# PoTaTo-Mika/fish-speech

Measured on AMD Instinct MI355X. Metric: audio-sec/wall-sec (RTF) + p50 first-sample latency, S2-Pro 4B @1/2/4/8 GPU, higher is better.
Workload: dtype bf16; 1 GPU; BASELINE config 2 per GPU: one utterance = 64-token prompt + 216 Dual-AR frames (top_k 30, top_p 0.8, temp 0.8) + codec decode [1,10,216] -> 442368 samples; global_batch=1, frames=216, prompt_len=64, first_chunk_frames=1, vocoder_chunks=first_chunk_frames, then growing 4x, vocoder=serial, parallelism=dp1

## Files before the change

### fish-speech_amd/csrc/fm_attn_dev.h

```cpp
#pragma once
#include "fm_common.h"
#include "fm_kernels.h"

constexpr int FAST_ATTN_MAXJ = 16;

template <typename T> __device__ __forceinline__ void ld_pair(const T* p, float& x0, float& x1) {
    if constexpr (sizeof(T) == 2) {
        const uint32_t w = *reinterpret_cast<const uint32_t*>(p);
        x0 = __uint_as_float(w << 16);
        x1 = __uint_as_float(w & 0xffff0000u);
    } else {
        x0 = ld(p, 0);
        x1 = ld(p, 1);
    }
}
template <typename T>
__device__ __forceinline__ void raw_pair(const T* qkv, int ldq, const float* qslab, int kp, int R, const T* bias,
                                         int r, size_t e, float& x0, float& x1) {
    if (qslab) {
        const size_t i = (size_t)r * ldq + e, st = (size_t)R * ldq;
        float a = qslab[i], b = qslab[i + 1];
        for (int q = 1; q < kp; ++q) {
            a += qslab[q * st + i];
            b += qslab[q * st + i + 1];
        }
        if (bias) {
            a += ld(bias, e);
            b += ld(bias, e + 1);
        }
        x0 = rnd<T>(a);
        x1 = rnd<T>(b);
    } else {
        ld_pair<T>(qkv + (size_t)r * ldq + e, x0, x1);
    }
}

template <typename T>
__device__ __forceinline__ void fast_attn_head(const FastFusedArgs<T>& a, int r, int h, int lane,
                                               unsigned long long (&tz)[7]) {
    const int hd = a.hd, g = a.nh / a.nkv, kvh = h / g, cpos = a.cpos, half = hd >> 1;
    const float* tab = a.rope + (size_t)cpos * hd;
    const int slot = a.row_slot[r];
    float q0[2], q1[2], k0[2], k1[2], v0[2], v1[2], qw0[2], qw1[2], kw0[2], kw1[2], c_[2], s_[2];
#pragma unroll
    for (int u = 0; u < 2; ++u) {
        const int p = lane + 64 * u;
        const bool ok = p < half;
        const int pp = ok ? p : 0;
        raw_pair<T>(a.qkv, a.ldqkv, a.qslab, a.qslab_kp, gridDim.x, a.qbias, r, (size_t)h * hd + 2 * pp, q0[u], q1[u]);
        raw_pair<T>(a.qkv, a.ldqkv, a.qslab, a.qslab_kp, gridDim.x, a.qbias, r, (size_t)(a.nh + kvh) * hd + 2 * pp,
                    k0[u], k1[u]);
        raw_pair<T>(a.qkv, a.ldqkv, a.qslab, a.qslab_kp, gridDim.x, a.qbias, r,
                    (size_t)(a.nh + a.nkv + kvh) * hd + 2 * pp, v0[u], v1[u]);
        qw0[u] = a.qk_norm ? ld(a.qn, 2 * pp) : 1.f;
        qw1[u] = a.qk_norm ? ld(a.qn, 2 * pp + 1) : 1.f;
        kw0[u] = a.qk_norm ? ld(a.kn, 2 * pp) : 1.f;
        kw1[u] = a.qk_norm ? ld(a.kn, 2 * pp + 1) : 1.f;
        c_[u] = tab[2 * pp];
        s_[u] = tab[2 * pp + 1];
        if (!ok) q0[u] = q1[u] = k0[u] = k1[u] = v0[u] = v1[u] = 0.f;
    }
    const size_t base = (size_t)slot * a.slot_stride + a.layer_off + (size_t)kvh * a.S * hd;
    T* kc = a.kc + base;
    T* vc = a.vc + base;
    float K0[FAST_ATTN_MAXJ][2], K1[FAST_ATTN_MAXJ][2], V0[FAST_ATTN_MAXJ][2], V1[FAST_ATTN_MAXJ][2];
#pragma unroll
    for (int j = 0; j < FAST_ATTN_MAXJ; ++j) {
        if (j < cpos) {
#pragma unroll
            for (int u = 0; u < 2; ++u) {
                const int p = lane + 64 * u;
                const int pp = p < half ? p : 0;
                ld_pair<T>(kc + (size_t)j * hd + 2 * pp, K0[j][u], K1[j][u]);
                ld_pair<T>(vc + (size_t)j * hd + 2 * pp, V0[j][u], V1[j][u]);
                if (p >= half) K0[j][u] = K1[j][u] = V0[j][u] = V1[j][u] = 0.f;
            }
        }
    }
    if (a.dbg) tz[1] = __builtin_amdgcn_s_memrealtime();
    auto prep = [&](float (&x0)[2], float (&x1)[2], const float (&w0)[2], const float (&w1)[2], bool norm) {
        if (norm) {
            float ss = 0.f;
#pragma unroll
            for (int u = 0; u < 2; ++u) ss += x0[u] * x0[u] + x1[u] * x1[u];
            ss = wave_sum(ss);
            const float rs = 1.0f / sqrtf(ss / (float)hd + a.eps);
#pragma unroll
            for (int u = 0; u < 2; ++u) {
                x0[u] = rnd<T>((x0[u] * rs) * w0[u]);
                x1[u] = rnd<T>((x1[u] * rs) * w1[u]);
            }
        }
#pragma unroll
        for (int u = 0; u < 2; ++u) {
            const float y0 = rnd<T>(x0[u] * c_[u] - x1[u] * s_[u]);
            const float y1 = rnd<T>(x1[u] * c_[u] + x0[u] * s_[u]);
            x0[u] = y0;
            x1[u] = y1;
        }
    };
    prep(q0, q1, qw0, qw1, a.qk_norm);
    prep(k0, k1, kw0, kw1, a.qk_norm);
    if (a.qdbg) {
#pragma unroll
        for (int u = 0; u < 2; ++u) {
            const int p = lane + 64 * u;
            if (p < half) {
                a.qdbg[((size_t)r * a.nh + h) * hd + 2 * p] = q0[u];
                a.qdbg[((size_t)r * a.nh + h) * hd + 2 * p + 1] = q1[u];
            }
        }
    }
    if (a.dbg) tz[2] = __builtin_amdgcn_s_memrealtime();
    if (h == kvh * g) {
#pragma unroll
        for (int u = 0; u < 2; ++u) {
            const int p = lane + 64 * u;
            if (p < half) {
                st(kc + (size_t)cpos * hd, 2 * p, k0[u]);
                st(kc + (size_t)cpos * hd, 2 * p + 1, k1[u]);
                st(vc + (size_t)cpos * hd, 2 * p, v0[u]);
                st(vc + (size_t)cpos * hd, 2 * p + 1, v1[u]);
            }
        }
    }
    float sc[FAST_ATTN_MAXJ + 1];
    float mx = -INFINITY;
#pragma unroll
    for (int j = 0; j <= FAST_ATTN_MAXJ; ++j) {
        if (j > cpos) break;
        float d = 0.f;
#pragma unroll
        for (int u = 0; u < 2; ++u) {
            const float a0 = j < cpos ? K0[j < FAST_ATTN_MAXJ ? j : 0][u] : k0[u];
            const float a1 = j < cpos ? K1[j < FAST_ATTN_MAXJ ? j : 0][u] : k1[u];
            d += q0[u] * a0 + q1[u] * a1;
        }
        d = wave_sum(d);
        sc[j] = rnd<T>(rnd<T>(d) * a.scale);
        mx = fmaxf(mx, sc[j]);
    }
    if (a.dbg) tz[3] = __builtin_amdgcn_s_memrealtime();
    float den = 0.f;
#pragma unroll
    for (int j = 0; j <= FAST_ATTN_MAXJ; ++j) {
        if (j > cpos) break;
        sc[j] = expf(sc[j] - mx);
        den += sc[j];
    }
    float o0[2] = {0.f, 0.f}, o1[2] = {0.f, 0.f};
#pragma unroll
    for (int j = 0; j <= FAST_ATTN_MAXJ; ++j) {
        if (j > cpos) break;
        const float p = rnd<T>(sc[j] / den);
#pragma unroll
        for (int u = 0; u < 2; ++u) {
            o0[u] += p * (j < cpos ? V0[j < FAST_ATTN_MAXJ ? j : 0][u] : v0[u]);
            o1[u] += p * (j < cpos ? V1[j < FAST_ATTN_MAXJ ? j : 0][u] : v1[u]);
        }
    }
    T* out = a.out + (size_t)r * a.nh * hd + (size_t)h * hd;
#pragma unroll
    for (int u = 0; u < 2; ++u) {
        const int p = lane + 64 * u;
        if (p < half) {
            st(out, 2 * p, o0[u]);
            st(out, 2 * p + 1, o1[u]);
        }
    }
}

constexpr int FATT_MAXPP = 8;
template <typename T>
__device__ __forceinline__ void fast_attn_heads8_lds(const FastFusedArgs<T>& a, int hbase, int hend, int lane,
                                                     const T* raw, const T* kvs, const T* qn, const T* kn,
                                                     const float* tab, T* out, bool store_kv, int slot) {
    const int hd = a.hd, g = a.nh / a.nkv, cpos = a.cpos, PP = hd >> 4;
    const int sub = lane & 7, h = hbase + (lane >> 3);
    const bool live = h < hend;
    const int hh = live ? h : hbase, kvh = hh / g;
    float q0[FATT_MAXPP], q1[FATT_MAXPP], k0[FATT_MAXPP], k1[FATT_MAXPP], v0[FATT_MAXPP], v1[FATT_MAXPP];
#pragma unroll
    for (int i = 0; i < FATT_MAXPP; ++i) {
        const int d = 2 * (sub + 8 * (i < PP ? i : 0));
        q0[i] = ld(raw, (size_t)hh * hd + d);
        q1[i] = ld(raw, (size_t)hh * hd + d + 1);
        k0[i] = ld(raw, (size_t)(a.nh + kvh) * hd + d);
        k1[i] = ld(raw, (size_t)(a.nh + kvh) * hd + d + 1);
        v0[i] = ld(raw, (size_t)(a.nh + a.nkv + kvh) * hd + d);
        v1[i] = ld(raw, (size_t)(a.nh + a.nkv + kvh) * hd + d + 1);
        if (i >= PP) q0[i] = q1[i] = k0[i] = k1[i] = v0[i] = v1[i] = 0.f;
    }
    auto sum8 = [](float v) {
        v += __shfl_xor(v, 1);
        v += __shfl_xor(v, 2);
        v += __shfl_xor(v, 4);
        return v;
    };
    auto prep = [&](float (&x0)[FATT_MAXPP], float (&x1)[FATT_MAXPP], const T* w, bool norm) {
        if (norm) {
            float ss = 0.f;
#pragma unroll
            for (int i = 0; i < FATT_MAXPP; ++i) ss += x0[i] * x0[i] + x1[i] * x1[i];
            ss = sum8(ss);
            const float rs = 1.0f / sqrtf(ss / (float)hd + a.eps);
#pragma unroll
            for (int i = 0; i < FATT_MAXPP; ++i) {
                const int d = 2 * (sub + 8 * (i < PP ? i : 0));
                x0[i] = rnd<T>((x0[i] * rs) * ld(w, d));
                x1[i] = rnd<T>((x1[i] * rs) * ld(w, d + 1));
            }
        }
#pragma unroll
        for (int i = 0; i < FATT_MAXPP; ++i) {
            const int d = 2 * (sub + 8 * (i < PP ? i : 0));
            const float c = tab[d], s = tab[d + 1];
            const float y0 = rnd<T>(x0[i] * c - x1[i] * s);
            const float y1 = rnd<T>(x1[i] * c + x0[i] * s);
            x0[i] = y0;
            x1[i] = y1;
        }
    };
    prep(q0, q1, qn, a.qk_norm);
    prep(k0, k1, kn, a.qk_norm);
    if (store_kv && live && h == kvh * g) {
        const size_t base = (size_t)slot * a.slot_stride + a.layer_off + (size_t)kvh * a.S * hd + (size_t)cpos * hd;
#pragma unroll
        for (int i = 0; i < FATT_MAXPP; ++i) {
            if (i < PP) {
                const int d = 2 * (sub + 8 * i);
                st(a.kc + base, d, k0[i]);
                st(a.kc + base, d + 1, k1[i]);
                st(a.vc + base, d, v0[i]);
                st(a.vc + base, d + 1, v1[i]);
            }
        }
    }
    const T* K = kvs + (size_t)(2 * kvh) * cpos * hd;
    const T* V = K + (size_t)cpos * hd;
    float sc[FAST_ATTN_MAXJ + 1];
    float mx = -INFINITY;
#pragma unroll
    for (int j = 0; j <= FAST_ATTN_MAXJ; ++j) {
        if (j > cpos) break;
        float dd = 0.f;
#pragma unroll
        for (int i = 0; i < FATT_MAXPP; ++i) {
            if (i < PP) {
                const int d = 2 * (sub + 8 * i);
                const float a0 = j < cpos ? ld(K, (size_t)j * hd + d) : k0[i];
                const float a1 = j < cpos ? ld(K, (size_t)j * hd + d + 1) : k1[i];
                dd += q0[i] * a0 + q1[i] * a1;
            }
        }
        dd = sum8(dd);
        sc[j] = rnd<T>(rnd<T>(dd) * a.scale);
        mx = fmaxf(mx, sc[j]);
    }
    float den = 0.f;
#pragma unroll
    for (int j = 0; j <= FAST_ATTN_MAXJ; ++j) {
        if (j > cpos) break;
        sc[j] = expf(sc[j] - mx);
        den += sc[j];
    }
    float o0[FATT_MAXPP], o1[FATT_MAXPP];
#pragma unroll
    for (int i = 0; i < FATT_MAXPP; ++i) o0[i] = o1[i] = 0.f;
#pragma unroll
    for (int j = 0; j <= FAST_ATTN_MAXJ; ++j) {
        if (j > cpos) break;
        const float pj = rnd<T>(sc[j] / den);
#pragma unroll
        for (int i = 0; i < FATT_MAXPP; ++i) {
            if (i < PP) {
                const int d = 2 * (sub + 8 * i);
                o0[i] += pj * (j < cpos ? ld(V, (size_t)j * hd + d) : v0[i]);
                o1[i] += pj * (j < cpos ? ld(V, (size_t)j * hd + d + 1) : v1[i]);
            }
        }
    }
    if (live) {
        T* o = out + (size_t)(h - hbase) * hd;
#pragma unroll
        for (int i = 0; i < FATT_MAXPP; ++i) {
            if (i < PP) {
                const int d = 2 * (sub + 8 * i);
                st(o, d, o0[i]);
                st(o, d + 1, o1[i]);
            }
        }
    }
}
```

### fish-speech_amd/csrc/fm_kernels.h

```cpp
#pragma once
#include <algorithm>
#include "fm_common.h"

enum { EPI_STORE = 0, EPI_RESID = 1, EPI_SWIGLU = 2, EPI_F32 = 3 };

template <typename T> void launch_swiglu_i8(hipStream_t s, const T* t, int ldt, T* act, int lda, int inter, int R);
template <typename T> void launch_pack(hipStream_t s, const T* src, int N, int K, T* dst);
template <typename T> void launch_quant_rows(hipStream_t s, T* w, int N, int K, int8_t* q, T* scale);
template <typename T> void launch_i8_to(hipStream_t s, const int8_t* q, int64_t n, T* dst);
void launch_pack_q8(hipStream_t s, const int8_t* src, int N, int K, int8_t* dst);
void launch_quant4(hipStream_t s, bf16_t* w, int N, int K, int gs, uint8_t* q, uint32_t* sz);
void launch_pack_q4(hipStream_t s, const uint8_t* q, int N, int K, uint8_t* dst);
void launch_pack_q4_rows(hipStream_t s, const uint8_t* q, int N, int K, uint32_t* dst);
void launch_pack_sz4(hipStream_t s, const uint32_t* sz, int N, int K, int gs, uint32_t* dst);

template <typename T> struct LinearArgs {
    const T* W;
    const T* W2;
    const T* bias;
    const T* X;
    int ldx, R, N, K;
    T* Y;
    int ldy;
    const T* res;
    int ldr;
    float* Yf;
    float* part = nullptr;
    int* tickets = nullptr;
    const T* wscale = nullptr;
};

template <typename T> struct QkArgs {
    const T* qkv;
    int ldqkv;
    const int* row_slot;
    const int* row_pos;
    int fixed_pos;
    int nh, nkv, hd, qk_norm;
    float eps;
    const T* qn;
    const T* kn;
    const float* rope;
    T* qout;
    T* kc;
    T* vc;
    size_t slot_stride, layer_off;
    int S;
    const float* qslab = nullptr;
    int qslab_kp = 1;
    const T* qbias = nullptr;
};

template <typename T> struct AttnArgs {
    const T* q;
    const int* row_slot;
    const int* row_pos;
    const T* kc;
    const T* vc;
    size_t slot_stride, layer_off;
    int S, nh, nkv, hd, split, maxsplit;
    float scale;
    float* part;
};

template <typename T> struct FastAttnArgs {
    const T* q;
    const int* row_slot;
    const T* kc;
    const T* vc;
    size_t slot_stride, layer_off;
    int S, nh, nkv, hd, cpos;
    float scale;
    T* out;
};

struct SlotParams {
    float temperature, top_p;
    int top_k, mask_im_end;
    uint64_t seed;
    int step;
    int force;
};

struct SampleArgs {
    const float* logits;
    int ldl, Nl;
    const int* row_slot;
    const SlotParams* sp;
    const int32_t* ras;
    int ras_stride, ras_enable;
    int slow, sb, se, im_end, cb, draw, col_idx;
    unsigned long long* dbg;
    int32_t* cols;
    int ldc;
    const int32_t* force_cols;
    float* tap;
    int tap_ld;
    int kth_fast;
};

template <typename T>
void launch_embed(hipStream_t s, const int32_t* tok, int R, const T* emb, const T* cbemb, int d,
                  int C, int cb, int sb, int se, int scale, T* x, const int* row_slot);
template <typename T>
void launch_gather_rows(hipStream_t s, const int32_t* codes, int ldc, int col, const T* table,
                        int d, int rows, int R, T* x);
template <typename T>
void launch_rmsnorm(hipStream_t s, const T* x, int ldx, const T* w, int d, float eps, T* y,
                    int ldy, int R);
template <typename T> void launch_linear(hipStream_t s, const LinearArgs<T>& a, int epi);
constexpr size_t LINEAR_PART_CAP = (size_t)8 << 20;
int linear_ksb(int N, int K, int R, int nacc, bool can_split);
template <typename T> void launch_qk_rope_cache(hipStream_t s, const QkArgs<T>& a, int R);
template <typename T>
void launch_attn(hipStream_t s, const AttnArgs<T>& a, int R, int nsplit, T* out, bool one_slot);
template <typename T> void launch_fast_attn(hipStream_t s, const FastAttnArgs<T>& a, int R);
void launch_finish(hipStream_t s, int R, const int* row_slot, int* row_pos, const int32_t* cols,
                   int ldc, int32_t* tok_in, int32_t* ras, int ras_stride, int C1, int update_ras,
                   SlotParams* sp);
template <typename T>
void launch_synth(hipStream_t s, T* dst, int64_t n, uint64_t seed, uint32_t tid, float center,
                  int log2_half);
template <typename T>
void launch_convert(hipStream_t s, const void* src, int src_bf16, int64_t n, T* dst);

enum { PRO_PLAIN = 0, PRO_NORM = 1, PRO_PRENORM = 3, PRO_FATT = 4 };
enum { EPI_SLAB = 4, EPI_SLABFIN = 5, EPI_SWIGLU8 = 7 };

template <typename T> struct FastFusedArgs {
    const T* qkv;
    int ldqkv;
    const int* row_slot;
    int nh, nkv, hd, qk_norm;
    float eps;
    const T* qn;
    const T* kn;
    const float* rope;
    T* kc;
    T* vc;
    size_t slot_stride, layer_off;
    int S, cpos;
    float scale;
    T* out;
    unsigned long long* dbg;
    float* qdbg = nullptr;
    int nwb = 4;
    const float* qslab = nullptr;
    int qslab_kp = 1;
    const T* qbias = nullptr;
    const int* row_pos = nullptr;
};
template <typename T> struct GemvArgs {
    const T* W;
    const T* W2;
    const T* bias;
    const T* X;
    int ldx;
    const int32_t* xidx;
    int xidx_ld, xidx_col;
    int xidx_rows;
    const int32_t* residx;
    const T* res;
    int ldr;
    const float* ss_in;
    int ss_gran;
    const T* nw;
    float eps;
    int R, N, K;
    T* Y;
    int ldy;
    float* Yf;
    T* res_out;
    int ldro;
    float* ss_out;
    int* tickets;
    T* xn_out;
    int ldxo;
    unsigned long long* dbg;
    FastFusedArgs<T> att;
    int fatt_off;
    const unsigned char* Wq;
    const T* wscale;
    const uint32_t* wsz;
    int q4_xsum_off;
    const T* pf_kc;
    const T* pf_vc;
    const int32_t* pf_slot;
    const int32_t* pf_pos;
    size_t pf_slot_stride, pf_layer_off;
    int pf_S, pf_nkv, pf_hd;
    int dummy_tail;
};
struct FmTuning {
    int gemv_nt = 1;
    int gemv_u = 8;
    int gemv_wpb = 4;
    int sampler_kth = 1;
    int sampler_fast = 1;
    int attn_cap = 32;
    int attn_wo = 0;
    int ksb_blocks = 512;
    int batched_fused_attn = 1;
    int attn_cap_batched = 128;
    int linear_u32 = 4;
    int linear_fill = 0;
    int attn3 = 1;
    int attn_fd = 1;
    int fd_min = 32;
    int fd_min_batched = 512;
    int fd_nw = 8;
    int fin_ksb = 0;
    int fd_nw_batched = 4;
    int fd_min16 = 256;
    int prefill_attn = 1;
    int prompt_gemm = 1;
    int prompt_skinny = 1;
    int prompt_skinny_blocks = 256;
    int prompt_unroll = 1;
    int prompt_qkv_slab = 1;
    int prompt_fin = 1;
    int prompt_swiglu = 1;
    int prompt_ks_tiles = 384;
    int prompt_ks_max = 8;
    int conv2 = 1;
    int conv_splitk = 1;
    int resunit_cfg = 1;
    int resunit_enc = 1;
    int resunit_384 = 1;
    int codec_norm = 1;
    int codec_rope = 1;
    int codec_swiglu = 1;
    int codec_fuse = 1;
    int bstream = 1;
    int bstream_kparts = 0;
    int bstream_nw = 0;
    int bs_dummy = 2;
    int gemv_dummy = 2;
    int bs_qkv_slab = 1;
    int fast_tail = 1;
    int fkv_prefetch = 0;
    int kv_prefetch = 1;
    int bstream_chain = 0;
    int bstream_acc = 1;
    int rmsnorm_block = 0;
    int ksb_balance = 0;
    int chain_max = 4;
    int chain_sleep = 4;
    int gemv_chain = 0;
    int bs_xfirst = 1;
    int bs_vec_epi = 1;
    int bsacc_kparts = 0;
    int q_u = 4;
    int fin8 = 1;
    int fin_split = 0;
    int int4_stream = 1;
    int fw_delay = 0;
    int fw_cheap = 0;
    int fw_prio = 0;
    int fattn_wo = 1;
    int row_qkv_rp = 8;
    int rowgemv_q4 = 31;
    int rowgemv = 27;
    int row_copies = 1;
    int prefix_vec = 1;
    unsigned long long* dbg = nullptr;
};
FmTuning& fm_tuning();
struct KvPrefixArgs {
    char *kc, *vc;
    char* store;
    const int* slots;
    size_t slot_stride_b, layer_stride_b, head_stride_b;
    size_t run_bytes;
    int64_t run_units;
    int nkv;
    int to_store;
};
void launch_kv_prefix_copy(hipStream_t s, const KvPrefixArgs& a, int n_layer, int nslots);
inline size_t fatt_lds_bytes(int ldqkv, int nkv, int S, int hd, size_t esz) {
    return ((size_t)ldqkv + (size_t)nkv * 2 * (S - 1) * hd + 2 * (size_t)hd) * esz + (size_t)hd * 4 + 64;
}
inline size_t gemv_lds_bytes(int R, int Kb, size_t esz) {
    return (size_t)R * (Kb + 8) * esz + 16 * sizeof(float) + (2 * 8 * 16 + 16) * (size_t)R * sizeof(float) +
           8 * 8 * sizeof(float);
}
template <typename T> void launch_gemv(hipStream_t s, const GemvArgs<T>& a, int pro, int epi, int ksb);
enum { ROWGEMV_FIN = 0, ROWGEMV_NORM_STORE = 1, ROWGEMV_NORM_SWIGLU = 2, ROWGEMV_NORM_F32 = 3 };
struct RowGemvArgs {
    const bf16_t* W;
    const int8_t* Wq;
    const bf16_t* wscale;
    const uint32_t* Wq4;
    const uint32_t* wsz;
    int gs;
    const bf16_t* X;
    int ldx;
    const int32_t* xidx;
    int xcol, xrows;
    const bf16_t* bias;
    const bf16_t* nw;
    float eps;
    const bf16_t* res;
    int ldr;
    const int32_t* residx;
    int res_col, res_rows;
    bf16_t* res_out;
    bf16_t* Y;
    float* Yf;
    int N, K;
    const bf16_t* pf_kc;
    const bf16_t* pf_vc;
    const int32_t* pf_slot;
    const int32_t* pf_pos;
    size_t pf_slot_stride, pf_layer_off;
    int pf_S, pf_nkv, pf_hd;
    unsigned long long* dbg;
};
int rowgemv_u(int K, int qm);
void launch_rowgemv(hipStream_t s, const RowGemvArgs& a, int kind);
struct FattnWoArgs {
    FastFusedArgs<bf16_t> at;
    RowGemvArgs wo;
    uint32_t* xt;
    int gen;
    int* err;
    int delay;
    int cheap;
    int prio;
    unsigned long long* dbg;
};
bool fattn_wo_ok(int nh, int nkv, int hd, int cpos, int N, int K, int qm);
void launch_fattn_wo(hipStream_t s, const FattnWoArgs& a);
constexpr int GEMV_CHAIN_MAX = 4;
constexpr int GEMV_CHAIN_LINE = 32;
constexpr int GEMV_CHAIN_SLOTS = 17;
constexpr int GEMV_CHAIN_WORDS = GEMV_CHAIN_MAX * GEMV_CHAIN_SLOTS * GEMV_CHAIN_LINE;
enum { GEMV_CHAIN_WO_W2 = 0, GEMV_CHAIN_W13 = 1, GEMV_CHAIN_QKV = 2, GEMV_CHAIN_HEAD = 3 };
template <typename T> struct GemvChainArgs {
    GemvArgs<T> st[GEMV_CHAIN_MAX];
    int kind[GEMV_CHAIN_MAX];
    int off[GEMV_CHAIN_MAX + 1];
    int n;
    unsigned* cnt;
    int* err;
    int sleep;
};
template <typename T> void launch_gemv_chain(hipStream_t s, const GemvChainArgs<T>& c);

template <typename T> struct BstreamArgs {
    const T* W;
    const T* bias;
    const T* X;
    int ldx, R, N, K;
    T* Y;
    int ldy;
    float* Yf;
    int kparts = 1;
    const T* wscale = nullptr;
    unsigned long long* dbg = nullptr;
    int pro = 0;
    const float* ss_in = nullptr;
    const T* nw = nullptr;
    float eps = 0.f;
    const T* res = nullptr;
    int ldr = 0;
    T* res_out = nullptr;
    int ldro = 0;
    float* ss_out = nullptr;
    int* tickets = nullptr;
    int dummy_tail = 0;
    int xfirst = 1;
    int vec_epi = 1;
};
struct BstreamPlan {
    bool ok = false;
    int kparts = 1, nw = 0, spw = 0, tpi = 1, grid = 0;
    int acc = 0, ntm = 0;
};
BstreamPlan bstream_plan(int N, int K, int R, int epi, size_t esz);
void bsacc_init();
template <typename T> bool launch_bstream(hipStream_t s, const BstreamArgs<T>& a, int epi, const BstreamPlan& p);
template <typename T> struct FinalizeArgs {
    const float* slab;
    int kparts, lds;
    const T* bias;
    const T* res;
    int ldr;
    T* x_out;
    int ldx;
    const T* nw;
    float eps;
    T* xn_out;
    int ldxn, d, R;
    const T* wscale = nullptr;
    int ch = 0;
    int* cnt = nullptr;
    float* ss_part = nullptr;
    int fin8 = 0;
    int* err = nullptr;
};
template <typename T> void launch_finalize_norm(hipStream_t s, const FinalizeArgs<T>& a);

struct PromptSkinnyArgs {
    const bf16_t* w;
    const bf16_t* x;
    int ldx, R, N, K;
    float* slab;
    bf16_t* act = nullptr;
    int lda = 0;
};
void launch_prompt_skinny(hipStream_t s, const PromptSkinnyArgs& a, int ks);
int prompt_skinny_ks(int N, int K, int target);

template <typename T> struct AttnDecArgs {
    const T* qkv;
    int ldqkv;
    const int* row_slot;
    const int* row_pos;
    int nh, nkv, hd, qk_norm;
    float eps;
    const T* qn;
    const T* kn;
    const float* rope;
    T* kc;
    T* vc;
    size_t slot_stride, layer_off;
    int S, maxsplit;
    float scale;
    float* part;
    int cap;
    int* cnt;
    T* out;
    unsigned long long* dbg;
    float* qdbg = nullptr;
    int nwb = 4;
    const float* qslab = nullptr;
    int qslab_kp = 1;
    const T* qbias = nullptr;
};
template <typename T> void launch_attn_decode2(hipStream_t s, const AttnDecArgs<T>& a, int R);
inline size_t attn2_lds_bytes(int hd, int g, int cap, size_t esz) {
    return (size_t)cap * (hd + 8) * esz + (size_t)cap * hd * esz + (size_t)g * hd * 4 + (size_t)g * cap * 4 +
           16 + 8 * (size_t)g * 4;
}
inline int attn2_cap(int hd, int g, size_t esz) {
    long budget = 150L * 1024 - 16 - 8L * g * 4 - (long)g * hd * 4;
    long per = (long)(2 * hd + 8) * (long)esz + 4L * g;
    long c = budget / per;
    c = c > 256 ? 256 : c;
    return (int)(c & ~15L);
}
constexpr int FD_NSP = 16;
inline bool attn_fd_ok(int hd, int g) { return (hd == 32 || hd == 64 || hd == 128) && g >= 1 && g <= 4; }
template <typename T> void launch_attn_fd(hipStream_t s, const AttnDecArgs<T>& a, int R);
template <typename T> void launch_attn_decode3(hipStream_t s, const AttnDecArgs<T>& a, int R);
template <typename T> void launch_fast_attn_fused(hipStream_t s, const FastFusedArgs<T>& a, int R);
template <typename T> void launch_fast_attn2(hipStream_t s, const FastFusedArgs<T>& a, int R);
template <typename T> void launch_sample_radix(hipStream_t s, const SampleArgs& a, int R);
void sample_init();
template <typename T>
void launch_attn_combine(hipStream_t s, const float* part, const int* row_pos, int R, int nh, int hd,
                         int split, int maxsplit, T* out);
```

### fish-speech_amd/csrc/fm_llm.cpp

```cpp
#include <dlfcn.h>
#include <execinfo.h>
#include <hip/hip_runtime.h>
#include <math.h>
#include <signal.h>

#include <algorithm>
#include <array>
#include <memory>

#include "fm_codec.h"
#include "fm_kernels.h"
#include "fm_runtime.h"

namespace {
void segv_trace(int sig, siginfo_t* si, void*) {
    void* fr[64];
    const int n = backtrace(fr, 64);
    fprintf(stderr, "fishmi: signal %d at address %p, %d frames\n", sig, si ? si->si_addr : nullptr, n);
    for (int i = 0; i < n; ++i) {
        Dl_info d{};
        if (dladdr(fr[i], &d) && d.dli_fname)
            fprintf(stderr, "  #%d %s +0x%lx (%s)\n", i, d.dli_fname,
                    (unsigned long)((const char*)fr[i] - (const char*)d.dli_fbase), d.dli_sname ? d.dli_sname : "?");
        else
            fprintf(stderr, "  #%d %p\n", i, fr[i]);
    }
    fflush(stderr);
    signal(sig, SIG_DFL);
    raise(sig);
}
struct SegvTraceInstaller {
    SegvTraceInstaller() {
        const char* e = getenv("FISHMI_SEGV_TRACE");
        if (!e || e[0] != '1') return;
        struct sigaction sa {};
        sa.sa_sigaction = segv_trace;
        sa.sa_flags = SA_SIGINFO;
        sigaction(SIGSEGV, &sa, nullptr);
        sigaction(SIGBUS, &sa, nullptr);
    }
} g_segv_trace;
}

static thread_local std::string g_err;
void fm_set_error(const std::string& s) { g_err = s; }
extern "C" const char* fm_last_error(void) { return g_err.c_str(); }
extern "C" int fm_device_count(void) {
    int n = 0;
    if (hipGetDeviceCount(&n) != hipSuccess) return 0;
    return n;
}

static constexpr int PREFILL_CHUNK = 1024;
static constexpr int ATTN_PIECE = 256;
static constexpr int ATTN_SPLIT = 64;
static constexpr int GEMV_MAX_ROWS = 8;
static constexpr int KSB_MAX = 8;
static constexpr int BS_KPARTS = 8;

FmTuning& fm_tuning() {
    static FmTuning t;
    return t;
}

static int pick_ksb(int N, int K, int R, size_t esz) {
    const int nb = (N + 15) / 16;
    const FmTuning& tu = fm_tuning();
    int ksb = 1;
    while (ksb < KSB_MAX && nb * ksb < tu.ksb_blocks && K % (32 * ksb * 2) == 0) ksb *= 2;
    if (tu.ksb_balance) {
        double best = 1e9;
        int bk = ksb;
        for (int k = 1; k <= KSB_MAX && K % (32 * k) == 0; k *= 2) {
            const int b = nb * k;
            if (b < 256) continue;
            const double rounds = (double)((b + 255) / 256), waste = rounds * 256.0 / b;
            if (waste < best - 1e-3) {
                best = waste;
                bk = k;
            }
        }
        ksb = bk;
    }
    while (gemv_lds_bytes(R, K / ksb, esz) > 96 * 1024 && ksb < KSB_MAX && K % (32 * ksb * 2) == 0) ksb *= 2;
    while (K / ksb > 4096 && K % (32 * ksb * 2) == 0) ksb *= 2;
    return ksb;
}

struct LayerW {
    void *wqkv = nullptr, *bqkv = nullptr, *wo = nullptr, *bo = nullptr, *qn = nullptr, *kn = nullptr;
    void *w13 = nullptr, *w2 = nullptr, *an = nullptr, *fn = nullptr;
    void *wo_rm = nullptr, *w2_rm = nullptr, *wqkv_rm = nullptr, *w13_rm = nullptr;
};

struct StackDims {
    int n_layer, dim, nh, nkv, hd, inter, qkv_bias, o_bias, qk_norm;
    int nq() const { return nh * hd; }
    int nqkv() const { return (nh + 2 * nkv) * hd; }
};

struct fm_llm {
    fm_model_config c{};
    int device = 0, prec = FM_PREC_BF16, max_slots = 1;
    size_t esz = 2;
    hipStream_t stream = nullptr;
    std::map<std::string, DTensor> w;
    bool finalized = false;
    StackDims sd{}, fdm{};
    int S = 0, C = 0, C1 = 0, cb = 0, nsem = 0, Nhead = 0, maxsplit = 0, Rmax = 0;
    std::vector<LayerW> slow, fast;
    void *emb = nullptr, *cbemb = nullptr, *norm = nullptr, *head_c = nullptr, *fproj_w = nullptr,
         *fproj_b = nullptr, *femb = nullptr, *fnorm = nullptr, *fout = nullptr;
    void *kc = nullptr, *vc = nullptr, *fkc = nullptr, *fvc = nullptr;
    size_t slot_stride = 0, layer_stride = 0, fslot_stride = 0, flayer_stride = 0;
    float *rope = nullptr, *frope = nullptr;
    void *x = nullptr, *h = nullptr, *xn = nullptr, *qkv = nullptr, *q = nullptr, *att = nullptr,
         *act = nullptr;
    void *xl = nullptr, *xnl = nullptr, *fx = nullptr, *fh = nullptr, *fxn = nullptr;
    void *x2 = nullptr, *fx2 = nullptr;
    unsigned* chain_cnt = nullptr;
    int* chain_err = nullptr;
    int* h_chain_err = nullptr;
    void* plast = nullptr;
    float *part = nullptr, *logits = nullptr, *flogits = nullptr;
    void* act2 = nullptr;
    int* attn_cnt = nullptr;
    float *ssX = nullptr, *ssH = nullptr;
    int* tickets = nullptr;
    float* skpart = nullptr;
    long long skpart_cap = 0;
    float *slabA = nullptr, *slabB = nullptr;
    float *bsA = nullptr, *bsB = nullptr;
    float* bsQ = nullptr;
    int *frame_slot = nullptr, *frame_pos = nullptr, *prow_slot = nullptr, *prow_pos = nullptr;
    int32_t *tok_in = nullptr, *cols = nullptr, *ptok = nullptr, *ras = nullptr;
    SlotParams* sp = nullptr;
    int32_t* force_cols = nullptr;
    float *tap_slow = nullptr, *tap_fast = nullptr;
    std::vector<int> host_force;
    int32_t* h_cols = nullptr;
    int32_t* h_hist = nullptr;
    size_t h_hist_n = 0;
    std::vector<int> host_pos, host_step;
    std::vector<int> uploaded_slots;
    bool use_graph = true;
    std::map<int, hipGraphExec_t> graphs;
    Profiler prof;
    std::vector<void*> allocs;
    int quant = FM_QUANT_NONE;
    int q4_gs = 0;
    int* fin_cnt = nullptr;
    float* fin_ss = nullptr;
    struct QInfo {
        const unsigned char* q8 = nullptr;
        const void* scale = nullptr;
        const uint32_t* sz = nullptr;
    };
    std::map<const void*, QInfo> qmap;
    std::map<const void*, void*> rowmajor;
    std::map<const void*, const void*> rowsz;
    std::map<const void*, const void*> rowscale;
    bool row_ok = false;
    bool row_qkv_ok = false;
    bool row_w13_ok = false;
    uint32_t* fxt = nullptr;
    void* fout_rm = nullptr;
    int32_t* fiota = nullptr;
    struct Prefix {
        void* buf = nullptr;
        int npos = 0;
        size_t bytes = 0;
    };
    std::map<int, Prefix> prefixes;
    int next_prefix_id = 1;
    int* pfx_slots = nullptr;
    const QInfo* qinfo(const void* W) const {
        auto it = qmap.find(W);
        return it == qmap.end() ? nullptr : &it->second;
    }

    ~fm_llm() {
        if (device >= 0) (void)hipSetDevice(device);
        for (auto& g : graphs) (void)hipGraphExecDestroy(g.second);
        for (auto& kv : w) {
            if (kv.second.p) (void)hipFree(kv.second.p);
            if (kv.second.q) (void)hipFree(kv.second.q);
        }
        for (void* p : allocs) (void)hipFree(p);
        for (auto& kv : prefixes) (void)hipFree(kv.second.buf);
        if (h_cols) (void)hipHostFree(h_cols);
        if (h_hist) (void)hipHostFree(h_hist);
        if (h_chain_err) (void)hipHostFree(h_chain_err);
        if (stream) (void)hipStreamDestroy(stream);
    }
    void* dalloc(size_t bytes, bool zero = true) {
        void* p = nullptr;
        if (bytes == 0) bytes = 16;
        hipError_t e = hipMalloc(&p, bytes);
        if (e != hipSuccess)
            throw FmError{FM_ERR_OOM, "hipMalloc(" + std::to_string(bytes) + ") failed: " + hipGetErrorString(e)};
        if (zero) HIPCHK(hipMemsetAsync(p, 0, bytes, stream));
        allocs.push_back(p);
        return p;
    }
};

static void add_t(fm_llm* m, const std::string& n, int64_t rows, int64_t cols) {
    DTensor t;
    t.rows = rows;
    t.cols = cols;
    t.numel = rows * cols;
    m->w[n] = t;
}
static void add_stack(fm_llm* m, const std::string& pre, const StackDims& s) {
    for (int i = 0; i < s.n_layer; ++i) {
        std::string p = pre + std::to_string(i) + ".";
        add_t(m, p + "attention.wqkv.weight", s.nqkv(), s.dim);
        if (s.qkv_bias) add_t(m, p + "attention.wqkv.bias", 1, s.nqkv());
        add_t(m, p + "attention.wo.weight", s.dim, s.nq());
        if (s.o_bias) add_t(m, p + "attention.wo.bias", 1, s.dim);
        if (s.qk_norm) {
            add_t(m, p + "attention.q_norm.weight", 1, s.hd);
            add_t(m, p + "attention.k_norm.weight", 1, s.hd);
        }
        add_t(m, p + "feed_forward.w1.weight", s.inter, s.dim);
        add_t(m, p + "feed_forward.w3.weight", s.inter, s.dim);
        add_t(m, p + "feed_forward.w2.weight", s.dim, s.inter);
        add_t(m, p + "ffn_norm.weight", 1, s.dim);
        add_t(m, p + "attention_norm.weight", 1, s.dim);
    }
}

static void build_inventory(fm_llm* m) {
    const fm_model_config& c = m->c;
    m->sd = StackDims{c.n_layer, c.dim, c.n_head, c.n_local_heads, c.head_dim, c.intermediate_size,
                      c.qkv_bias, c.o_bias, c.qk_norm};
    m->fdm = StackDims{c.n_fast_layer, c.fast_dim, c.fast_n_head, c.fast_n_local_heads, c.fast_head_dim,
                       c.fast_intermediate_size, c.fast_qkv_bias, c.fast_o_bias, c.fast_qk_norm};
    add_t(m, "embeddings.weight", c.vocab_size, c.dim);
    add_t(m, "codebook_embeddings.weight", (int64_t)c.codebook_size * c.num_codebooks, c.dim);
    add_stack(m, "layers.", m->sd);
    add_t(m, "norm.weight", 1, c.dim);
    if (!c.tie_word_embeddings) add_t(m, "output.weight", c.vocab_size, c.dim);
    if (c.fast_dim != c.dim) {
        add_t(m, "fast_project_in.weight", c.fast_dim, c.dim);
        add_t(m, "fast_project_in.bias", 1, c.fast_dim);
    }
    add_t(m, "fast_embeddings.weight", c.codebook_size, c.fast_dim);
    add_stack(m, "fast_layers.", m->fdm);
    add_t(m, "fast_norm.weight", 1, c.fast_dim);
    add_t(m, "fast_output.weight", c.codebook_size, c.fast_dim);
}

static DTensor& tensor_for(fm_llm* m, const char* name, int64_t numel) {
    auto it = m->w.find(name);
    FMCHECK(it != m->w.end(), std::string("unknown tensor: ") + name);
    FMCHECK(it->second.numel == numel, std::string("wrong numel for ") + name + ": got " +
                                           std::to_string(numel) + ", want " + std::to_string(it->second.numel));
    DTensor& t = it->second;
    if (!t.p) {
        const int64_t rows = t.rows > 1 ? (t.rows + 15) / 16 * 16 : 1;
        const size_t bytes = (size_t)rows * t.cols * m->esz;
        HIPCHK(hipMalloc(&t.p, bytes));
        HIPCHK(hipMemsetAsync(t.p, 0, bytes, m->stream));
    }
    return t;
}

template <typename T> struct Run {
    typedef T type_t;
    fm_llm* m;
    hipStream_t s;
    int64_t E;
    bool rows_distinct_slots = false;
    explicit Run(fm_llm* mm) : m(mm), s(mm->stream), E(sizeof(T)) {}

    bool prompt_gemm(const void* W, const void* W2, const void* bias, const void* X, int ldx, int R, int N, int K,
                     void* Y, int ldy, const void* res, int ldr, int epi, const char* cls) {
        if (R <= 32 || W2 || m->qinfo(W) || !fm_tuning().prompt_gemm ||
            (epi != EPI_STORE && epi != EPI_RESID && epi != EPI_SWIGLU8) || N % 16 || K % 32 || N < 96 ||
            (epi == EPI_SWIGLU8 && (bias || N % 16)))
            return false;
        ConvArgs<T> c{};
        c.x = (const T*)X;
        c.ldx = ldx;
        c.Ci = K;
        c.Lq = R;
        c.Lx = R;
        c.w = (const T*)W;
        c.Co = N;
        c.ntaps = 1;
        c.stride = 1;
        c.nphase = 1;
        c.bias = (const T*)bias;
        c.res = epi == EPI_RESID ? (const T*)res : nullptr;
        c.ldr = ldr;
        c.out = Y;
        c.ldo = ldy;
        c.flags = CE_STORE | (bias ? CE_BIAS : 0) | (epi == EPI_RESID ? CE_RES : 0) |
                  (epi == EPI_SWIGLU8 ? CE_SWIGLU8 : 0);
        hipStream_t st = s;
        const int64_t bytes = (int64_t)N * K * E + (int64_t)R * K * E + (int64_t)R * N * E;
        const double flops = 2.0 * R * N * K;
        if constexpr (sizeof(T) == 2) {
            auto al16 = [](const void* p) { return ((uintptr_t)p & 15) == 0; };
            const int ks = prompt_skinny_ks(N, K, fm_tuning().prompt_skinny_blocks);
            if (fm_tuning().prompt_skinny && ks > 0 && R <= 64 && ldx % 8 == 0 && al16(X) && al16(Y) && ldy % 8 == 0 &&
                (!c.res || (al16(c.res) && ldr % 8 == 0)) && (long long)ks * R * N <= m->skpart_cap) {
                c.ksplit = ks;
                c.slab = m->skpart;
                c.slab_cap = (size_t)m->skpart_cap;
                PromptSkinnyArgs p{(const bf16_t*)W, (const bf16_t*)X, ldx, R, N, K, m->skpart};
                const bool direct = ks == 1 && epi == EPI_SWIGLU8;
                if (direct) {
                    p.act = (bf16_t*)Y;
                    p.lda = ldy;
                }
                auto go = [st, c, p, ks, direct] {
                    launch_prompt_skinny(st, p, ks);
                    if (!direct) launch_conv_epi<T>(st, c);
                };
                m->prof.record(cls, bytes, go);
                run_(cls, bytes, flops, go);
                return true;
            }
        }
        if (epi == EPI_SWIGLU8) return false;
        const long long t128 = (long long)FM_CEIL(R, 128) * FM_CEIL(N, 128);
        int ks = 1;
        while (t128 * ks < fm_tuning().prompt_ks_tiles && ks < fm_tuning().prompt_ks_max && K / 32 >= 8 * ks * 2)
            ks *= 2;
        c.ksplit = ks;
        c.slab = m->skpart;
        c.slab_cap = (size_t)m->skpart_cap;
        auto go = [st, c] { launch_conv_gemm<T>(st, c); };
        m->prof.record(cls, bytes, go);
        run_(cls, bytes, flops, go);
        return true;
    }
    bool prompt_slab(const void* W, const void* X, int ldx, int R, int N, int K, int* ks_out) {
        if constexpr (sizeof(T) != 2) {
            return false;
        } else {
            if (!fm_tuning().prompt_fin || !fm_tuning().prompt_skinny || !fm_tuning().prompt_gemm || R <= 32 ||
                R > 64 || m->qinfo(W) || N % 16 || K % 32 || ldx % 8 || ((uintptr_t)X & 15))
                return false;
            const int ks = prompt_skinny_ks(N, K, fm_tuning().prompt_skinny_blocks);
            if (ks <= 0 || (long long)ks * R * N > m->skpart_cap) return false;
            const PromptSkinnyArgs p{(const bf16_t*)W, (const bf16_t*)X, ldx, R, N, K, m->skpart};
            hipStream_t st = s;
            auto go = [st, p, ks] { launch_prompt_skinny(st, p, ks); };
            const int64_t bytes = (int64_t)N * K * E + (int64_t)R * K * E + (int64_t)ks * R * N * 4;
            m->prof.record("linear", bytes, go);
            run_("linear", bytes, 2.0 * R * N * K, go);
            *ks_out = ks;
            return true;
        }
    }
    void linear(const void* W, const void* W2, const void* bias, const void* X, int ldx, int R, int N,
                int K, void* Y, int ldy, const void* res, int ldr, float* Yf, int epi, const char* cls) {
        if (bs_use(R, false) && !W2 && !res && (epi == EPI_F32 || epi == EPI_STORE) &&
            bs_linear(W, bias, X, ldx, R, N, K, Y, ldy, Yf, epi))
            return;
        if (prompt_gemm(W, W2, bias, X, ldx, R, N, K, Y, ldy, res, ldr, epi, cls)) return;
        LinearArgs<T> a{(const T*)W, (const T*)W2, (const T*)bias, (const T*)X, ldx, R, N, K, (T*)Y,
                        ldy, (const T*)res, ldr, Yf};
        if (const auto* q = m->qinfo(W)) a.wscale = (const T*)q->scale;
        if (R > GEMV_MAX_ROWS && R <= 64) {
            FMCHECK(m->skpart_cap >= (long long)LINEAR_PART_CAP, "split-K partial buffer too small");
            a.part = m->skpart;
            a.tickets = m->tickets;
        }
        const int64_t wbytes = (int64_t)N * K * E * (epi == EPI_SWIGLU ? 2 : 1);
        const int64_t bytes = wbytes + (int64_t)R * K * E + (int64_t)R * N * (epi == EPI_F32 ? 4 : E);
        const double flops = 2.0 * R * N * K * (epi == EPI_SWIGLU ? 2 : 1);
        hipStream_t st = s;
        auto go = [st, a, epi] { launch_linear<T>(st, a, epi); };
        m->prof.record(cls, bytes, go);
        run_(cls, bytes, flops, go);
    }

    struct BsPending {
        bool on = false;
        const float* slab = nullptr;
        int kparts = 0, d = 0, R = 0;
        void* res = nullptr;
        void* out = nullptr;
        const void* sc = nullptr;
    } pend;
    void attn_slow(const AttnDecArgs<T>& aa, int R) { attn_slow_on(s, aa, R); }
    static void attn_slow_on(hipStream_t s, const AttnDecArgs<T>& aa, int R) {
        if (fm_tuning().attn_fd && attn_fd_ok(aa.hd, aa.nh / aa.nkv)) {
            AttnDecArgs<T> b = aa;
            b.cap = std::max(16, R > GEMV_MAX_ROWS ? fm_tuning().fd_min_batched : fm_tuning().fd_min);
            if (R <= GEMV_MAX_ROWS && fm_tuning().fd_nw > 4) {
                b.nwb = fm_tuning().fd_nw;
                b.cap = std::max(16, fm_tuning().fd_min16);
            } else if (R > GEMV_MAX_ROWS && fm_tuning().fd_nw_batched > 4) {
                b.nwb = fm_tuning().fd_nw_batched;
            }
            launch_attn_fd<T>(s, b, R);
        } else if (fm_tuning().attn3 && R > GEMV_MAX_ROWS && aa.hd % 32 == 0 && aa.hd <= 128 && aa.nh / aa.nkv <= 6)
            launch_attn_decode3<T>(s, aa, R);
        else
            launch_attn_decode2<T>(s, aa, R);
    }
    bool bs_frame = false;
    bool bs_use(int R, bool) const {
        return fm_tuning().bstream && bs_frame && R > GEMV_MAX_ROWS && R <= 32 && m->bsA;
    }
    struct BsExtra {
        int pro = PRO_PLAIN;
        const float* ss_in = nullptr;
        const void* nw = nullptr;
        const void* res = nullptr;
        void* res_out = nullptr;
        float* ss_out = nullptr;
    };
    bool bs_linear(const void* W, const void* bias, const void* X, int ldx, int R, int N, int K, void* Y, int ldy,
                   float* Yf, int epi, int* kparts_out = nullptr, const BsExtra* ex = nullptr) {
        const BstreamPlan p = bstream_plan(N, K, R, epi, E);
        if (!p.ok || ((epi == EPI_SLABFIN || (ex && ex->pro == PRO_PRENORM)) && !p.acc)) return false;
        BstreamArgs<T> a{(const T*)W, (const T*)bias, (const T*)X, ldx, R, N, K, (T*)Y, ldy, Yf};
        if (const auto* q = m->qinfo(W)) a.wscale = (const T*)q->scale;
        a.dbg = fm_tuning().dbg;
        if (ex) {
            a.pro = ex->pro;
            a.ss_in = ex->ss_in;
            a.nw = (const T*)ex->nw;
            a.eps = m->c.norm_eps;
            a.res = (const T*)ex->res;
            a.ldr = N;
            a.res_out = (T*)ex->res_out;
            a.ldro = N;
            a.ss_out = ex->ss_out;
            a.tickets = m->tickets;
        }
        const int64_t bytes = (int64_t)N * K * E + (int64_t)R * K * E +
                              (int64_t)R * N * (epi == EPI_SLAB ? 4 * p.kparts : (epi == EPI_F32 ? 4 : E));
        const double flops = 2.0 * R * N * K;
        hipStream_t st = s;
        auto go = [st, a, epi, p] { FMCHECK(launch_bstream<T>(st, a, epi, p), "bstream: no kernel for the plan"); };
        m->prof.record("linear", bytes, go);
        run_("linear", bytes, flops, go);
        if (kparts_out) *kparts_out = p.kparts;
        return true;
    }
    const void* wscale(const void* W) const {
        const auto* q = m->qinfo(W);
        return q ? q->scale : nullptr;
    }
    bool x_ss = false;
    bool bs_chain(const StackDims& d, int R) const {
        if (!fm_tuning().bstream_chain || E != 2 || R > 32) return false;
        auto ok = [&](int N, int K, int epi) { return bstream_plan(N, K, R, epi, E).acc; };
        return ok(d.nqkv(), d.dim, EPI_STORE) && ok(d.dim, d.nq(), EPI_SLABFIN) && ok(2 * d.inter, d.dim, EPI_SWIGLU8) &&
               ok(d.dim, d.inter, EPI_SLABFIN);
    }
    void finalize_norm(const float* slab, int kparts, const void* bias, const void* res, void* out, const void* nw,
                       void* xn, int d, int R, const void* sc) {
        FinalizeArgs<T> f{slab, kparts, d, (const T*)bias, (const T*)res, d, (T*)out, d, (const T*)nw,
                          m->c.norm_eps, (T*)xn, d, d, R, (const T*)sc};
        if (fm_tuning().fin_split > 1 && m->fin_cnt) {
            f.ch = fm_tuning().fin_split;
            f.cnt = m->fin_cnt;
            f.ss_part = m->fin_ss;
            f.err = m->chain_err;
        }
        run_("norm", 0, 0, [&] { launch_finalize_norm<T>(s, f); });
    }
// ... 28 lines not shown
            e.ss_in = m->ssX;
            e.nw = L.an;
            FMCHECK(bs_linear(L.wqkv, L.bqkv, xb, d.dim, R, d.nqkv(), d.dim, m->qkv, d.nqkv(), nullptr, EPI_STORE,
                              nullptr, &e),
                    "bsacc: no PRENORM QKV plan");
        } else if (bs) {
            bs_norm_in(d, L, R, xb, xnb);
            int kp = 0;
            const bool fused_fast = is_fast && fixed_pos >= 0 && fixed_pos < 16 && d.hd <= 256;
            const bool fused_slow = !is_fast && rows_distinct_slots && fm_tuning().attn_fd &&
                                    attn_fd_ok(d.hd, d.nh / d.nkv);
            const bool slab_ok = fm_tuning().bs_qkv_slab && fm_tuning().batched_fused_attn && m->bsQ && R <= 32 &&
                                 (fused_fast || fused_slow) && !m->qinfo(L.wqkv);
            if (slab_ok && bs_linear(L.wqkv, nullptr, xnb, d.dim, R, d.nqkv(), d.dim, nullptr, d.nqkv(), m->bsQ,
                                     EPI_SLAB, &kp)) {
                qslab = m->bsQ;
                qslab_kp = kp;
            } else if (!bs_linear(L.wqkv, L.bqkv, xnb, d.dim, R, d.nqkv(), d.dim, m->qkv, d.nqkv(), nullptr, EPI_STORE))
                linear(L.wqkv, nullptr, L.bqkv, xnb, d.dim, R, d.nqkv(), d.dim, m->qkv, d.nqkv(), nullptr, 0,
                       nullptr, EPI_STORE, "linear");
        } else {
            bs_norm_in(d, L, R, xb, xnb);
            int kq = 0;
            if (!is_fast && !rows_distinct_slots && fm_tuning().prompt_qkv_slab &&
                prompt_slab(L.wqkv, xnb, d.dim, R, d.nqkv(), d.dim, &kq)) {
                qslab = m->skpart;
                qslab_kp = kq;
            } else {
                linear(L.wqkv, nullptr, L.bqkv, xnb, d.dim, R, d.nqkv(), d.dim, m->qkv, d.nqkv(), nullptr, 0,
                       nullptr, EPI_STORE, "linear");
            }
        }
        const float scale = 1.0f / sqrtf((float)d.hd);
        const bool rows_are_slots = is_fast || rows_distinct_slots;
        if (rows_are_slots && !is_fast && fm_tuning().batched_fused_attn) {
            AttnDecArgs<T> aa{(const T*)m->qkv, d.nqkv(), rslot, rpos, d.nh, d.nkv, d.hd, d.qk_norm, eps,
                              (const T*)L.qn, (const T*)L.kn, rope, (T*)kc, (T*)vc, sstride, loff, Sc,
                              m->maxsplit, scale, m->part};
            aa.cap = attn2_cap(d.hd, d.nh / d.nkv, E);
            if (fm_tuning().attn_cap_batched) aa.cap = std::min(aa.cap, fm_tuning().attn_cap_batched);
            aa.maxsplit = FM_CEIL(Sc, aa.cap);
            aa.cnt = m->attn_cnt;
            aa.dbg = fm_tuning().dbg;
            aa.out = (T*)m->att;
            aa.qslab = qslab;
            aa.qslab_kp = qslab_kp;
            aa.qbias = (const T*)L.bqkv;
            FMCHECK(!qslab || (fm_tuning().attn_fd && attn_fd_ok(d.hd, d.nh / d.nkv)), "bs_qkv_slab needs attn_fd");
            hipStream_t st = s;
            auto go = [st, aa, R] { attn_slow_on(st, aa, R); };
            m->prof.record("attn_slow", 0, go);
            run_rec("attn", go);
        } else if (is_fast && fm_tuning().batched_fused_attn && fixed_pos >= 0 && fixed_pos < 16 && d.hd <= 256) {
            FastFusedArgs<T> fa{(const T*)m->qkv, d.nqkv(), rslot, d.nh, d.nkv, d.hd, d.qk_norm, eps,
                                (const T*)L.qn, (const T*)L.kn, rope, (T*)kc, (T*)vc, sstride, loff, Sc,
                                fixed_pos, scale, (T*)m->att};
            fa.dbg = fm_tuning().dbg;
            fa.qslab = qslab;
            fa.qslab_kp = qslab_kp;
            fa.qbias = (const T*)L.bqkv;
            hipStream_t st = s;
            run_rec("attn", [st, fa, R] { launch_fast_attn2<T>(st, fa, R); });
        } else {
            QkArgs<T> qa{(const T*)m->qkv, d.nqkv(), rslot, rpos, fixed_pos, d.nh, d.nkv, d.hd, d.qk_norm,
                         eps, (const T*)L.qn, (const T*)L.kn, rope, (T*)m->q, (T*)kc, (T*)vc, sstride, loff, Sc};
            qa.qslab = qslab;
            qa.qslab_kp = qslab_kp;
            qa.qbias = (const T*)L.bqkv;
            run_("rope", 0, 0, [&] { launch_qk_rope_cache<T>(s, qa, R); });
            if (!is_fast) {
                auto attn_rows = [&](int r0, int len, bool one_slot) {
                    for (int p0 = r0; p0 < r0 + len; p0 += ATTN_PIECE) {
                        const int pn = std::min(ATTN_PIECE, r0 + len - p0);
                        const size_t o = (size_t)p0 * d.nh * d.hd;
                        AttnArgs<T> aa{(const T*)m->q + o, rslot + p0, rpos + p0, (const T*)kc, (const T*)vc, sstride,
                                       loff, Sc, d.nh, d.nkv, d.hd, ATTN_SPLIT, m->maxsplit, scale, m->part};
                        run_("attn", 0, 0, [&] { launch_attn<T>(s, aa, pn, m->maxsplit, (T*)m->att + o, one_slot); });
                    }
                };
                if (!segs.empty())
                    for (const auto& sg : segs) attn_rows(sg[0], sg[1], true);
                else
                    attn_rows(0, R, !rows_are_slots);
            } else {
                FastAttnArgs<T> fa{(const T*)m->q, rslot, (const T*)kc, (const T*)vc, sstride, loff, Sc,
                                   d.nh, d.nkv, d.hd, fixed_pos, scale, (T*)m->att};
                run_("attn", 0, 0, [&] { launch_fast_attn<T>(s, fa, R); });
            }
        }
        int kp = 0;
        if (chain) {
            BsExtra eo;
            eo.res = xb;
            eo.res_out = hb;
            eo.ss_out = m->ssH;
            FMCHECK(bs_linear(L.wo, L.bo, m->att, d.nq(), R, d.dim, d.nq(), nullptr, d.dim, m->bsA, EPI_SLABFIN, &kp, &eo),
                    "bsacc: no SLABFIN wo plan");
            BsExtra e13;
            e13.pro = PRO_PRENORM;
            e13.ss_in = m->ssH;
            e13.nw = L.fn;
            FMCHECK(bs_linear(L.w13, nullptr, hb, d.dim, R, 2 * d.inter, d.dim, m->act, d.inter, nullptr, EPI_SWIGLU8,
                              nullptr, &e13),
                    "bsacc: no PRENORM w13 plan");
            BsExtra e2;
            e2.res = hb;
            e2.res_out = xb;
            e2.ss_out = m->ssX;
            FMCHECK(bs_linear(L.w2, nullptr, m->act, d.inter, R, d.dim, d.inter, nullptr, d.dim, m->bsB, EPI_SLABFIN, &kp,
                              &e2),
                    "bsacc: no SLABFIN w2 plan");
            x_ss = true;
            return;
        }
        if (bs && bs_linear(L.wo, nullptr, m->att, d.nq(), R, d.dim, d.nq(), nullptr, d.dim, m->bsA, EPI_SLAB, &kp)) {
            finalize_norm(m->bsA, kp, L.bo, xb, hb, L.fn, xnb, d.dim, R, wscale(L.wo));
        } else if (!bs && prompt_slab(L.wo, m->att, d.nq(), R, d.dim, d.nq(), &kp)) {
            finalize_norm(m->skpart, kp, L.bo, xb, hb, L.fn, xnb, d.dim, R, nullptr);
        } else {
            linear(L.wo, nullptr, L.bo, m->att, d.nq(), R, d.dim, d.nq(), hb, d.dim, xb, d.dim, nullptr,
                   EPI_RESID, "linear");
            run_("norm", 0, 0, [&] {
                launch_rmsnorm<T>(s, (const T*)hb, d.dim, (const T*)L.fn, d.dim, eps, (T*)xnb, d.dim, R);
            });
        }
        if (!(bs && bs_linear(L.w13, nullptr, xnb, d.dim, R, 2 * d.inter, d.dim, m->act, d.inter, nullptr,
                              EPI_SWIGLU8))) {
            if (!(fm_tuning().prompt_swiglu &&
                  prompt_gemm(L.w13, nullptr, nullptr, xnb, d.dim, R, 2 * d.inter, d.dim, m->act, d.inter, nullptr, 0,
                              EPI_SWIGLU8, "linear"))) {
                linear(L.w13, nullptr, nullptr, xnb, d.dim, R, 2 * d.inter, d.dim, m->act2, 2 * d.inter, nullptr, 0,
                       nullptr, EPI_STORE, "linear");
                run_("other", 0, 0, [&] {
                    launch_swiglu_i8<T>(s, (const T*)m->act2, 2 * d.inter, (T*)m->act, d.inter, d.inter, R);
                });
            }
        }
        if (bs && bs_linear(L.w2, nullptr, m->act, d.inter, R, d.dim, d.inter, nullptr, d.dim, m->bsB, EPI_SLAB, &kp)) {
            pend.on = true;
            pend.slab = m->bsB;
            pend.kparts = kp;
            pend.d = d.dim;
            pend.R = R;
            pend.res = hb;
            pend.out = xb;
            pend.sc = wscale(L.w2);
        } else if (!bs && prompt_slab(L.w2, m->act, d.inter, R, d.dim, d.inter, &kp)) {
            pend.on = true;
            pend.slab = m->skpart;
            pend.kparts = kp;
            pend.d = d.dim;
            pend.R = R;
            pend.res = hb;
            pend.out = xb;
            pend.sc = nullptr;
        } else {
            linear(L.w2, nullptr, nullptr, m->act, d.inter, R, d.dim, d.inter, xb, d.dim, hb, d.dim, nullptr,
                   EPI_RESID, "linear");
        }
    }

    GemvArgs<T> ga() {
        GemvArgs<T> a{};
        a.eps = m->c.norm_eps;
        a.dummy_tail = fm_tuning().gemv_dummy;
        return a;
    }
    struct ChainSt {
        GemvArgs<T> a;
        int kind;
        int64_t bytes;
        double flops;
    };
    std::vector<ChainSt> chain;
    int chain_kind(const GemvArgs<T>& a, int pro, int epi, int ksb) const {
        const FmTuning& t = fm_tuning();
        if (!t.gemv_chain || m->prof.on || ksb != 1 || a.R != 1 || a.Wq || m->qinfo(a.W) || !t.gemv_nt ||
            t.gemv_u != 8 || t.gemv_wpb != 4 || a.N % 16 || a.xidx)
            return -1;
        if (pro == PRO_PLAIN && epi == EPI_SLABFIN) return GEMV_CHAIN_WO_W2;
        if (a.xn_out || a.K > 4096 || pro != PRO_PRENORM) return a.xn_out && pro == PRO_PRENORM && epi == EPI_F32 &&
                                                                    a.K <= 4096 ? GEMV_CHAIN_HEAD : -1;
        if (epi == EPI_SWIGLU8) return GEMV_CHAIN_W13;
        if (epi == EPI_STORE) return GEMV_CHAIN_QKV;
        if (epi == EPI_F32) return GEMV_CHAIN_HEAD;
        return -1;
    }
    void chain_flush() {
        if (chain.empty()) return;
        std::vector<ChainSt> c;
        c.swap(chain);
        if (c.size() == 1) {
            static const int pro_of[4] = {PRO_PLAIN, PRO_PRENORM, PRO_PRENORM, PRO_PRENORM};
            static const int epi_of[4] = {EPI_SLABFIN, EPI_SWIGLU8, EPI_STORE, EPI_F32};
            gemv_now(c[0].a, pro_of[c[0].kind], epi_of[c[0].kind], 1, "linear");
            return;
        }
        GemvChainArgs<T> g{};
        int64_t bytes = 0;
        double flops = 0;
        g.n = (int)c.size();
        for (int i = 0; i < g.n; ++i) {
            g.st[i] = c[i].a;
            if (!g.st[i].tickets) g.st[i].tickets = m->tickets;
            g.kind[i] = c[i].kind;
            bytes += c[i].bytes;
            flops += c[i].flops;
        }
        g.cnt = m->chain_cnt;
        g.err = m->chain_err;
        g.sleep = fm_tuning().chain_sleep;
        hipStream_t st = s;
        auto go = [st, g] { launch_gemv_chain<T>(st, g); };
        m->prof.record("linear", bytes, go);
        m->prof.run(s, "linear", bytes, flops, go);
    }
    void gemv(GemvArgs<T> a, int pro, int epi, int ksb, const char* cls) {
        const int kind = chain_kind(a, pro, epi, ksb);
        if (kind < 0) {
            chain_flush();
            gemv_now(a, pro, epi, ksb, cls);
            return;
        }
        const size_t E = sizeof(T);
        const int64_t bytes = (int64_t)a.N * a.K * E + (int64_t)a.K * E;
        chain.push_back(ChainSt{a, kind, bytes, 2.0 * a.N * a.K});
        if ((int)chain.size() >= std::min(GEMV_CHAIN_MAX, fm_tuning().chain_max) || kind == GEMV_CHAIN_HEAD)
            chain_flush();
    }
    void gemv_now(GemvArgs<T> a, int pro, int epi, int ksb, const char* cls) {
        int64_t wbytes = (int64_t)a.N * a.K * E * (epi == EPI_SWIGLU ? 2 : 1);
        const auto* q = m->qinfo(a.W);
        if (q && q->sz && !fm_tuning().int4_stream) q = nullptr;
        if (q) {
            a.Wq = q->q8;
            if (q->sz) {
                a.wsz = q->sz;
                a.wscale = nullptr;
                while (ksb > 1 && (a.K / ksb) % 128) ksb /= 2;
                wbytes = (int64_t)a.N * a.K / 2 + (int64_t)(a.N + 15) / 16 * 16 * (a.K / 128) * 4;
            } else {
                a.wscale = (const T*)q->scale;
                while (ksb > 1 && (a.K / ksb) % 64) ksb /= 2;
                wbytes = (int64_t)a.N * a.K;
            }
        }
        const int64_t bytes = wbytes + (int64_t)a.R * a.K * E;
        const double flops = 2.0 * a.R * a.N * a.K * (epi == EPI_SWIGLU ? 2 : 1);
        hipStream_t st = s;
        if (!a.tickets) a.tickets = m->tickets;
        auto go = [st, a, pro, epi, ksb] { launch_gemv<T>(st, a, pro, epi, ksb); };
        m->prof.record(cls, bytes, go);
        m->prof.run(s, cls, bytes, flops, go);
    }
    int row_bits() const {
        const FmTuning& t = fm_tuning();
        return m->quant == FM_QUANT_INT4 ? t.rowgemv_q4 : t.rowgemv;
    }
    bool row_fin(int n) const {
        const FmTuning& t = fm_tuning();
        return sizeof(T) == 2 && n == 1 && m->row_ok && (row_bits() & 1) && !t.gemv_chain && !t.attn_wo &&
               (m->quant != FM_QUANT_INT4 || t.int4_stream);
    }
    bool row_qkv(int n) const {
        const FmTuning& t = fm_tuning();
        return sizeof(T) == 2 && n == 1 && m->row_qkv_ok && m->quant != FM_QUANT_INT8 && (row_bits() & 2) &&
               !t.gemv_chain && (m->quant != FM_QUANT_INT4 || t.int4_stream);
    }
    bool row_w13(int n) const {
        const FmTuning& t = fm_tuning();
        return sizeof(T) == 2 && n == 1 && m->row_w13_ok && (row_bits() & 4) && !t.gemv_chain &&
               (m->quant != FM_QUANT_INT4 || t.int4_stream);
    }
    void rowgemv(const RowGemvArgs& a, int kind) {
        chain_flush();
        const int64_t wbytes = a.Wq4 ? (int64_t)a.N * a.K / 2 + (int64_t)a.N * (a.K / a.gs) * 4
                               : (a.Wq ? (int64_t)a.N * a.K + (int64_t)a.N * 2 : (int64_t)a.N * a.K * 2);
        const int64_t bytes = wbytes + (int64_t)a.K * 2;
        hipStream_t st = s;
        auto go = [st, a, kind] { launch_rowgemv(st, a, kind); };
        m->prof.record("linear", bytes, go);
        m->prof.run(s, "linear", bytes, 2.0 * a.N * a.K, go);
    }
    template <typename F> void run_(const char* cls, int64_t bytes, double flops, F&& f) {
        chain_flush();
        m->prof.run(s, cls, bytes, flops, std::forward<F>(f));
    }
    template <typename F> void run_rec(const char* cls, F go) {
        chain_flush();
        m->prof.record(cls, 0, go);
        m->prof.run(s, cls, 0, 0, go);
    }
    struct KsbPlan {
        int wo, w2;
    };
    KsbPlan plan(const StackDims& d, int n) {
        auto fin_ksb = [&](int N, int K) {
            const int fk = fm_tuning().fin_ksb;
            if (fk > 0 && K % (32 * fk) == 0) return fk;
            return gemv_lds_bytes(n, K, E) <= 120 * 1024 ? 1 : pick_ksb(N, K, n, E);
        };
        return KsbPlan{fin_ksb(d.dim, d.nq()), fin_ksb(d.dim, d.inter)};
    }
    void block_small(const StackDims& d, const LayerW& L, int n, bool first, const void* x_in, int ldx_in,
                     const int32_t* xidx, int xcol, void* xb, void* hb, bool is_fast, int cpos, int layer,
                     const KsbPlan& kp, void* xo, bool kv_only = false) {
        const int C1 = m->C1;
        const float scale = 1.0f / sqrtf((float)d.hd);
        FastFusedArgs<T> fa{(const T*)m->qkv, d.nqkv(), m->frame_slot, d.nh, d.nkv, d.hd, d.qk_norm,
                            m->c.norm_eps, (const T*)L.qn, (const T*)L.kn, m->frope, (T*)m->fkc,
                            (T*)m->fvc, m->fslot_stride, (size_t)layer * m->flayer_stride, m->C, cpos,
                            scale, (T*)m->att};
        fa.dbg = fm_tuning().dbg;
        const bool rf = row_fin(n);
        auto row_w = [&](RowGemvArgs& r, void* rm, const void* packed) {
            if (m->quant == FM_QUANT_INT4) {
                r.Wq4 = (const uint32_t*)rm;
                r.wsz = (const uint32_t*)m->rowsz.at(packed);
                r.gs = m->q4_gs;
            } else if (m->quant) {
                r.Wq = (const int8_t*)rm;
                auto it = m->rowscale.find(packed);
                r.wscale = (const bf16_t*)(it != m->rowscale.end() ? it->second : m->qinfo(packed)->scale);
            } else {
                r.W = (const bf16_t*)rm;
            }
        };
        const int fq = m->quant == FM_QUANT_INT8 ? 1 : (m->quant == FM_QUANT_INT4 ? 2 : 0);
        const bool fw = is_fast && !kv_only && rf && fm_tuning().fattn_wo && m->fxt && m->fdm.n_layer * m->C >= 2 &&
                        m->fdm.n_layer * m->C <= 40 &&
                        fattn_wo_ok(d.nh, d.nkv, d.hd, cpos, d.dim, d.nq(), fq);
        const bool att_wo = is_fast && !kv_only && fm_tuning().attn_wo && !m->quant && n == 1 && cpos < 16 && d.hd % 16 == 0 &&
                            d.hd <= 128 && d.nh % d.nkv == 0 && (d.nq() / kp.wo) % d.hd == 0 && d.nqkv() % 8 == 0;
        {
            GemvArgs<T> a = ga();
            a.W = (const T*)L.wqkv;
            a.bias = (const T*)L.bqkv;
            a.nw = (const T*)L.an;
            a.R = n;
            a.N = d.nqkv();
            a.K = d.dim;
            a.Y = (T*)m->qkv;
            a.ldy = d.nqkv();
            if (!is_fast && n == 1 && fm_tuning().kv_prefetch) {
                a.pf_kc = (const T*)m->kc;
                a.pf_vc = (const T*)m->vc;
                a.pf_slot = m->frame_slot;
                a.pf_pos = m->frame_pos;
                a.pf_slot_stride = m->slot_stride;
                a.pf_layer_off = (size_t)layer * m->layer_stride;
                a.pf_S = m->S;
                a.pf_nkv = d.nkv;
                a.pf_hd = d.hd;
            } else if (is_fast && n == 1 && fm_tuning().fkv_prefetch && m->fiota && cpos < 16) {
                a.pf_kc = (const T*)m->fkc;
                a.pf_vc = (const T*)m->fvc;
                a.pf_slot = m->frame_slot;
                a.pf_pos = m->fiota + cpos;
                a.pf_slot_stride = m->fslot_stride;
                a.pf_layer_off = (size_t)layer * m->flayer_stride;
                a.pf_S = m->C;
                a.pf_nkv = d.nkv;
                a.pf_hd = d.hd;
            }
            const int epi = EPI_STORE;
            if (row_qkv(n) && (!first || (row_bits() & 16))) {
                RowGemvArgs r{};
                row_w(r, L.wqkv_rm, L.wqkv);
                if (first) {
                    r.X = (const bf16_t*)x_in;
                    r.ldx = ldx_in;
                    r.xidx = xidx;
                    r.xcol = xcol;
                    r.xrows = xidx ? m->cb : 0;
                } else {
                    r.X = (const bf16_t*)xb;
                }
                r.bias = (const bf16_t*)L.bqkv;
                r.nw = (const bf16_t*)L.an;
                r.eps = m->c.norm_eps;
                r.Y = (bf16_t*)m->qkv;
                r.N = d.nqkv();
                r.K = d.dim;
                r.pf_kc = (const bf16_t*)a.pf_kc;
                r.pf_vc = (const bf16_t*)a.pf_vc;
                r.pf_slot = a.pf_slot;
                r.pf_pos = a.pf_pos;
                r.pf_slot_stride = a.pf_slot_stride;
                r.pf_layer_off = a.pf_layer_off;
                r.pf_S = a.pf_S;
                r.pf_nkv = a.pf_nkv;
                r.pf_hd = a.pf_hd;
                rowgemv(r, ROWGEMV_NORM_STORE);
            } else if (first) {
                a.X = (const T*)x_in;
                a.ldx = ldx_in;
                a.xidx = xidx;
                a.xidx_ld = C1;
                a.xidx_col = xcol;
                a.xidx_rows = xidx ? m->cb : 0;
                gemv(a, PRO_NORM, epi, 1, "linear");
            } else {
                a.X = (const T*)xb;
                a.ldx = d.dim;
                a.ss_in = m->ssX;
                a.ss_gran = rf ? 1 : 0;
                gemv(a, PRO_PRENORM, epi, 1, "linear");
            }
        }
        if (!is_fast) {
            AttnDecArgs<T> aa{(const T*)m->qkv, d.nqkv(), m->frame_slot, m->frame_pos, d.nh, d.nkv, d.hd,
                              d.qk_norm, m->c.norm_eps, (const T*)L.qn, (const T*)L.kn, m->rope, (T*)m->kc,
                              (T*)m->vc, m->slot_stride, (size_t)layer * m->layer_stride, m->S,
                              m->maxsplit, scale, m->part};
            aa.cap = attn2_cap(d.hd, d.nh / d.nkv, E);
            if (fm_tuning().attn_cap) aa.cap = std::min(aa.cap, fm_tuning().attn_cap);
            aa.maxsplit = FM_CEIL(m->S, aa.cap);
            aa.cnt = m->attn_cnt;
            aa.dbg = fm_tuning().dbg;
            aa.out = (T*)m->att;
            hipStream_t st = s;
            auto go = [st, aa, n] { attn_slow_on(st, aa, n); };
            m->prof.record("attn_slow", 0, go);
            run_rec("attn", go);
        } else if (!att_wo && !fw) {
            hipStream_t st = s;
            const bool f2 = cpos < 16 && d.hd <= 256;
            run_rec("attn", [st, fa, n, f2] {
                if (f2)
                    launch_fast_attn2<T>(st, fa, n);
                else
                    launch_fast_attn_fused<T>(st, fa, n);
            });
        }
        if (kv_only) return;
        if (fw) {
            FattnWoArgs A{};
            A.at = *reinterpret_cast<const FastFusedArgs<bf16_t>*>(&fa);
            A.at.dbg = nullptr;
            A.at.row_pos = m->frame_pos;
            RowGemvArgs& r = A.wo;
            row_w(r, L.wo_rm, L.wo);
            r.X = (const bf16_t*)m->att;
            r.bias = (const bf16_t*)L.bo;
            if (first) {
                r.res = (const bf16_t*)x_in;
                r.ldr = ldx_in;
                r.residx = xidx;
                r.res_col = xcol;
                r.res_rows = xidx ? m->cb : 0;
            } else {
                r.res = (const bf16_t*)xb;
                r.ldr = d.dim;
            }
            r.res_out = (bf16_t*)hb;
            r.N = d.dim;
            r.K = d.nq();
            A.xt = m->fxt;
            A.gen = 1 + layer + m->fdm.n_layer * cpos;
            A.err = m->chain_err;
            A.delay = fm_tuning().fw_delay;
            A.cheap = fm_tuning().fw_cheap;
            A.prio = fm_tuning().fw_prio;
            chain_flush();
            const int64_t bytes = r.Wq4 ? (int64_t)r.N * r.K / 2 + (int64_t)r.N * (r.K / r.gs) * 4
                                  : (r.Wq ? (int64_t)r.N * r.K + (int64_t)r.N * 2 : (int64_t)r.N * r.K * 2);
            hipStream_t st = s;
            auto go = [st, A] { launch_fattn_wo(st, A); };
            m->prof.record("attn_wo", bytes, go);
            m->prof.run(s, "attn", bytes, 2.0 * r.N * r.K, go);
        } else if (rf) {
            RowGemvArgs r{};
            row_w(r, L.wo_rm, L.wo);
            r.X = (const bf16_t*)m->att;
            r.bias = (const bf16_t*)L.bo;
            if (first) {
                r.res = (const bf16_t*)x_in;
                r.ldr = ldx_in;
                r.residx = xidx;
                r.res_col = xcol;
                r.res_rows = xidx ? m->cb : 0;
            } else {
                r.res = (const bf16_t*)xb;
                r.ldr = d.dim;
            }
            r.res_out = (bf16_t*)hb;
            r.N = d.dim;
            r.K = d.nq();
            rowgemv(r, ROWGEMV_FIN);
        } else {
            GemvArgs<T> a = ga();
            a.W = (const T*)L.wo;
            a.bias = (const T*)L.bo;
            a.X = (const T*)m->att;
            a.ldx = d.nq();
            a.R = n;
            a.N = d.dim;
            a.K = d.nq();
            a.Yf = m->slabA;
            a.ldy = d.dim;
            if (first) {
                a.res = (const T*)x_in;
                a.ldr = ldx_in;
                a.residx = xidx;
                a.xidx_ld = C1;
                a.xidx_col = xcol;
                a.xidx_rows = xidx ? m->cb : 0;
            } else {
                a.res = (const T*)xb;
                a.ldr = d.dim;
            }
            a.res_out = (T*)hb;
            a.ldro = d.dim;
            a.ss_out = m->ssH;
            a.tickets = m->tickets;
            if (att_wo) {
                a.att = fa;
                gemv(a, PRO_FATT, EPI_SLABFIN, kp.wo, "linear");
            } else {
                gemv(a, PRO_PLAIN, EPI_SLABFIN, kp.wo, "linear");
            }
        }
        if (row_w13(n)) {
            RowGemvArgs r{};
            row_w(r, L.w13_rm, L.w13);
            r.X = (const bf16_t*)hb;
            r.nw = (const bf16_t*)L.fn;
            r.eps = m->c.norm_eps;
            r.Y = (bf16_t*)m->act;
            r.N = 2 * d.inter;
            r.K = d.dim;
            rowgemv(r, ROWGEMV_NORM_SWIGLU);
        } else {
            GemvArgs<T> a = ga();
            a.W = (const T*)L.w13;
            a.nw = (const T*)L.fn;
            a.R = n;
            a.N = 2 * d.inter;
            a.K = d.dim;
            a.X = (const T*)hb;
            a.ldx = d.dim;
            a.ss_in = m->ssH;
            a.ss_gran = rf ? 1 : 0;
            a.Y = (T*)m->act;
            a.ldy = d.inter;
            gemv(a, PRO_PRENORM, EPI_SWIGLU8, 1, "linear");
        }
        if (rf) {
            RowGemvArgs r{};
            row_w(r, L.w2_rm, L.w2);
            r.X = (const bf16_t*)m->act;
            r.res = (const bf16_t*)hb;
            r.ldr = d.dim;
            r.res_out = (bf16_t*)xo;
            r.N = d.dim;
            r.K = d.inter;
            rowgemv(r, ROWGEMV_FIN);
        } else {
            GemvArgs<T> a = ga();
            a.W = (const T*)L.w2;
            a.X = (const T*)m->act;
            a.ldx = d.inter;
            a.R = n;
            a.N = d.dim;
            a.K = d.inter;
            a.Yf = m->slabB;
            a.ldy = d.dim;
            a.res = (const T*)hb;
            a.ldr = d.dim;
            a.res_out = (T*)xo;
            a.ldro = d.dim;
            a.ss_out = m->ssX;
            a.tickets = m->tickets;
            gemv(a, PRO_PLAIN, EPI_SLABFIN, kp.w2, "linear");
        }
    }

    void* xbuf(void* x0, void* x1, int l) const { return (fm_tuning().gemv_chain && (l & 1)) ? x1 : x0; }
    void* xfin = nullptr;
    void slow_small(int n) {
        const KsbPlan kp = plan(m->sd, n);
        for (int l = 0; l < m->sd.n_layer; ++l)
            block_small(m->sd, m->slow[l], n, l == 0, m->x, m->c.dim, nullptr, 0, xbuf(m->x, m->x2, l), m->h, false, 0,
                        l, kp, xbuf(m->x, m->x2, l + 1));
        xfin = xbuf(m->x, m->x2, m->sd.n_layer);
    }

    const void* head_small(const void* xlast, bool pending, int n, int ksb_prev) {
        const fm_model_config& c = m->c;
        GemvArgs<T> a = ga();
        a.W = (const T*)m->head_c;
        a.nw = (const T*)m->norm;
        a.R = n;
        a.N = m->Nhead;
        a.K = c.dim;
        a.Yf = m->logits;
        a.ldy = m->Nhead;
        a.xn_out = (T*)m->xnl;
        a.ldxo = c.dim;
        const void* xs = xfin ? xfin : m->x;
        if (pending) {
            a.X = (const T*)xs;
            a.ldx = c.dim;
            a.ss_in = m->ssX;
            a.ss_gran = row_fin(n) ? 1 : 0;
            gemv(a, PRO_PRENORM, EPI_F32, 1, "linear");
        } else {
            a.X = (const T*)xlast;
            a.ldx = c.dim;
            gemv(a, PRO_NORM, EPI_F32, 1, "linear");
        }
        const void* hid = c.norm_fastlayer_input ? m->xnl : (pending ? xs : xlast);
        if (m->fproj_w) {
            GemvArgs<T> p = ga();
            p.W = (const T*)m->fproj_w;
            p.bias = (const T*)m->fproj_b;
            p.X = (const T*)hid;
            p.ldx = c.dim;
            p.R = n;
            p.N = c.fast_dim;
            p.K = c.dim;
            p.Y = (T*)m->xl;
            p.ldy = c.fast_dim;
            gemv(p, PRO_PLAIN, EPI_STORE, 1, "linear");
            return m->xl;
        }
        return hid;
    }

    void fast_small(int n, int cc, bool with_head, const void* hidden) {
        const fm_model_config& c = m->c;
        const KsbPlan kp = plan(m->fdm, n);
        for (int l = 0; l < m->fdm.n_layer; ++l) {
            const bool first = l == 0;
            const void* xin = cc == 0 ? hidden : m->femb;
            const int32_t* xidx = cc == 0 ? nullptr : m->cols;
            const bool kv_only = !with_head && l == m->fdm.n_layer - 1 && fm_tuning().fast_tail;
            block_small(m->fdm, m->fast[l], n, first, xin, c.fast_dim, xidx, cc, xbuf(m->fx, m->fx2, l), m->fh, true,
                        cc, l, kp, xbuf(m->fx, m->fx2, l + 1), kv_only);
        }
        if (with_head && sizeof(T) == 2 && n == 1 && m->fout_rm && (row_bits() & 8) && !fm_tuning().gemv_chain &&
            (m->quant != FM_QUANT_INT4 || fm_tuning().int4_stream)) {
            RowGemvArgs r{};
            auto row_w = [&](RowGemvArgs& rr, void* rm, const void* packed) {
                if (m->quant == FM_QUANT_INT4) {
                    rr.Wq4 = (const uint32_t*)rm;
                    rr.wsz = (const uint32_t*)m->rowsz.at(packed);
                    rr.gs = m->q4_gs;
                } else if (m->quant) {
                    rr.Wq = (const int8_t*)rm;
                    rr.wscale = (const bf16_t*)m->qinfo(packed)->scale;
                } else {
                    rr.W = (const bf16_t*)rm;
                }
            };
            row_w(r, m->fout_rm, m->fout);
            r.X = (const bf16_t*)xbuf(m->fx, m->fx2, m->fdm.n_layer);
            r.nw = (const bf16_t*)m->fnorm;
            r.eps = c.norm_eps;
            r.Yf = m->flogits;
            r.N = m->cb;
            r.K = c.fast_dim;
            rowgemv(r, ROWGEMV_NORM_F32);
        } else if (with_head) {
            GemvArgs<T> a = ga();
            a.W = (const T*)m->fout;
            a.nw = (const T*)m->fnorm;
            a.R = n;
            a.N = m->cb;
            a.K = c.fast_dim;
            a.Yf = m->flogits;
            a.ldy = m->cb;
            a.X = (const T*)xbuf(m->fx, m->fx2, m->fdm.n_layer);
            a.ldx = c.fast_dim;
            a.ss_in = m->ssX;
            a.ss_gran = row_fin(n) ? 1 : 0;
            gemv(a, PRO_PRENORM, EPI_F32, 1, "linear");
        }
    }

    void frame_tail_small(int n, bool ras_enable, bool sample, const void* hidden) {
        if (sample) {
            SampleArgs a = sargs(true, ras_enable, 0);
            run_("sample", 0, 0, [&] { launch_sample_radix<T>(s, a, n); });
        }
        fast_small(n, 0, false, hidden);
        for (int cc = 1; cc < m->C; ++cc) {
            fast_small(n, cc, true, hidden);
            if (sample) {
                SampleArgs a = sargs(false, 0, cc);
                run_("sample", 0, 0, [&] { launch_sample_radix<T>(s, a, n); });
            }
        }
    }

    void decode_frame_small(int n) {
        run_("other", 0, 0, [&] {
            launch_embed<T>(s, m->tok_in, n, (const T*)m->emb, (const T*)m->cbemb, m->c.dim, m->C, m->cb,
                            m->c.semantic_begin_id, m->c.semantic_end_id, m->c.scale_codebook_embeddings,
                            (T*)m->x, m->frame_slot);
        });
        slow_small(n);
        const KsbPlan kp = plan(m->sd, n);
        const void* hid = head_small(nullptr, true, n, kp.w2);
        frame_tail_small(n, true, true, hid);
        chain_flush();
        launch_finish(s, n, m->frame_slot, m->frame_pos, m->cols, m->C1, m->tok_in, m->ras, m->C1 * 10, m->C1,
                      1, m->sp);
    }

    void slow_layers(int R, const int* rslot, const int* rpos) {
        x_ss = false;
        for (int l = 0; l < m->sd.n_layer; ++l)
            block(m->sd, m->slow[l], R, rslot, rpos, -1, false, m->kc, m->vc, m->slot_stride,
                  (size_t)l * m->layer_stride, m->S, m->rope, m->x, m->h, m->xn);
        flush();
    }

    void head_and_hidden(const void* xlast, int n) {
        const fm_model_config& c = m->c;
        chain_flush();
        run_("norm", 0, 0, [&] {
            launch_rmsnorm<T>(s, (const T*)xlast, c.dim, (const T*)m->norm, c.dim, c.norm_eps, (T*)m->xnl,
                              c.dim, n);
        });
        linear(m->head_c, nullptr, nullptr, m->xnl, c.dim, n, m->Nhead, c.dim, nullptr, m->Nhead,
               nullptr, 0, m->logits, EPI_F32, "linear");
        const void* src = c.norm_fastlayer_input ? m->xnl : xlast;
        if (m->fproj_w)
            linear(m->fproj_w, nullptr, m->fproj_b, src, c.dim, n, c.fast_dim, c.dim, m->fx, c.fast_dim,
                   nullptr, 0, nullptr, EPI_STORE, "linear");
        else
            HIPCHK(hipMemcpyAsync(m->fx, src, (size_t)n * c.dim * E, hipMemcpyDeviceToDevice, s));
    }

    void fast_pass(int n, int cpos, bool with_head) {
        const fm_model_config& c = m->c;
        x_ss = false;
        for (int l = 0; l < m->fdm.n_layer; ++l)
            block(m->fdm, m->fast[l], n, m->frame_slot, nullptr, cpos, true, m->fkc, m->fvc,
                  m->fslot_stride, (size_t)l * m->flayer_stride, m->C, m->frope, m->fx, m->fh, m->fxn);
        flush();
        if (with_head) {
            run_("norm", 0, 0, [&] {
                launch_rmsnorm<T>(s, (const T*)m->fx, c.fast_dim, (const T*)m->fnorm, c.fast_dim,
                                  c.norm_eps, (T*)m->fxn, c.fast_dim, n);
            });
            linear(m->fout, nullptr, nullptr, m->fxn, c.fast_dim, n, m->cb, c.fast_dim, nullptr, m->cb,
                   nullptr, 0, m->flogits, EPI_F32, "linear");
        }
    }

    SampleArgs sargs(bool slow, int ras_enable, int c) {
        const fm_model_config& cc = m->c;
        SampleArgs a{};
        a.logits = slow ? m->logits : m->flogits;
        a.ldl = slow ? m->Nhead : m->cb;
        a.Nl = a.ldl;
        a.row_slot = m->frame_slot;
        a.sp = m->sp;
        a.ras = m->ras;
        a.ras_stride = m->C1 * 10;
        a.ras_enable = ras_enable;
        a.slow = slow;
        a.sb = cc.semantic_begin_id;
        a.se = cc.semantic_end_id;
// ... 354 lines not shown
            if (qi.q8) m->qmap[pk] = qi;
            const bool keep = row_keep(m, kv.first, (int)t.rows, (int)t.cols);
            if (keep) {
                void* rw = m->dalloc((size_t)t.rows * t.cols / 2, false);
                launch_pack_q4_rows(m->stream, (const uint8_t*)t.q, (int)t.rows, (int)t.cols, (uint32_t*)rw);
                HIPCHK(hipGetLastError());
                m->rowmajor[pk] = rw;
                m->rowsz[pk] = t.s;
                m->allocs.push_back(const_cast<void*>(t.s));
            }
            HIPCHK(hipStreamSynchronize(m->stream));
            HIPCHK(hipFree(t.q));
            if (!keep) HIPCHK(hipFree(const_cast<void*>(t.s)));
            t.q = nullptr;
            t.s = nullptr;
        } else if (m->quant) {
            m->qmap[pk] = fm_llm::QInfo{(const unsigned char*)pack_q8_dev(m, t.q, (int)t.rows, (int)t.cols), t.s};
            HIPCHK(hipStreamSynchronize(m->stream));
            if (row_keep(m, kv.first, (int)t.rows, (int)t.cols)) {
                m->rowmajor[pk] = t.q;
                m->allocs.push_back(t.q);
            } else {
                HIPCHK(hipFree(t.q));
            }
            t.q = nullptr;
        }
        HIPCHK(hipStreamSynchronize(m->stream));
        if (!m->quant && row_keep(m, kv.first, (int)t.rows, (int)t.cols)) {
            m->rowmajor[pk] = t.p;
            m->allocs.push_back(t.p);
        } else {
            HIPCHK(hipFree(t.p));
        }
        t.p = pk;
    }
    auto stack = [&](const std::string& pre, const StackDims& d, std::vector<LayerW>& out) {
        out.resize(d.n_layer);
        for (int i = 0; i < d.n_layer; ++i) {
            std::string p = pre + std::to_string(i) + ".";
            LayerW& L = out[i];
            L.wqkv = W(m, p + "attention.wqkv.weight");
            L.bqkv = Wopt(m, p + "attention.wqkv.bias");
            L.wo = W(m, p + "attention.wo.weight");
            L.bo = Wopt(m, p + "attention.wo.bias");
            L.qn = Wopt(m, p + "attention.q_norm.weight");
            L.kn = Wopt(m, p + "attention.k_norm.weight");
            L.w13 = pack_w13(m, p, d.inter, d.dim);
            L.w2 = W(m, p + "feed_forward.w2.weight");
            L.an = W(m, p + "attention_norm.weight");
            L.fn = W(m, p + "ffn_norm.weight");
            auto rm = [&](const void* pk) -> void* {
                auto it = m->rowmajor.find(pk);
                return it == m->rowmajor.end() ? nullptr : it->second;
            };
            L.wo_rm = rm(L.wo);
            L.w2_rm = rm(L.w2);
            L.wqkv_rm = rm(L.wqkv);
            L.w13_rm = rm(L.w13);
        }
    };
    stack("layers.", m->sd, m->slow);
    stack("fast_layers.", m->fdm, m->fast);
    {
        int32_t io[16];
        for (int c = 0; c < 16; ++c) io[c] = c - 1;
        m->fiota = (int32_t*)m->dalloc(sizeof(io), false);
        HIPCHK(hipMemcpy(m->fiota, io, sizeof(io), hipMemcpyHostToDevice));
    }
    if (m->prec == FM_PREC_BF16)
        m->fxt = (uint32_t*)m->dalloc((size_t)m->fdm.nh * m->fdm.hd * sizeof(uint32_t));
    m->row_ok = m->row_qkv_ok = m->row_w13_ok = true;
    for (auto* st : {&m->slow, &m->fast})
        for (const LayerW& L : *st) {
            m->row_ok = m->row_ok && L.wo_rm && L.w2_rm;
            m->row_qkv_ok = m->row_qkv_ok && L.wqkv_rm;
            m->row_w13_ok = m->row_w13_ok && L.w13_rm;
        }
    if (m->quant) {
        for (auto* st : {&m->slow, &m->fast})
            for (LayerW& L : *st) L.bqkv = L.bo = nullptr;
    }
    m->emb = W(m, "embeddings.weight");
    m->cbemb = W(m, "codebook_embeddings.weight");
    m->norm = W(m, "norm.weight");
    m->fproj_w = Wopt(m, "fast_project_in.weight");
    m->fproj_b = m->quant ? nullptr : Wopt(m, "fast_project_in.bias");
    m->femb = W(m, "fast_embeddings.weight");
    m->fnorm = W(m, "fast_norm.weight");
    m->fout = W(m, "fast_output.weight");
    {
        auto it = m->rowmajor.find(m->fout);
        m->fout_rm = it == m->rowmajor.end() ? nullptr : it->second;
    }
    const void* outw = c.tie_word_embeddings ? m->emb : W(m, "output.weight");
    m->nsem = c.semantic_end_id - c.semantic_begin_id + 1;
    m->Nhead = m->nsem + 1;
    FMCHECK(m->Nhead <= 8192, "constrained head wider than 8192 rows is not supported");
    const size_t rowb = (size_t)c.dim * m->esz;
    void* head_rm = m->dalloc((size_t)(m->Nhead + 15) / 16 * 16 * rowb);
    HIPCHK(hipMemcpyAsync(head_rm, (const char*)outw + (size_t)c.semantic_begin_id * rowb,
                          (size_t)m->nsem * rowb, hipMemcpyDeviceToDevice, m->stream));
    HIPCHK(hipMemcpyAsync((char*)head_rm + (size_t)m->nsem * rowb,
                          (const char*)outw + (size_t)c.im_end_id * rowb, rowb, hipMemcpyDeviceToDevice,
                          m->stream));
    m->head_c = pack_dev(m, head_rm, m->Nhead, c.dim);
    m->allocs.push_back(m->head_c);
    if (m->quant == FM_QUANT_INT4 && !c.tie_word_embeddings) {
        DTensor& o = m->w.at("output.weight");
        const size_t gb = (size_t)(c.dim / m->q4_gs) * 4;
        void* hq = nullptr;
        void* hs = nullptr;
        HIPCHK(hipMalloc(&hq, (size_t)(m->Nhead + 15) / 16 * 16 * c.dim));
        HIPCHK(hipMalloc(&hs, (size_t)(m->Nhead + 15) / 16 * 16 * gb));
        HIPCHK(hipMemcpyAsync(hq, (const char*)o.q + (size_t)c.semantic_begin_id * c.dim, (size_t)m->nsem * c.dim,
                              hipMemcpyDeviceToDevice, m->stream));
        HIPCHK(hipMemcpyAsync((char*)hq + (size_t)m->nsem * c.dim, (const char*)o.q + (size_t)c.im_end_id * c.dim,
                              c.dim, hipMemcpyDeviceToDevice, m->stream));
        HIPCHK(hipMemcpyAsync(hs, (const char*)o.s + (size_t)c.semantic_begin_id * gb, (size_t)m->nsem * gb,
                              hipMemcpyDeviceToDevice, m->stream));
        HIPCHK(hipMemcpyAsync((char*)hs + (size_t)m->nsem * gb, (const char*)o.s + (size_t)c.im_end_id * gb, gb,
                              hipMemcpyDeviceToDevice, m->stream));
        const fm_llm::QInfo qi = pack_q4_dev(m, hq, hs, m->Nhead, c.dim);
        if (qi.q8) m->qmap[m->head_c] = qi;
        HIPCHK(hipStreamSynchronize(m->stream));
        for (void* p : {hq, hs, o.q, o.s}) HIPCHK(hipFree(p));
        o.q = o.s = nullptr;
    } else if (m->quant && !c.tie_word_embeddings) {
        DTensor& o = m->w.at("output.weight");
        void* hq = m->dalloc((size_t)(m->Nhead + 15) / 16 * 16 * c.dim);
        HIPCHK(hipMemcpyAsync(hq, (const char*)o.q + (size_t)c.semantic_begin_id * c.dim, (size_t)m->nsem * c.dim,
                              hipMemcpyDeviceToDevice, m->stream));
        HIPCHK(hipMemcpyAsync((char*)hq + (size_t)m->nsem * c.dim, (const char*)o.q + (size_t)c.im_end_id * c.dim,
                              c.dim, hipMemcpyDeviceToDevice, m->stream));
        void* hs = m->dalloc((size_t)(m->Nhead + 15) / 16 * 16 * m->esz);
        HIPCHK(hipMemcpyAsync(hs, (const char*)o.s + (size_t)c.semantic_begin_id * m->esz, (size_t)m->nsem * m->esz,
                              hipMemcpyDeviceToDevice, m->stream));
        HIPCHK(hipMemcpyAsync((char*)hs + (size_t)m->nsem * m->esz, (const char*)o.s + (size_t)c.im_end_id * m->esz,
                              m->esz, hipMemcpyDeviceToDevice, m->stream));
        m->qmap[m->head_c] = fm_llm::QInfo{(const unsigned char*)pack_q8_dev(m, hq, m->Nhead, c.dim), hs};
        HIPCHK(hipStreamSynchronize(m->stream));
        HIPCHK(hipFree(o.q));
        o.q = nullptr;
    }
    const StackDims& d = m->sd;
    m->layer_stride = (size_t)d.nkv * m->S * d.hd;
    m->slot_stride = m->layer_stride * d.n_layer;
    m->kc = m->dalloc(m->slot_stride * m->max_slots * m->esz);
    m->vc = m->dalloc(m->slot_stride * m->max_slots * m->esz);
    const StackDims& f = m->fdm;
    m->flayer_stride = (size_t)f.nkv * m->C * f.hd;
    m->fslot_stride = m->flayer_stride * f.n_layer;
    m->fkc = m->dalloc(m->fslot_stride * m->max_slots * m->esz);
    m->fvc = m->dalloc(m->fslot_stride * m->max_slots * m->esz);
    auto rt = rope_table_host(m->S, d.hd, c.rope_base);
    m->rope = (float*)m->dalloc(rt.size() * 4, false);
    HIPCHK(hipMemcpy(m->rope, rt.data(), rt.size() * 4, hipMemcpyHostToDevice));
    auto frt = rope_table_host(m->C, f.hd, c.rope_base);
    m->frope = (float*)m->dalloc(frt.size() * 4, false);
    HIPCHK(hipMemcpy(m->frope, frt.data(), frt.size() * 4, hipMemcpyHostToDevice));
    const int R = m->Rmax = std::max(m->max_slots, PREFILL_CHUNK);
    const int dmax = std::max(c.dim, c.fast_dim);
    const int qkvmax = std::max(d.nqkv(), f.nqkv()), qmax = std::max(d.nq(), f.nq());
    const int imax = std::max(d.inter, f.inter);
    const size_t E = m->esz;
    m->x = m->dalloc((size_t)R * dmax * E);
    m->h = m->dalloc((size_t)R * dmax * E);
    m->xn = m->dalloc((size_t)R * dmax * E);
    m->qkv = m->dalloc((size_t)R * qkvmax * E);
    m->q = m->dalloc((size_t)R * qmax * E);
    m->att = m->dalloc((size_t)R * qmax * E);
    m->act = m->dalloc((size_t)R * imax * E);
    m->act2 = m->dalloc((size_t)R * 2 * imax * E);
    const int n = m->max_slots;
    m->xl = m->dalloc((size_t)n * dmax * E);
    m->plast = m->dalloc((size_t)n * dmax * E);
    m->xnl = m->dalloc((size_t)n * dmax * E);
    m->fx = m->dalloc((size_t)n * dmax * E);
    m->fh = m->dalloc((size_t)n * dmax * E);
    m->fxn = m->dalloc((size_t)n * dmax * E);
    m->x2 = m->dalloc((size_t)std::min(n, GEMV_MAX_ROWS) * dmax * E);
    m->fx2 = m->dalloc((size_t)std::min(n, GEMV_MAX_ROWS) * dmax * E);
    m->chain_cnt = (unsigned*)m->dalloc(GEMV_CHAIN_WORDS * sizeof(unsigned));
    m->chain_err = (int*)m->dalloc(16 * sizeof(int));
    HIPCHK(hipHostMalloc((void**)&m->h_chain_err, 16 * sizeof(int), hipHostMallocDefault));
    m->h_chain_err[0] = 0;
    m->maxsplit = FM_CEIL(m->S, ATTN_SPLIT);
    const int Rpart = std::max(m->max_slots, ATTN_PIECE);
    m->part = (float*)m->dalloc((size_t)Rpart * d.nh * std::max(m->maxsplit, FM_CEIL(m->S, 16)) * (d.hd + 2) * 4, false);
    m->attn_cnt = (int*)m->dalloc((size_t)R * d.nkv * sizeof(int));
    m->ssX = (float*)m->dalloc((size_t)(dmax / 16) * std::min(n, 32) * 4);
    m->ssH = (float*)m->dalloc((size_t)(dmax / 16) * std::min(n, 32) * 4);
    {
        const int maxn = std::max({m->Nhead, 2 * c.intermediate_size, 2 * c.fast_intermediate_size, qkvmax, dmax, m->cb});
        m->tickets = (int*)m->dalloc((size_t)(maxn / 16 + 16) * sizeof(int));
        m->fin_cnt = (int*)m->dalloc((size_t)std::max(m->max_slots, 64) * 2 * sizeof(int));
        m->fin_ss = (float*)m->dalloc((size_t)std::max(m->max_slots, 64) * 16 * sizeof(float));
        m->skpart_cap = 16ll << 20;
        m->skpart = (float*)m->dalloc((size_t)m->skpart_cap * sizeof(float), false);
    }
    HIPCHK(hipMemsetAsync(m->attn_cnt, 0, (size_t)R * d.nkv * sizeof(int), m->stream));
    m->slabA = (float*)m->dalloc((size_t)KSB_MAX * std::min(n, GEMV_MAX_ROWS) * dmax * 4);
    m->slabB = (float*)m->dalloc((size_t)KSB_MAX * std::min(n, GEMV_MAX_ROWS) * dmax * 4);
    if (n > GEMV_MAX_ROWS) {
        m->bsA = (float*)m->dalloc((size_t)BS_KPARTS * 32 * dmax * 4, false);
        m->bsB = (float*)m->dalloc((size_t)BS_KPARTS * 32 * dmax * 4, false);
        m->bsQ = (float*)m->dalloc((size_t)BS_KPARTS * 32 * std::max(m->sd.nqkv(), m->fdm.nqkv()) * 4, false);
    }
    m->logits = (float*)m->dalloc((size_t)n * m->Nhead * 4);
    m->flogits = (float*)m->dalloc((size_t)n * m->cb * 4);
    m->frame_slot = (int*)m->dalloc(n * 4);
    m->frame_pos = (int*)m->dalloc(n * 4);
    m->prow_slot = (int*)m->dalloc(PREFILL_CHUNK * 4);
    m->prow_pos = (int*)m->dalloc(PREFILL_CHUNK * 4);
    m->pfx_slots = (int*)m->dalloc((size_t)n * 4);
    m->tok_in = (int32_t*)m->dalloc((size_t)n * m->C1 * 4);
    m->cols = (int32_t*)m->dalloc((size_t)n * m->C1 * 4);
    m->ptok = (int32_t*)m->dalloc((size_t)PREFILL_CHUNK * m->C1 * 4);
    m->ras = (int32_t*)m->dalloc((size_t)n * m->C1 * 10 * 4);
    m->sp = (SlotParams*)m->dalloc(sizeof(SlotParams) * n);
    m->force_cols = (int32_t*)m->dalloc((size_t)n * m->C1 * 4);
    m->tap_slow = (float*)m->dalloc((size_t)n * m->Nhead * 4);
    m->tap_fast = (float*)m->dalloc((size_t)n * std::max(m->C - 1, 1) * m->cb * 4);
    m->host_force.assign(n, 0);
    HIPCHK(hipHostMalloc((void**)&m->h_cols, (size_t)2 * n * m->C1 * 4, hipHostMallocDefault));
    m->host_pos.assign(n, 0);
    m->host_step.assign(n, 0);
    HIPCHK(hipStreamSynchronize(m->stream));
    m->finalized = true;
}

template <typename F> static int with_prec(fm_llm* m, F&& f) {
    if (m->prec == FM_PREC_BF16) {
        Run<bf16_t> r(m);
        f(r);
        r.chain_flush();
    } else {
        Run<float> r(m);
        f(r);
        r.chain_flush();
    }
    return 0;
}

static void check_tokens(fm_llm* m, const int32_t* tok, int T) {
    const fm_model_config& c = m->c;
    for (int t = 0; t < T; ++t) {
        const int t0 = tok[t];
        FMCHECK(t0 >= 0 && t0 < c.vocab_size, "token id out of range: " + std::to_string(t0));
        for (int q = 0; q < m->C; ++q) {
            const int v = tok[(size_t)(q + 1) * T + t];
            FMCHECK(v >= 0 && v < m->cb, "codebook token out of range: " + std::to_string(v));
        }
    }
}

static void reset_slot(fm_llm* m, int slot, const fm_sampling* sp) {
    HIPCHK(hipMemsetAsync((char*)m->ras + (size_t)slot * m->C1 * 10 * 4, 0, (size_t)m->C1 * 10 * 4, m->stream));
    SlotParams p{};
    if (sp) {
        FMCHECK(sp->top_k >= 1, "top_k must be >= 1: got " + std::to_string(sp->top_k));
        p.temperature = sp->temperature;
        p.top_p = sp->top_p;
        p.top_k = sp->top_k;
        p.mask_im_end = sp->mask_im_end;
        p.seed = sp->seed;
    } else {
        p.temperature = 0.7f;
        p.top_p = 0.9f;
        p.top_k = 1;
    }
    p.step = 0;
    p.force = m->host_force[slot];
    HIPCHK(hipMemcpyAsync(m->sp + slot, &p, sizeof p, hipMemcpyHostToDevice, m->stream));
    HIPCHK(hipStreamSynchronize(m->stream));
    m->host_step[slot] = 0;
}

static void upload_frame_rows(fm_llm* m, const int32_t* slots, int n) {
    std::vector<int> s(slots, slots + n), p(n);
    if (s == m->uploaded_slots) return;
    for (int i = 0; i < n; ++i) p[i] = m->host_pos[s[i]];
    HIPCHK(hipMemcpyAsync(m->frame_slot, s.data(), (size_t)n * 4, hipMemcpyHostToDevice, m->stream));
    HIPCHK(hipMemcpyAsync(m->frame_pos, p.data(), (size_t)n * 4, hipMemcpyHostToDevice, m->stream));
    HIPCHK(hipStreamSynchronize(m->stream));
    m->uploaded_slots = s;
}

static void chain_err_async(fm_llm* m) {
    if (fm_tuning().gemv_chain || fm_tuning().fin_split > 1 ||
        (m->fxt && fm_tuning().fattn_wo))
        HIPCHK(hipMemcpyAsync(m->h_chain_err, m->chain_err, sizeof(int), hipMemcpyDeviceToHost, m->stream));
}
static void chain_err_check(fm_llm* m) {
    if (!m->h_chain_err || !m->h_chain_err[0]) return;
    m->h_chain_err[0] = 0;
    HIPCHK(hipMemset(m->chain_cnt, 0, GEMV_CHAIN_WORDS * sizeof(unsigned)));
    HIPCHK(hipMemset(m->chain_err, 0, 16 * sizeof(int)));
    if (m->fin_cnt) HIPCHK(hipMemset(m->fin_cnt, 0, (size_t)std::max(m->max_slots, 64) * 2 * sizeof(int)));
    throw FmError{FM_ERR_STATE,
                  "in-launch hand-off wait timed out (gemv chain / split finalize / fused fast "
                  "attention + wo; counters reset)"};
}

static void launch_frame(fm_llm* m, int n) {
    if (m->use_graph && !m->prof.on) {
        auto it = m->graphs.find(n);
        if (it == m->graphs.end()) {
            hipGraph_t g;
            HIPCHK(hipStreamBeginCapture(m->stream, hipStreamCaptureModeThreadLocal));
            with_prec(m, [&](auto& r) { r.decode_frame(n); });
            HIPCHK(hipStreamEndCapture(m->stream, &g));
            hipGraphExec_t ge;
            HIPCHK(hipGraphInstantiate(&ge, g, nullptr, nullptr, 0));
            HIPCHK(hipGraphDestroy(g));
            it = m->graphs.emplace(n, ge).first;
        }
        HIPCHK(hipGraphLaunch(it->second, m->stream));
    } else {
        with_prec(m, [&](auto& r) { r.decode_frame(n); });
    }
}

extern "C" {

int fm_llm_open(const fm_model_config* cfg, int device, int precision, int max_slots, fm_llm** out) {
    return fm_guard([&] {
        FMCHECK(cfg && out, "null argument");
        FMCHECK(precision == FM_PREC_BF16 || precision == FM_PREC_FP32, "bad precision");
        FMCHECK(max_slots >= 1 && max_slots <= 4096, "bad max_slots");
        const fm_model_config& c = *cfg;
        FMCHECK(c.dim % 32 == 0 && c.fast_dim % 32 == 0, "dims must be multiples of 32");
        FMCHECK(c.intermediate_size % 32 == 0 && c.fast_intermediate_size % 32 == 0,
                "intermediate sizes must be multiples of 32");
        FMCHECK((c.n_head * c.head_dim) % 32 == 0 && (c.fast_n_head * c.fast_head_dim) % 32 == 0,
                "n_head*head_dim must be a multiple of 32");
        FMCHECK(c.head_dim % 8 == 0 && c.head_dim <= 256 && c.fast_head_dim <= 256, "bad head_dim");
        FMCHECK(c.n_head % c.n_local_heads == 0 && c.fast_n_head % c.fast_n_local_heads == 0, "bad GQA");
        FMCHECK(c.num_codebooks >= 1 && c.num_codebooks <= 63, "bad num_codebooks");
        FMCHECK(c.codebook_size <= 8192, "codebook_size > 8192 unsupported");
        FMCHECK(c.im_end_id >= 0 && c.im_end_id < c.vocab_size, "im_end_id must be set");
        FMCHECK(c.semantic_begin_id >= 0 && c.semantic_end_id < c.vocab_size &&
                    c.semantic_begin_id <= c.semantic_end_id,
                "bad semantic id range");
        int ndev = fm_device_count();
        FMCHECK(ndev > 0, "no HIP device visible");
        FMCHECK(device >= 0 && device < ndev, "bad device index");
        HIPCHK(hipSetDevice(device));
        std::unique_ptr<fm_llm> m(new fm_llm());
        m->c = c;
        m->device = device;
        m->prec = precision;
        m->esz = precision == FM_PREC_BF16 ? 2 : 4;
        m->max_slots = max_slots;
        m->S = (c.max_seq_len + 7) / 8 * 8;
        m->C = c.num_codebooks;
        m->C1 = c.num_codebooks + 1;
        m->cb = c.codebook_size;
        HIPCHK(hipStreamCreateWithFlags(&m->stream, hipStreamNonBlocking));
        const char* g = getenv("FISHMI_GRAPH");
        m->use_graph = !(g && g[0] == '0');
        build_inventory(m.get());
        *out = m.release();
    });
}

int fm_llm_set_quant_int4(fm_llm* m, int groupsize) {
    return fm_guard([&] {
        FMCHECK(m && (groupsize == 32 || groupsize == 64 || groupsize == 128 || groupsize == 256),
                "int4: groupsize must be 32, 64, 128 or 256 (WeightOnlyInt4QuantHandler, quantize.py:366)");
        FMCHECK(!m->finalized, "weights are frozen after finalize");
        for (auto& kv : m->w) FMCHECK(!kv.second.set, "set the quantization mode before any tensor");
        FMCHECK(m->quant == FM_QUANT_NONE, "quantization mode already set");
        FMCHECK(m->prec == FM_PREC_BF16, "int4: bf16 precision only (the reference quantizes the bf16 weights)");
        const fm_model_config& c = m->c;
        FMCHECK(!c.qkv_bias && !c.o_bias && !c.fast_qkv_bias && !c.fast_o_bias,
                "int4: the linears must be bias-free (quantize.py:371)");
        for (auto& kv : m->w) {
            if (!is_quant_linear(kv.first)) continue;
            FMCHECK(kv.second.cols % groupsize == 0, "int4: in_features must be a multiple of the group size: " + kv.first);
            FMCHECK(m->w.find(base_of(kv.first) + ".bias") == m->w.end(),
                    "int4: the linears must be bias-free (quantize.py:371): " + kv.first);
        }
        m->quant = FM_QUANT_INT4;
        m->q4_gs = groupsize;
    });
}

int fm_llm_set_quant(fm_llm* m, int mode) {
    if (mode == FM_QUANT_INT4) return fm_llm_set_quant_int4(m, 128);
    return fm_guard([&] {
        FMCHECK(m && (mode == FM_QUANT_NONE || mode == FM_QUANT_INT8), "bad arguments");
        FMCHECK(!m->finalized, "weights are frozen after finalize");
        for (auto& kv : m->w) FMCHECK(!kv.second.set, "set the quantization mode before any tensor");
        if (mode == m->quant) return;
        FMCHECK(m->quant == FM_QUANT_NONE, "quantization mode already set");
        m->quant = mode;
        std::vector<std::pair<std::string, int64_t>> add;
        for (auto& kv : m->w) {
            if (!is_quant_linear(kv.first)) continue;
            FMCHECK(kv.second.cols % 64 == 0, "int8 weights need in_features % 64 == 0: " + kv.first);
            add.emplace_back(base_of(kv.first) + ".scales", kv.second.rows);
            auto b = m->w.find(base_of(kv.first) + ".bias");
            if (b != m->w.end()) b->second.optional = true;
        }
        for (auto& a : add) {
            add_t(m, a.first, 1, a.second);
            m->w[a.first].optional = true;
        }
    });
}

int fm_llm_set_tensor(fm_llm* m, const char* name, const void* data, int dtype, int64_t numel) {
    return fm_guard([&] {
        FMCHECK(m && name && data, "null argument");
        FMCHECK(!m->finalized, "weights are frozen after finalize");
        HIPCHK(hipSetDevice(m->device));
        if (dtype == FM_DT_I8) {
            FMCHECK(m->quant == FM_QUANT_INT8 && is_quant_linear(name), std::string("int8 data for ") + name +
                                                                             " needs fm_llm_set_quant(INT8) and a linear weight");
            auto it = m->w.find(name);
            FMCHECK(it != m->w.end() && it->second.numel == numel, std::string("unknown tensor or wrong numel: ") + name);
            DTensor& t = it->second;
            FMCHECK(!t.set, std::string("tensor set twice: ") + name);
            const size_t bytes = (size_t)(t.rows + 15) / 16 * 16 * t.cols;
            HIPCHK(hipMalloc(&t.q, bytes));
            HIPCHK(hipMemsetAsync(t.q, 0, bytes, m->stream));
            HIPCHK(hipMemcpyAsync(t.q, data, (size_t)numel, hipMemcpyHostToDevice, m->stream));
            HIPCHK(hipStreamSynchronize(m->stream));
            t.set = true;
            return;
        }
        DTensor& t = tensor_for(m, name, numel);
        const size_t sb = dtype == FM_DT_BF16 ? 2 : 4;
        void* tmp = nullptr;
        HIPCHK(hipMalloc(&tmp, (size_t)numel * sb));
        HIPCHK(hipMemcpy(tmp, data, (size_t)numel * sb, hipMemcpyHostToDevice));
        if (m->prec == FM_PREC_BF16)
            launch_convert<bf16_t>(m->stream, tmp, dtype == FM_DT_BF16, numel, (bf16_t*)t.p);
        else
            launch_convert<float>(m->stream, tmp, dtype == FM_DT_BF16, numel, (float*)t.p);
        HIPCHK(hipStreamSynchronize(m->stream));
        HIPCHK(hipFree(tmp));
        t.set = true;
    });
}

int fm_llm_synth_tensor(fm_llm* m, const char* name, int64_t numel, uint64_t seed, float center,
                        int log2_half) {
    return fm_guard([&] {
        FMCHECK(m && name, "null argument");
        FMCHECK(!m->finalized, "weights are frozen after finalize");
        HIPCHK(hipSetDevice(m->device));
        DTensor& t = tensor_for(m, name, numel);
        if (m->prec == FM_PREC_BF16)
            launch_synth<bf16_t>(m->stream, (bf16_t*)t.p, numel, seed, fnv1a32(name), center, log2_half);
        else
            launch_synth<float>(m->stream, (float*)t.p, numel, seed, fnv1a32(name), center, log2_half);
        HIPCHK(hipGetLastError());
        t.set = true;
    });
}

int fm_llm_finalize(fm_llm* m) {
    return fm_guard([&] {
        FMCHECK(m, "null handle");
        HIPCHK(hipSetDevice(m->device));
        finalize(m);
    });
}

static void do_prefill(fm_llm* m, int slot, const int32_t* tokens, int T, const fm_sampling* sp,
                       int32_t* first_col, int pos0 = 0) {
    FMCHECK(slot >= 0 && slot < m->max_slots, "bad slot");
    FMCHECK(T >= 1 && pos0 >= 0 && pos0 + T < m->c.max_seq_len, "prompt must end before max_seq_len");
    FMCHECK(pos0 <= m->host_pos[slot], "prefix reuse past the slot's cached positions");
    check_tokens(m, tokens, T);
    reset_slot(m, slot, sp);
    const int32_t one = slot;
    m->uploaded_slots.clear();
    HIPCHK(hipMemcpyAsync(m->frame_slot, &one, 4, hipMemcpyHostToDevice, m->stream));
    with_prec(m, [&](auto& r) {
        const void* last = r.prefill_slow(slot, tokens, T, pos0);
        const void* hid = r.head_small(last, false, 1, 1);
        r.frame_tail_small(1, false, true, hid);
    });
    int pos = pos0 + T - 1;
    HIPCHK(hipMemcpyAsync(m->frame_pos, &pos, 4, hipMemcpyHostToDevice, m->stream));
    launch_finish(m->stream, 1, m->frame_slot, m->frame_pos, m->cols, m->C1, m->tok_in, m->ras,
                  m->C1 * 10, m->C1, 0, m->sp);
    HIPCHK(hipMemcpyAsync(m->h_cols, m->cols, (size_t)m->C1 * 4, hipMemcpyDeviceToHost, m->stream));
    HIPCHK(hipStreamSynchronize(m->stream));
    m->prof.collect();
    m->host_pos[slot] = pos0 + T;
    m->host_step[slot] = 1;
    m->uploaded_slots.clear();
    if (first_col) memcpy(first_col, m->h_cols, (size_t)m->C1 * 4);
}

static void do_prefill_batch(fm_llm* m, int n, const int32_t* slots, const int32_t* tokens, const int32_t* T,
                             const fm_sampling* sps, int32_t* first_cols, const int32_t* pos0 = nullptr) {
    FMCHECK(n >= 1 && n <= m->max_slots, "bad request count");
    std::vector<const int32_t*> tk(n);
    size_t off = 0;
    for (int i = 0; i < n; ++i) {
        FMCHECK(slots[i] >= 0 && slots[i] < m->max_slots, "bad slot");
        for (int j = 0; j < i; ++j) FMCHECK(slots[j] != slots[i], "duplicate slot");
        const int p0 = pos0 ? pos0[i] : 0;
        FMCHECK(T[i] >= 1 && p0 >= 0 && (int64_t)p0 + T[i] < m->c.max_seq_len, "prompt must end before max_seq_len");
        FMCHECK(p0 <= m->host_pos[slots[i]], "prefix reuse past the slot's cached positions");
        tk[i] = tokens + off;
        check_tokens(m, tk[i], T[i]);
        off += (size_t)m->C1 * T[i];
    }
    for (int i = 0; i < n; ++i) reset_slot(m, slots[i], sps ? sps + i : nullptr);
    m->uploaded_slots.clear();
    HIPCHK(hipMemcpyAsync(m->frame_slot, slots, (size_t)n * 4, hipMemcpyHostToDevice, m->stream));
    with_prec(m, [&](auto& r) {
        r.prefill_multi(n, slots, tk.data(), T, pos0);
        if (n <= GEMV_MAX_ROWS) {
            const void* hid = r.head_small(m->plast, false, n, 1);
            r.frame_tail_small(n, false, true, hid);
        } else {
            r.bs_frame = true;
            r.head_and_hidden(m->plast, n);
            r.frame_tail(n, false, true);
            r.bs_frame = false;
        }
    });
    std::vector<int> pos(n);
    for (int i = 0; i < n; ++i) pos[i] = (pos0 ? pos0[i] : 0) + T[i] - 1;
    HIPCHK(hipMemcpyAsync(m->frame_pos, pos.data(), (size_t)n * 4, hipMemcpyHostToDevice, m->stream));
    launch_finish(m->stream, n, m->frame_slot, m->frame_pos, m->cols, m->C1, m->tok_in, m->ras, m->C1 * 10,
                  m->C1, 0, m->sp);
    HIPCHK(hipMemcpyAsync(m->h_cols, m->cols, (size_t)n * m->C1 * 4, hipMemcpyDeviceToHost, m->stream));
    HIPCHK(hipStreamSynchronize(m->stream));
    m->prof.collect();
    for (int i = 0; i < n; ++i) {
        m->host_pos[slots[i]] = (pos0 ? pos0[i] : 0) + T[i];
        m->host_step[slots[i]] = 1;
    }
    m->uploaded_slots.clear();
    if (first_cols) memcpy(first_cols, m->h_cols, (size_t)n * m->C1 * 4);
}

int fm_llm_prefill_batch(fm_llm* m, int n, const int32_t* slots, const int32_t* tokens, const int32_t* T,
                         const fm_sampling* sp, int32_t* first_cols) {
    return fm_guard([&] {
        FMCHECK(m && slots && tokens && T, "null argument");
        HIPCHK(hipSetDevice(m->device));
        finalize(m);
        do_prefill_batch(m, n, slots, tokens, T, sp, first_cols);
    });
}

int fm_llm_prefill_batch_at(fm_llm* m, int n, const int32_t* slots, const int32_t* tokens, const int32_t* T,
                            const int32_t* pos0, const fm_sampling* sp, int32_t* first_cols) {
    return fm_guard([&] {
        FMCHECK(m && slots && tokens && T && pos0, "null argument");
        HIPCHK(hipSetDevice(m->device));
        finalize(m);
        do_prefill_batch(m, n, slots, tokens, T, sp, first_cols, pos0);
    });
}

static void prefix_copy(fm_llm* m, const fm_llm::Prefix& e, const int32_t* slots, int n, bool to_store) {
    const StackDims& d = m->sd;
    HIPCHK(hipMemcpyAsync(m->pfx_slots, slots, (size_t)n * 4, hipMemcpyHostToDevice, m->stream));
    KvPrefixArgs a{};
    a.kc = (char*)m->kc;
    a.vc = (char*)m->vc;
    a.store = (char*)e.buf;
    a.slots = m->pfx_slots;
    a.slot_stride_b = m->slot_stride * m->esz;
    a.layer_stride_b = m->layer_stride * m->esz;
    a.head_stride_b = (size_t)m->S * d.hd * m->esz;
    a.run_bytes = (size_t)e.npos * d.hd * m->esz;
    a.nkv = d.nkv;
    a.to_store = to_store ? 1 : 0;
    launch_kv_prefix_copy(m->stream, a, d.n_layer, n);
    HIPCHK(hipGetLastError());
    HIPCHK(hipStreamSynchronize(m->stream));
}

static fm_llm::Prefix& prefix_of(fm_llm* m, int id) {
    auto it = m->prefixes.find(id);
    FMCHECK(it != m->prefixes.end(), "unknown or dropped prefix id " + std::to_string(id));
    return it->second;
}

int fm_llm_prefix_save(fm_llm* m, int slot, int npos, int* prefix_id) {
    return fm_guard([&] {
        FMCHECK(m && prefix_id, "null argument");
        FMCHECK(m->finalized, "prefix_save before any prefill");
        HIPCHK(hipSetDevice(m->device));
        FMCHECK(slot >= 0 && slot < m->max_slots, "bad slot");
        FMCHECK(npos >= 1 && npos <= m->host_pos[slot],
                "prefix_save: npos " + std::to_string(npos) + " outside [1, " + std::to_string(m->host_pos[slot]) +
                    "], the slot's cached positions");
        fm_llm::Prefix e;
        e.npos = npos;
        e.bytes = (size_t)m->sd.n_layer * 2 * m->sd.nkv * npos * m->sd.hd * m->esz;
        const hipError_t err = hipMalloc(&e.buf, e.bytes);
        if (err != hipSuccess) {
            (void)hipGetLastError();
            throw FmError{FM_ERR_OOM, "prefix_save: hipMalloc(" + std::to_string(e.bytes) + ") failed: " +
                                          hipGetErrorString(err)};
        }
        try {
            const int32_t one = slot;
            prefix_copy(m, e, &one, 1, true);
        } catch (...) {
            (void)hipFree(e.buf);
            throw;
        }
        const int id = m->next_prefix_id++;
        m->prefixes[id] = e;
        *prefix_id = id;
    });
}

int fm_llm_prefix_load(fm_llm* m, int prefix_id, const int32_t* slots, int n) {
    return fm_guard([&] {
        FMCHECK(m && slots, "null argument");
        FMCHECK(m->finalized, "prefix_load before any prefill");
        HIPCHK(hipSetDevice(m->device));
        const fm_llm::Prefix& e = prefix_of(m, prefix_id);
        FMCHECK(n >= 1 && n <= m->max_slots, "bad slot count");
        for (int i = 0; i < n; ++i) {
            FMCHECK(slots[i] >= 0 && slots[i] < m->max_slots, "bad slot");
            for (int j = 0; j < i; ++j) FMCHECK(slots[j] != slots[i], "duplicate slot");
        }
        FMCHECK(e.npos <= m->S, "prefix longer than the slot cache");
        prefix_copy(m, e, slots, n, false);
        for (int i = 0; i < n; ++i) {
            m->host_pos[slots[i]] = e.npos;
            m->host_step[slots[i]] = 0;
        }
        m->uploaded_slots.clear();
    });
}

int fm_llm_prefix_drop(fm_llm* m, int prefix_id) {
    return fm_guard([&] {
        FMCHECK(m, "null handle");
        HIPCHK(hipSetDevice(m->device));
        const fm_llm::Prefix e = prefix_of(m, prefix_id);
        HIPCHK(hipStreamSynchronize(m->stream));
        m->prefixes.erase(prefix_id);
        HIPCHK(hipFree(e.buf));
    });
}

int fm_llm_prefix_info(fm_llm* m, int prefix_id, int* npos, int64_t* bytes) {
    return fm_guard([&] {
        FMCHECK(m, "null handle");
        const fm_llm::Prefix& e = prefix_of(m, prefix_id);
        if (npos) *npos = e.npos;
        if (bytes) *bytes = (int64_t)e.bytes;
    });
}

int fm_llm_prefill(fm_llm* m, int slot, const int32_t* tokens, int T, const fm_sampling* sp,
                   int32_t* first_col) {
    return fm_guard([&] {
        FMCHECK(m && tokens, "null argument");
        HIPCHK(hipSetDevice(m->device));
        finalize(m);
        do_prefill(m, slot, tokens, T, sp, first_col);
    });
}

int fm_llm_prefill_at(fm_llm* m, int slot, const int32_t* suffix, int T, int pos0, const fm_sampling* sp,
                      int32_t* first_col) {
    return fm_guard([&] {
        FMCHECK(m && suffix, "null argument");
        HIPCHK(hipSetDevice(m->device));
        finalize(m);
        do_prefill(m, slot, suffix, T, sp, first_col, pos0);
    });
}

int fm_llm_decode(fm_llm* m, const int32_t* slots, int n, int32_t* cols) {
    return fm_guard([&] {
        FMCHECK(m && slots && n >= 1 && n <= m->max_slots, "bad arguments");
        FMCHECK(m->finalized, "call fm_llm_prefill first");
        HIPCHK(hipSetDevice(m->device));
        for (int i = 0; i < n; ++i) {
            FMCHECK(slots[i] >= 0 && slots[i] < m->max_slots, "bad slot");
            FMCHECK(m->host_pos[slots[i]] < m->c.max_seq_len, "slot reached max_seq_len");
        }
        upload_frame_rows(m, slots, n);
        launch_frame(m, n);
        HIPCHK(hipMemcpyAsync(m->h_cols, m->cols, (size_t)n * m->C1 * 4, hipMemcpyDeviceToHost, m->stream));
        chain_err_async(m);
        HIPCHK(hipStreamSynchronize(m->stream));
        chain_err_check(m);
        m->prof.collect();
        for (int i = 0; i < n; ++i) {
            m->host_pos[slots[i]]++;
            m->host_step[slots[i]]++;
        }
        if (cols) memcpy(cols, m->h_cols, (size_t)n * m->C1 * 4);
    });
}

int fm_llm_decode_frames(fm_llm* m, const int32_t* slots, int n, int nframes, int32_t* cols) {
    return fm_guard([&] {
        FMCHECK(m && slots && cols && n >= 1 && n <= m->max_slots && nframes >= 0, "bad arguments");
        FMCHECK(m->finalized, "call fm_llm_prefill first");
        HIPCHK(hipSetDevice(m->device));
        for (int i = 0; i < n; ++i) {
            FMCHECK(slots[i] >= 0 && slots[i] < m->max_slots, "bad slot");
            for (int j = 0; j < i; ++j) FMCHECK(slots[j] != slots[i], "duplicate slot");
            FMCHECK(m->host_pos[slots[i]] + nframes <= m->c.max_seq_len, "slot would pass max_seq_len");
        }
        if (nframes == 0) return;
        const size_t per = (size_t)n * m->C1;
        if (m->h_hist_n < per * nframes) {
            if (m->h_hist) HIPCHK(hipHostFree(m->h_hist));
            m->h_hist = nullptr;
            m->h_hist_n = 0;
            HIPCHK(hipHostMalloc((void**)&m->h_hist, per * nframes * 4, hipHostMallocDefault));
            m->h_hist_n = per * nframes;
        }
        upload_frame_rows(m, slots, n);
        for (int k = 0; k < nframes; ++k) {
            launch_frame(m, n);
            HIPCHK(hipMemcpyAsync(m->h_hist + per * k, m->cols, per * 4, hipMemcpyDeviceToHost, m->stream));
        }
        chain_err_async(m);
        HIPCHK(hipStreamSynchronize(m->stream));
        chain_err_check(m);
        m->prof.collect();
        for (int i = 0; i < n; ++i) {
            m->host_pos[slots[i]] += nframes;
            m->host_step[slots[i]] += nframes;
        }
        memcpy(cols, m->h_hist, per * nframes * 4);
    });
}

static void do_generate(fm_llm* m, int slot, const int32_t* prompt, int T, int pos0, int max_new,
                        const fm_sampling* sp, int32_t* out, int* n_out) {
        FMCHECK(m && prompt && out && n_out, "null argument");
        HIPCHK(hipSetDevice(m->device));
        finalize(m);
        const fm_model_config& c = m->c;
        if (max_new <= 0 || pos0 + T + max_new > c.max_seq_len) max_new = c.max_seq_len - pos0 - T;
        FMCHECK(max_new >= 1, "prompt leaves no room to generate");
        const int C1 = m->C1;
        int32_t col[64];
        do_prefill(m, slot, prompt, T, sp, col, pos0);
        for (int q = 0; q < C1; ++q) out[(size_t)q * max_new] = col[q];
        int n = 1;
        upload_frame_rows(m, &slot, 1);
        hipEvent_t ev[2];
        HIPCHK(hipEventCreateWithFlags(&ev[0], hipEventDisableTiming));
        HIPCHK(hipEventCreateWithFlags(&ev[1], hipEventDisableTiming));
        auto issue = [&](int k) {
            launch_frame(m, 1);
            HIPCHK(hipMemcpyAsync(m->h_cols + (size_t)(k & 1) * m->max_slots * C1, m->cols, (size_t)C1 * 4,
                                  hipMemcpyDeviceToHost, m->stream));
            HIPCHK(hipEventRecord(ev[k & 1], m->stream));
        };
        const int steps = max_new - 1;
        int issued = 0;
        if (steps > 0) issue(issued++);
        for (int k = 0; k < steps; ++k) {
            if (issued < steps && issued <= k + 1) issue(issued++);
            HIPCHK(hipEventSynchronize(ev[k & 1]));
            const int32_t* hc = m->h_cols + (size_t)(k & 1) * m->max_slots * C1;
            for (int q = 0; q < C1; ++q) out[(size_t)q * max_new + n] = hc[q];
            n++;
            if (hc[0] == c.im_end_id) break;
        }
        chain_err_async(m);
        HIPCHK(hipStreamSynchronize(m->stream));
        chain_err_check(m);
        m->prof.collect();
        (void)hipEventDestroy(ev[0]);
        (void)hipEventDestroy(ev[1]);
        m->host_pos[slot] = pos0 + T + issued;
        m->host_step[slot] = 1 + issued;
        m->uploaded_slots.clear();
        *n_out = n;
}

int fm_llm_generate(fm_llm* m, int slot, const int32_t* prompt, int T, int max_new, const fm_sampling* sp,
                    int32_t* out, int* n_out) {
    return fm_guard([&] { do_generate(m, slot, prompt, T, 0, max_new, sp, out, n_out); });
}

int fm_llm_generate_at(fm_llm* m, int slot, const int32_t* suffix, int T, int pos0, int max_new,
                       const fm_sampling* sp, int32_t* out, int* n_out) {
    return fm_guard([&] { do_generate(m, slot, suffix, T, pos0, max_new, sp, out, n_out); });
}

int fm_llm_slot_pos(fm_llm* m, int slot, int* pos) {
    return fm_guard([&] {
        FMCHECK(m && pos && slot >= 0 && slot < m->max_slots, "bad arguments");
        *pos = m->host_pos[slot];
    });
}

int fm_llm_teacher_step(fm_llm* m, int slot, const int32_t* x, int S, int pos0, const int32_t* next_col,
                        float* slow_logits, float* hidden, float* fast_logits) {
    return fm_guard([&] {
        FMCHECK(m && x && S >= 1, "bad arguments");
        HIPCHK(hipSetDevice(m->device));
        finalize(m);
        FMCHECK(slot >= 0 && slot < m->max_slots, "bad slot");
        FMCHECK(pos0 + S <= m->c.max_seq_len, "beyond max_seq_len");
        check_tokens(m, x, S);
        if (next_col)
            for (int q = 1; q < m->C1; ++q)
                FMCHECK(next_col[q] >= 0 && next_col[q] < m->cb, "next_col codebook token out of range");
        if (pos0 == 0) reset_slot(m, slot, nullptr);
        const fm_model_config& c = m->c;
        const int32_t one = slot;
        HIPCHK(hipMemcpyAsync(m->frame_slot, &one, 4, hipMemcpyHostToDevice, m->stream));
        m->uploaded_slots.clear();
        std::vector<float> lg(m->Nhead);
        with_prec(m, [&](auto& r) {
            const void* last = r.prefill_slow(slot, x, S, pos0);
            const void* hid = r.head_small(last, false, 1, 1);
                HIPCHK(hipMemcpyAsync(lg.data(), m->logits, (size_t)m->Nhead * 4, hipMemcpyDeviceToHost, m->stream));
            if (hidden) {
                std::vector<uint8_t> hb((size_t)c.fast_dim * m->esz);
                HIPCHK(hipMemcpyAsync(hb.data(), hid, hb.size(), hipMemcpyDeviceToHost, m->stream));
                HIPCHK(hipStreamSynchronize(m->stream));
                for (int i = 0; i < c.fast_dim; ++i) {
                    if (m->esz == 2) {
                        uint32_t u = ((uint32_t)((uint16_t*)hb.data())[i]) << 16;
                        memcpy(&hidden[i], &u, 4);
                    } else {
                        hidden[i] = ((float*)hb.data())[i];
                    }
                }
            }
            if (next_col) {
                HIPCHK(hipMemcpyAsync(m->cols, next_col, (size_t)m->C1 * 4, hipMemcpyHostToDevice, m->stream));
                r.fast_small(1, 0, false, hid);
                for (int cc = 1; cc < m->C; ++cc) {
                    r.fast_small(1, cc, true, hid);
                                if (fast_logits)
                        HIPCHK(hipMemcpyAsync(fast_logits + (size_t)(cc - 1) * m->cb, m->flogits, (size_t)m->cb * 4,
                                              hipMemcpyDeviceToHost, m->stream));
                }
            }
        });
        HIPCHK(hipStreamSynchronize(m->stream));
        m->prof.collect();
        m->host_pos[slot] = pos0 + S;
        if (slow_logits) {
            for (int i = 0; i < c.vocab_size; ++i) slow_logits[i] = -INFINITY;
            for (int i = 0; i < m->nsem; ++i) slow_logits[c.semantic_begin_id + i] = lg[i];
            slow_logits[c.im_end_id] = lg[m->nsem];
        }
    });
}

int64_t fm_llm_frame_bytes(fm_llm* m, int n, int pos) {
    if (!m) return -1;
    const fm_model_config& c = m->c;
    const int64_t E = (int64_t)m->esz;
    const bool q4 = m->quant == FM_QUANT_INT4 && m->q4_gs % 128 == 0;
    auto lin = [&](int64_t N, int64_t K) -> int64_t {
        if (q4 && K % 128 == 0) return N * K / 2 + N * (K / 128) * 4;
        if (m->quant == FM_QUANT_INT8) return N * K + N * E;
        return N * K * E;
    };
    auto stack_bytes = [&](const StackDims& d) {
        int64_t per = lin(d.nqkv(), d.dim) + lin(d.dim, d.nq()) + lin(2LL * d.inter, d.dim) + lin(d.dim, d.inter) +
                      2LL * d.dim * E;
        if (d.qk_norm) per += 2LL * d.hd * E;
        return per * d.n_layer;
    };
    int64_t b = stack_bytes(m->sd) + (c.tie_word_embeddings ? (int64_t)m->Nhead * c.dim * E : lin(m->Nhead, c.dim)) +
                (int64_t)c.dim * E;
    b += (int64_t)m->C * stack_bytes(m->fdm) + (int64_t)(m->C - 1) * (lin(m->cb, c.fast_dim) + (int64_t)c.fast_dim * E);
    if (m->fproj_w) b += lin(c.fast_dim, c.dim);
    int64_t per_stream = 2LL * m->sd.n_layer * m->sd.nkv * m->sd.hd * E * (pos + 1);
    for (int cc = 0; cc < m->C; ++cc) per_stream += 2LL * m->fdm.n_layer * m->fdm.nkv * m->fdm.hd * E * (cc + 1);
    per_stream += (int64_t)(m->C + 1) * c.dim * E + (int64_t)(m->C - 1) * c.fast_dim * E;
    return b + per_stream * n;
}

int fm_llm_profile(fm_llm* m, int enable) {
    return fm_guard([&] {
        FMCHECK(m, "null handle");
        m->prof.on = enable != 0;
        if (enable) m->prof.acc.clear();
    });
}

int fm_llm_profile_read(fm_llm* m, const char* cls, double* ms, int64_t* launches, int64_t* bytes) {
    return fm_guard([&] {
        FMCHECK(m && cls, "null argument");
        auto it = m->prof.acc.find(cls);
        Profiler::Acc a = it == m->prof.acc.end() ? Profiler::Acc{} : it->second;
        if (ms) *ms = a.ms;
        if (launches) *launches = a.n;
        if (bytes) *bytes = a.bytes;
    });
}

int fm_tune(const char* key, int value) {
    return fm_guard([&] {
        FMCHECK(key, "null key");
        FmTuning& t = fm_tuning();
        const std::string k = key;
        if (k == "gemv_nt") {
            t.gemv_nt = value != 0;
        } else if (k == "gemv_u") {
            FMCHECK(value == 2 || value == 4 || value == 8, "gemv_u must be 2, 4 or 8");
            t.gemv_u = value;
        } else if (k == "sampler_fast") {
            t.sampler_fast = value != 0;
        } else if (k == "attn_cap") {
            FMCHECK(value == 0 || (value >= 16 && value % 16 == 0), "attn_cap must be 0 or a multiple of 16");
            t.attn_cap = value;
        } else if (k == "prefill_attn") {
            t.prefill_attn = value != 0;
        } else if (k == "prefix_vec") {
            t.prefix_vec = value != 0;
        } else if (k == "prompt_qkv_slab") {
            t.prompt_qkv_slab = value != 0;
        } else if (k == "prompt_unroll") {
            t.prompt_unroll = value != 0;
        } else if (k == "prompt_fin") {
            t.prompt_fin = value != 0;
        } else if (k == "prompt_swiglu") {
            t.prompt_swiglu = value != 0;
        } else if (k == "prompt_skinny") {
            t.prompt_skinny = value != 0;
        } else if (k == "prompt_skinny_blocks") {
            FMCHECK(value >= 1, "prompt_skinny_blocks must be >= 1");
            t.prompt_skinny_blocks = value;
        } else if (k == "prompt_ks_tiles") {
            FMCHECK(value >= 1, "prompt_ks_tiles must be >= 1");
            t.prompt_ks_tiles = value;
        } else if (k == "prompt_ks_max") {
            FMCHECK(value == 1 || value == 2 || value == 4 || value == 8, "prompt_ks_max must be 1, 2, 4 or 8");
            t.prompt_ks_max = value;
        } else if (k == "prompt_gemm") {
            t.prompt_gemm = value != 0;
        } else if (k == "conv2") {
            t.conv2 = value != 0;
        } else if (k == "conv_splitk") {
            t.conv_splitk = value != 0;
        } else if (k == "codec_norm") {
            t.codec_norm = value != 0;
        } else if (k == "codec_rope") {
            t.codec_rope = value != 0;
        } else if (k == "codec_swiglu") {
            t.codec_swiglu = value != 0;
        } else if (k == "codec_fuse") {
            t.codec_fuse = value != 0;
        } else if (k == "resunit_enc") {
            t.resunit_enc = value != 0;
        } else if (k == "resunit_384") {
            t.resunit_384 = value != 0;
        } else if (k == "resunit_cfg") {
            FMCHECK(value >= 0 && value <= 2, "resunit_cfg must be 0..2");
            t.resunit_cfg = value;
        } else if (k == "attn_wo") {
            t.attn_wo = value != 0;
        } else if (k == "gemv_wpb") {
            FMCHECK(value == 4 || value == 8, "gemv_wpb must be 4 or 8");
            t.gemv_wpb = value;
        } else if (k == "ksb_blocks") {
            FMCHECK(value >= 1, "ksb_blocks must be >= 1");
            t.ksb_blocks = value;
        } else if (k == "attn_cap_batched") {
            FMCHECK(value == 0 || (value >= 16 && value % 16 == 0), "attn_cap_batched must be 0 or a multiple of 16");
            t.attn_cap_batched = value;
        } else if (k == "linear_u32") {
            FMCHECK(value == 4 || value == 8, "linear_u32 must be 4 or 8");
            t.linear_u32 = value;
        } else if (k == "batched_fused_attn") {
            t.batched_fused_attn = value != 0;
        } else if (k == "linear_fill") {
            FMCHECK(value >= 0, "linear_fill must be >= 0");
            t.linear_fill = value;
        } else if (k == "ksb_balance") {
            t.ksb_balance = value != 0;
        } else if (k == "attn3") {
            t.attn3 = value != 0;
        } else if (k == "attn_fd") {
            t.attn_fd = value != 0;
        } else if (k == "fd_min") {
            FMCHECK(value >= 16 && value % 16 == 0, "fd_min must be a multiple of 16");
            t.fd_min = value;
        } else if (k == "chain_max") {
            FMCHECK(value >= 2 && value <= GEMV_CHAIN_MAX, "chain_max must be 2..4");
            t.chain_max = value;
        } else if (k == "chain_sleep") {
            FMCHECK(value == 1 || value == 4 || value == 16, "chain_sleep must be 1, 4 or 16");
            t.chain_sleep = value;
        } else if (k == "gemv_chain") {
            t.gemv_chain = value != 0;
        } else if (k == "fd_nw") {
            FMCHECK(value == 4 || value == 8 || value == 16, "fd_nw must be 4, 8 or 16");
            t.fd_nw = value;
        } else if (k == "fin_ksb") {
            FMCHECK(value >= 0 && value <= KSB_MAX, "fin_ksb must be in [0, KSB_MAX]");
            t.fin_ksb = value;
        } else if (k == "fd_nw_batched") {
            FMCHECK(value == 4 || value == 8 || value == 16, "fd_nw_batched must be 4, 8 or 16");
            t.fd_nw_batched = value;
        } else if (k == "fd_min16") {
            FMCHECK(value >= 16 && value % 16 == 0, "fd_min16 must be a multiple of 16");
            t.fd_min16 = value;
        } else if (k == "fd_min_batched") {
            FMCHECK(value >= 16 && value % 16 == 0, "fd_min_batched must be a multiple of 16");
            t.fd_min_batched = value;
        } else if (k == "gemv_dummy") {
            FMCHECK(value >= 0 && value <= 2, "gemv_dummy must be 0, 1 or 2");
            t.gemv_dummy = value;
        } else if (k == "bs_dummy") {
            FMCHECK(value >= 0 && value <= 2, "bs_dummy must be 0, 1 or 2");
            t.bs_dummy = value;
        } else if (k == "bs_qkv_slab") {
            t.bs_qkv_slab = value != 0;
        } else if (k == "fast_tail") {
            t.fast_tail = value != 0;
        } else if (k == "fkv_prefetch") {
            t.fkv_prefetch = value != 0;
        } else if (k == "kv_prefetch") {
            t.kv_prefetch = value != 0;
        } else if (k == "bstream") {
            t.bstream = value != 0;
        } else if (k == "bstream_kparts") {
            FMCHECK(value == 0 || value == 1 || value == 2 || value == 4 || value == 8, "bstream_kparts must be 0, 1, 2, 4 or 8");
            t.bstream_kparts = value;
        } else if (k == "bstream_acc") {
            t.bstream_acc = value;
        } else if (k == "bstream_chain") {
            t.bstream_chain = value;
        } else if (k == "bstream_nw") {
            FMCHECK(value >= 0 && value <= 16, "bstream_nw must be in [0, 16]");
            t.bstream_nw = value;
        } else if (k == "bs_xfirst") {
            t.bs_xfirst = value != 0;
        } else if (k == "bs_vec_epi") {
            t.bs_vec_epi = value != 0;
        } else if (k == "bsacc_kparts") {
            FMCHECK(value == 0 || value == 1 || value == 2 || value == 4 || value == 8, "bsacc_kparts must be 0, 1, 2, 4 or 8");
            t.bsacc_kparts = value;
        } else if (k == "q_u") {
            FMCHECK(value == 2 || value == 4 || value == 8 || value == 16, "q_u must be 2, 4, 8 or 16");
            t.q_u = value;
        } else if (k == "fin8") {
            t.fin8 = value != 0;
        } else if (k == "fin_split") {
            FMCHECK(value >= 0 && value <= 16, "fin_split must be 0..16");
            t.fin_split = value;
        } else if (k == "int4_stream") {
            t.int4_stream = value != 0;
        } else if (k == "fw_delay") {
            FMCHECK(value >= 0 && value <= 1000, "fw_delay must be 0..1000 (10-ns ticks)");
            t.fw_delay = value;
        } else if (k == "fw_prio") {
            t.fw_prio = value != 0;
        } else if (k == "fw_cheap") {
            t.fw_cheap = value != 0;
        } else if (k == "fattn_wo") {
            t.fattn_wo = value != 0;
        } else if (k == "sampler_kth") {
            t.sampler_kth = value != 0;
        } else if (k == "row_qkv_rp") {
            FMCHECK(value == 4 || value == 8 || value == 16, "row_qkv_rp must be 4, 8 or 16");
            t.row_qkv_rp = value;
        } else if (k == "rowgemv_q4") {
            FMCHECK(value >= 0 && value <= 31, "rowgemv_q4 must be 0..31");
            t.rowgemv_q4 = value;
        } else if (k == "row_copies") {
            t.row_copies = value != 0;
        } else if (k == "rowgemv") {
            FMCHECK(value >= 0 && value <= 31, "rowgemv must be 0..31 (bit 0 wo / w2, bit 1 wqkv, bit 2 w1 || w3, bit 3 fast head, bit 4 first-layer wqkv)");
            t.rowgemv = value;
        } else if (k == "rmsnorm_block") {
            t.rmsnorm_block = value != 0;
        } else if (k == "debug_ts") {
            if (t.dbg) HIPCHK(hipFree(t.dbg));
            t.dbg = nullptr;
            if (value) {
                HIPCHK(hipMalloc(&t.dbg, (8 + 8 * (1 << 20)) * sizeof(unsigned long long)));
                HIPCHK(hipMemset(t.dbg, 0, 8 * sizeof(unsigned long long)));
            }
        } else {
            FMCHECK(false, "unknown tuning key: " + k);
        }
    });
}

int fm_debug_ts_read(unsigned long long* out, int64_t max_records, int64_t* n_records) {
    return fm_guard([&] {
        FMCHECK(out && n_records, "null argument");
        const FmTuning& t = fm_tuning();
        FMCHECK(t.dbg, "debug_ts is not armed");
        HIPCHK(hipDeviceSynchronize());
        unsigned long long n = 0;
        HIPCHK(hipMemcpy(&n, t.dbg, sizeof n, hipMemcpyDeviceToHost));
        n = std::min<unsigned long long>(n, 1ull << 20);
        n = std::min<unsigned long long>(n, (unsigned long long)max_records);
        HIPCHK(hipMemcpy(out, t.dbg + 8, n * 8 * sizeof(unsigned long long), hipMemcpyDeviceToHost));
        *n_records = (int64_t)n;
    });
}

int fm_llm_kernel_bench(fm_llm* m, const char* cls, int reps, double* avg_us, int64_t* launches,
                        int64_t* bytes) {
    return fm_guard([&] {
        FMCHECK(m && cls && reps >= 1, "bad arguments");
        FMCHECK(m->finalized && !m->uploaded_slots.empty(), "decode a frame first");
        HIPCHK(hipSetDevice(m->device));
        const int n = (int)m->uploaded_slots.size();
        const bool was_on = m->prof.on;
        m->prof.on = false;
        m->prof.rec.clear();
        m->prof.rec_bytes.clear();
        m->prof.rec_cls = cls;
        with_prec(m, [&](auto& r) { r.decode_frame(n); });
        m->prof.rec_cls.clear();
        m->prof.on = was_on;
        HIPCHK(hipStreamSynchronize(m->stream));
        for (int s : m->uploaded_slots) {
            m->host_pos[s]++;
            m->host_step[s]++;
        }
        std::vector<std::function<void()>> rec;
        rec.swap(m->prof.rec);
        FMCHECK(!rec.empty(), std::string("no launches of class ") + cls + " in a decode frame");
        int64_t b = 0;
        for (int64_t x : m->prof.rec_bytes) b += x;
        hipGraph_t g;
        HIPCHK(hipStreamBeginCapture(m->stream, hipStreamCaptureModeThreadLocal));
        for (auto& f : rec) f();
        HIPCHK(hipStreamEndCapture(m->stream, &g));
        hipGraphExec_t ge;
        HIPCHK(hipGraphInstantiate(&ge, g, nullptr, nullptr, 0));
        HIPCHK(hipGraphDestroy(g));
        hipEvent_t ea, eb;
        HIPCHK(hipEventCreate(&ea));
        HIPCHK(hipEventCreate(&eb));
        HIPCHK(hipGraphLaunch(ge, m->stream));
        HIPCHK(hipEventRecord(ea, m->stream));
        for (int i = 0; i < reps; ++i) HIPCHK(hipGraphLaunch(ge, m->stream));
        HIPCHK(hipEventRecord(eb, m->stream));
        HIPCHK(hipEventSynchronize(eb));
        float ms = 0;
        HIPCHK(hipEventElapsedTime(&ms, ea, eb));
        (void)hipEventDestroy(ea);
        (void)hipEventDestroy(eb);
        (void)hipGraphExecDestroy(ge);
        if (avg_us) *avg_us = (double)ms * 1e3 / ((double)reps * rec.size());
        if (launches) *launches = (int64_t)rec.size();
        if (bytes) *bytes = b;
    });
}

int fm_llm_force(fm_llm* m, int slot, const int32_t* col) {
    return fm_guard([&] {
        FMCHECK(m, "null handle");
        HIPCHK(hipSetDevice(m->device));
        finalize(m);
        FMCHECK(slot >= 0 && slot < m->max_slots, "bad slot");
        const int on = col != nullptr;
        if (on) {
            const fm_model_config& c = m->c;
            FMCHECK(col[0] >= 0 && col[0] < c.vocab_size, "forced token outside the vocabulary");
            for (int q = 1; q < m->C1; ++q)
                FMCHECK(col[q] >= 0 && col[q] < m->cb, "forced codebook token out of range");
            HIPCHK(hipMemcpyAsync(m->force_cols + (size_t)slot * m->C1, col, (size_t)m->C1 * 4,
                                  hipMemcpyHostToDevice, m->stream));
        }
        m->host_force[slot] = on;
        HIPCHK(hipMemcpyAsync(&m->sp[slot].force, &m->host_force[slot], sizeof(int), hipMemcpyHostToDevice,
                              m->stream));
        HIPCHK(hipStreamSynchronize(m->stream));
    });
}

int fm_llm_read_logits(fm_llm* m, int slot, float* slow_logits, float* fast_logits) {
    return fm_guard([&] {
        FMCHECK(m && m->finalized, "null or unfinalized handle");
        FMCHECK(slot >= 0 && slot < m->max_slots, "bad slot");
        HIPCHK(hipSetDevice(m->device));
        const fm_model_config& c = m->c;
        std::vector<float> lg(m->Nhead);
        HIPCHK(hipMemcpyAsync(lg.data(), m->tap_slow + (size_t)slot * m->Nhead, (size_t)m->Nhead * 4,
                              hipMemcpyDeviceToHost, m->stream));
        if (fast_logits && m->C > 1)
            HIPCHK(hipMemcpyAsync(fast_logits, m->tap_fast + (size_t)slot * (m->C - 1) * m->cb,
                                  (size_t)(m->C - 1) * m->cb * 4, hipMemcpyDeviceToHost, m->stream));
        HIPCHK(hipStreamSynchronize(m->stream));
        if (slow_logits) {
            for (int i = 0; i < c.vocab_size; ++i) slow_logits[i] = -INFINITY;
            for (int i = 0; i < m->nsem; ++i) slow_logits[c.semantic_begin_id + i] = lg[i];
            slow_logits[c.im_end_id] = lg[m->nsem];
        }
    });
}

int fm_llm_use_graph(fm_llm* m, int enable) {
    return fm_guard([&] {
        FMCHECK(m, "null handle");
        m->use_graph = enable != 0;
        for (auto& g : m->graphs) (void)hipGraphExecDestroy(g.second);
        m->graphs.clear();
    });
}

int fm_llm_debug_vec(fm_llm* m, const char* name, int index, float* out, int64_t n) {
    return fm_guard([&] {
        FMCHECK(m && m->finalized && name && out && n > 0, "bad arguments");
        HIPCHK(hipSetDevice(m->device));
        HIPCHK(hipStreamSynchronize(m->stream));
        const std::string k = name;
        void* p = k == "qkv" ? m->qkv : k == "att" ? m->att : k == "fh" ? m->fh : k == "act" ? m->act
                : k == "fx" ? m->fx : k == "fx2" ? m->fx2 : k == "xl" ? m->xl : k == "xnl" ? m->xnl : nullptr;
        if (k == "kc" || k == "vc") {
            FMCHECK(index >= 0 && index < m->sd.n_layer, "layer out of range");
            FMCHECK(n <= (int64_t)m->layer_stride, "n past the layer's cache");
            p = (char*)(k == "kc" ? m->kc : m->vc) + (size_t)index * m->layer_stride * m->esz;
        }
        FMCHECK(p, "unknown buffer: " + k);
        if (m->esz == 4) {
            HIPCHK(hipMemcpy(out, p, (size_t)n * 4, hipMemcpyDeviceToHost));
        } else {
            std::vector<uint16_t> v((size_t)n);
            HIPCHK(hipMemcpy(v.data(), p, (size_t)n * 2, hipMemcpyDeviceToHost));
            for (int64_t i = 0; i < n; ++i) {
                const uint32_t u = (uint32_t)v[(size_t)i] << 16;
                memcpy(out + i, &u, 4);
            }
        }
    });
}

int fm_llm_close(fm_llm* m) {
    return fm_guard([&] { delete m; });
}

}
```

### fish-speech_amd/csrc/fm_rowgemv.hip

```cpp
#include "fm_common.h"
#include "fm_kernels.h"
#include "fm_runtime.h"
#include <type_traits>

typedef __attribute__((ext_vector_type(2))) uint32_t u32x2_t;
typedef __attribute__((ext_vector_type(4))) __bf16 bf16x4_t;

__device__ __forceinline__ float dot4(u32x2_t w, u32x2_t x, float acc) {
    const bf16x4_t wb = __builtin_bit_cast(bf16x4_t, w), xb = __builtin_bit_cast(bf16x4_t, x);
    acc = __builtin_amdgcn_fdot2_f32_bf16(__builtin_shufflevector(wb, wb, 0, 1), __builtin_shufflevector(xb, xb, 0, 1),
                                          acc, false);
    acc = __builtin_amdgcn_fdot2_f32_bf16(__builtin_shufflevector(wb, wb, 2, 3), __builtin_shufflevector(xb, xb, 2, 3),
                                          acc, false);
    return acc;
}
__device__ __forceinline__ float lo16(uint32_t w) { return __uint_as_float(w << 16); }
__device__ __forceinline__ float hi16(uint32_t w) { return __uint_as_float(w & 0xffff0000u); }
__device__ __forceinline__ float dot8r(u32x4_t w, u32x4_t x, float acc) {
    const bf16x8_t wb = __builtin_bit_cast(bf16x8_t, w), xb = __builtin_bit_cast(bf16x8_t, x);
    acc = __builtin_amdgcn_fdot2_f32_bf16(__builtin_shufflevector(wb, wb, 0, 1), __builtin_shufflevector(xb, xb, 0, 1),
                                          acc, false);
    acc = __builtin_amdgcn_fdot2_f32_bf16(__builtin_shufflevector(wb, wb, 2, 3), __builtin_shufflevector(xb, xb, 2, 3),
                                          acc, false);
    acc = __builtin_amdgcn_fdot2_f32_bf16(__builtin_shufflevector(wb, wb, 4, 5), __builtin_shufflevector(xb, xb, 4, 5),
// ... 39 lines not shown
        const int32_t iv = a.xidx[a.xcol];
        xi = iv < 0 ? 0 : (iv >= a.xrows ? a.xrows - 1 : iv);
    }
    bf16_t rv = 0;
    if constexpr (FIN) rv = a.res[(size_t)ri * a.ldr + er];
    const bf16_t bv = *(a.bias ? a.bias + er : a.X);
    bf16_t sv = 0;
    if constexpr (QM == 1) sv = a.wscale[er];
    const XV* xp = reinterpret_cast<const XV*>(a.X + (size_t)xi * a.ldx) + (size_t)wa * 64 + lane;
    const XV* gp = reinterpret_cast<const XV*>(PRENORM ? a.nw : a.X) + (size_t)wa * 64 + lane;
    XV xv[U], gv[PRENORM ? U : 1];
    if constexpr (!TX) {
#pragma unroll
        for (int u = 0; u < U; ++u) {
            const int j = (u < last ? u : last) * 64;
            xv[u] = xp[j];
            if constexpr (PRENORM) gv[u] = gp[j];
        }
    }
    constexpr int PF = 2;
    const bool pf_on = EPI == 0 && a.pf_kc != nullptr;
    int pf_s = 0, pf_p = 0;
    if constexpr (EPI == 0) {
        pf_s = *(pf_on ? a.pf_slot : reinterpret_cast<const int32_t*>(a.X));
        pf_p = *(pf_on ? a.pf_pos : reinterpret_cast<const int32_t*>(a.X));
    }
    asm volatile("" ::: "memory");
    constexpr int WU = QM == 2 ? 1 : U, WR = QM == 2 ? 1 : RP;
    constexpr int QU = QM == 2 ? U : 1, QR = QM == 2 ? RP : 1;
    u32x2_t wv[WU][WR];
    uint32_t w4[QU][QR], szv[QU][QR];
    if constexpr (QM == 2) {
        const size_t rw = (size_t)(a.K >> 3);
        const int ng = a.K / a.gs;
        const uint32_t* wp = a.Wq4 + (size_t)n0 * rw + (size_t)wa * 64 + lane;
#pragma unroll
        for (int u = 0; u < U; ++u) {
            const int jc = u < last ? u : last;
#pragma unroll
            for (int r = 0; r < RP; ++r) {
                w4[u][r] = __builtin_nontemporal_load(wp + r * rw + jc * 64);
                szv[u][r] = a.wsz[(size_t)(n0 + r) * ng + ((wa + jc) * 512 + lane * 8) / a.gs];
            }
        }
    } else {
        const unsigned char* wb = QM ? reinterpret_cast<const unsigned char*>(a.Wq) : reinterpret_cast<const unsigned char*>(a.W);
        const size_t rowb = (size_t)a.K * (QM ? 1 : 2);
        const u32x2_t* wp = reinterpret_cast<const u32x2_t*>(wb + (size_t)n0 * rowb) + (size_t)wa * 64 + lane;
        const size_t rs8 = rowb / 8;
#pragma unroll
        for (int u = 0; u < U; ++u) {
            const int j = (u < last ? u : last) * 64;
#pragma unroll
            for (int r = 0; r < RP; ++r) wv[u][r] = __builtin_nontemporal_load(wp + r * rs8 + j);
        }
    }
    asm volatile("" ::: "memory");
    if constexpr (TX) {
        const __amdgpu_buffer_rsrc_t xr = __builtin_amdgcn_make_buffer_rsrc((void*)xt, (short)0, a.K * 4, 0x00020000);
        u32x4_t xw[U][EPL / 4];
        for (unsigned it = 0;; ++it) {
#pragma unroll
            for (int u = 0; u < U; ++u) {
                const int jc = u < last ? u : last;
#pragma unroll
                for (int q = 0; q < EPL / 4; ++q)
                    xw[u][q] = __builtin_amdgcn_raw_buffer_load_b128(xr, ((wa + jc) * R::CE + EPL * lane + 4 * q) * 4, 0, 16);
            }
            bool ok = true;
#pragma unroll
            for (int u = 0; u < U; ++u)
#pragma unroll
                for (int q = 0; q < EPL / 4; ++q)
#pragma unroll
                    for (int e = 0; e < 4; ++e) ok = ok && ((xw[u][q][e] & 0xffffu) == gen);
            if (__all(ok)) break;
            if (it >= (1u << 14)) {
                if (lane == 0) __hip_atomic_store(err, 1, __ATOMIC_RELAXED, __HIP_MEMORY_SCOPE_AGENT);
                break;
            }
            __builtin_amdgcn_s_sleep(1);
        }
#pragma unroll
        for (int u = 0; u < U; ++u)
#pragma unroll
            for (int h = 0; h < NW; ++h) {
                const uint32_t w0 = xw[u][(2 * h) >> 2][(2 * h) & 3], w1 = xw[u][(2 * h + 1) >> 2][(2 * h + 1) & 3];
                xv[u][h] = (w0 >> 16) | (w1 & 0xffff0000u);
            }
    }
    float pfw[PF];
    if constexpr (EPI == 0) {
        const char* kcb = reinterpret_cast<const char*>(pf_on ? a.pf_kc : a.X);
        const long long dv = pf_on ? reinterpret_cast<const char*>(a.pf_vc) - kcb : 0;
        const int nkv = pf_on ? a.pf_nkv : 1;
        const int b = blockIdx.x, h = b % nkv, jb = b / nkv, nb = ((int)gridDim.x - 1 - h) / nkv + 1;
        const int spr = pf_on ? a.pf_hd * 2 / 64 : 1;
        const int np = pf_on ? pf_p + 1 : 0, total = 2 * np * spr;
        const long long base = pf_on ? (long long)pf_s * (long long)a.pf_slot_stride + (long long)a.pf_layer_off +
                                           (long long)h * a.pf_S * a.pf_hd
                                     : 0;
#pragma unroll
        for (int q = 0; q < PF; ++q) {
            const int i = (jb + nb * q) * 256 + (int)threadIdx.x;
            const bool ok = i < total;
            const int ii = ok ? i : 0, row = ii / spr, sec = ii - row * spr;
            const bool isv = row >= np;
            const long long off = (isv ? dv : 0) + 2 * (base + (long long)(isv ? row - np : row) * a.pf_hd) + sec * 64;
            pfw[q] = *reinterpret_cast<const float*>(kcb + (ok ? off : 0));
        }
    }
    if constexpr (PRENORM) {
        float sl = 0.f;
#pragma unroll
        for (int u = 0; u < U; ++u) {
            if (u < nmy) {
#pragma unroll
                for (int h = 0; h < NW; ++h) {
                    const float e0 = lo16(xv[u][h]), e1 = hi16(xv[u][h]);
                    sl += e0 * e0 + e1 * e1;
                }
            }
        }
        sl = wave_sum(sl);
        if (lane == 0) red[4 * RP + wave] = sl;
        lds_barrier();
        const float tot = ((red[4 * RP] + red[4 * RP + 1]) + red[4 * RP + 2]) + red[4 * RP + 3];
        const float rs = 1.0f / sqrtf(tot / (float)a.K + a.eps);
#pragma unroll
        for (int u = 0; u < U; ++u) {
            XV o;
#pragma unroll
            for (int h = 0; h < NW; ++h) {
                const float y0 = bfround(bfround(lo16(xv[u][h]) * rs) * lo16(gv[u][h]));
                const float y1 = bfround(bfround(hi16(xv[u][h]) * rs) * hi16(gv[u][h]));
                o[h] = (uint32_t)f2bf(y0) | ((uint32_t)f2bf(y1) << 16);
            }
            xv[u] = o;
        }
    }
    float acc[RP];
#pragma unroll
    for (int r = 0; r < RP; ++r) acc[r] = 0.f;
    float xs = 0.f;
#pragma unroll
    for (int u = 0; u < U; ++u) {
        if (u < nmy) {
            if constexpr (QM == 0) {
#pragma unroll
                for (int r = 0; r < RP; ++r) acc[r] = dot4(wv[u][r], xv[u], acc[r]);
            } else if constexpr (QM == 2) {
                const u32x4_t ones = {0x3F803F80u, 0x3F803F80u, 0x3F803F80u, 0x3F803F80u};
                const float xl = dot8r(ones, xv[u], 0.f);
#pragma unroll
                for (int r = 0; r < RP; ++r) {
                    const uint32_t w = w4[u][r];
                    u32x4_t A;
#pragma unroll
                    for (int p = 0; p < 4; ++p) A[p] = ((w >> (4 * p)) & 0x000F000Fu) | 0x43004300u;
                    const float B = dot8r(A, xv[u], 0.f);
                    const float sc = lo16(szv[u][r]), zr = hi16(szv[u][r]);
                    acc[r] = fmaf(sc, B, acc[r]);
                    acc[r] = fmaf(zr - 136.f * sc, xl, acc[r]);
                }
            } else {
                float xf[8];
#pragma unroll
                for (int h = 0; h < 4; ++h) {
                    xf[2 * h] = lo16(xv[u][h]);
                    xf[2 * h + 1] = hi16(xv[u][h]);
                }
                xs += ((xf[0] + xf[1]) + (xf[2] + xf[3])) + ((xf[4] + xf[5]) + (xf[6] + xf[7]));
#pragma unroll
                for (int r = 0; r < RP; ++r) {
                    const uint32_t c0 = wv[u][r][0] ^ 0x80808080u, c1 = wv[u][r][1] ^ 0x80808080u;
                    float t = acc[r];
#pragma unroll
                    for (int e = 0; e < 4; ++e) t = fmaf((float)((c0 >> (8 * e)) & 0xffu), xf[e], t);
#pragma unroll
                    for (int e = 0; e < 4; ++e) t = fmaf((float)((c1 >> (8 * e)) & 0xffu), xf[4 + e], t);
                    acc[r] = t;
                }
            }
        }
    }
    if constexpr (EPI == 0) {
#pragma unroll
        for (int q = 0; q < PF; ++q) asm volatile("" ::"v"(pfw[q]));
    }
    const unsigned long long ts1 = a.dbg ? __builtin_amdgcn_s_memrealtime() : 0;
#pragma unroll
    for (int r = 0; r < RP; ++r) {
        const float v = wave_sum(acc[r]);
        if (lane == 0) red[wave * RP + r] = v;
    }
    if constexpr (QM == 1) {
        const float v = wave_sum(xs);
        if (lane == 0) red[4 * RP + 4 + wave] = v;
    }
    __syncthreads();
    if ((int)threadIdx.x < RP) {
        const int t = threadIdx.x;
        float v = ((red[t] + red[RP + t]) + red[2 * RP + t]) + red[3 * RP + t];
        if constexpr (QM == 1) {
            const float xt = ((red[4 * RP + 4] + red[4 * RP + 5]) + red[4 * RP + 6]) + red[4 * RP + 7];
            v = bfround(bfround(v - 128.f * xt) * bf2f(sv));
        }
        if (a.bias) v += bf2f(bv);
        if constexpr (FIN) {
            a.res_out[er] = f2bf(bfround(bf2f(rv) + bfround(v)));
        } else if constexpr (EPI == 3) {
            a.Yf[er] = bfround(v);
        } else if constexpr (EPI == 2) {
            const float up = __shfl_down(v, RP / 2, 64);
            if (t < RP / 2) {
                const float g = bfround(v);
                a.Y[blockIdx.x * (RP / 2) + t] = f2bf(bfround(g / (1.0f + expf(-g))) * bfround(up));
            }
        } else {
            a.Y[er] = f2bf(v);
        }
    }
    if (a.dbg && threadIdx.x == 0) {
        const unsigned long long t[7] = {ts0, ts1, __builtin_amdgcn_s_memrealtime(), 0, 0, 0, 0};
        dbg_record(a.dbg, TX ? 0xFFF8u : 0xFFFAu, (unsigned)blk, t);
    }
}

template <int U, int RP, bool PRENORM, int EPI, bool G, int QM>
__global__ __launch_bounds__(256) __attribute__((amdgpu_waves_per_eu(RP == 2 ? 5 : 3)))
void rowgemv_kernel(RowGemvArgs a) {
    rowgemv_body<U, RP, PRENORM, EPI, G, QM, false>(a, blockIdx.x, nullptr, 0u, nullptr);
}

int rowgemv_u(int K, int qm) {
    const int ce = qm ? 512 : 256;
    if (K <= 0 || K % ce) return 0;
    const int need = (K / ce + 3) / 4;
    for (int u : {2, 3, 4, 5, 6, 8, 10, 12})
        if (need <= u) return u;
    return 0;
}

template <int RP, bool PRENORM, int EPI, int QM>
static void rowgemv_go(hipStream_t s, const RowGemvArgs& a, int U) {
    const dim3 grid(a.N / RP), block(256);
    auto go = [&](void (*plain)(RowGemvArgs), void (*gathered)(RowGemvArgs)) {
        ((EPI == 1 ? a.residx != nullptr : a.xidx != nullptr) ? gathered : plain)<<<grid, block, 0, s>>>(a);
    };
#define RG(u) go(rowgemv_kernel<u, RP, PRENORM, EPI, false, QM>, rowgemv_kernel<u, RP, PRENORM, EPI, true, QM>)
    switch (U) {
        case 2: RG(2); break;
        case 3: RG(3); break;
        case 4: RG(4); break;
        case 5: RG(5); break;
        case 6: RG(6); break;
        case 8: RG(8); break;
        case 10: RG(10); break;
        default: RG(12); break;
    }
#undef RG
}

void launch_rowgemv(hipStream_t s, const RowGemvArgs& a0, int kind) {
    RowGemvArgs a = a0;
    a.dbg = fm_tuning().dbg;
    if (!a.ldx) a.ldx = a.K;
    const int qm = a.Wq4 ? 2 : (a.Wq ? 1 : 0);
    const int U = rowgemv_u(a.K, qm);
    FMCHECK(U > 0 && a.X &&
                (qm == 2 ? (a.wsz && a.gs > 0 && a.gs % 8 == 0 && a.K % a.gs == 0 && !a.bias)
                         : (qm == 1 ? (a.Wq && a.wscale && !a.bias) : a.W != nullptr)),
            "row GEMV: K a whole number of chunks (256 k, int8 / int4 512 k), at most 48 per wave; operands set");
    if (kind == ROWGEMV_FIN) {
        FMCHECK(a.N % 2 == 0 && a.res && a.res_out, "row GEMV (fin): N even, residual rows set");
        if (qm == 2) rowgemv_go<2, false, 1, 2>(s, a, U);
        else if (qm == 1) rowgemv_go<2, false, 1, 1>(s, a, U);
        else rowgemv_go<2, false, 1, 0>(s, a, U);
    } else if (kind == ROWGEMV_NORM_F32) {
        FMCHECK(a.N % 8 == 0 && a.nw && a.Yf && U <= 8 && !a.xidx, "row GEMV (norm, f32): N % 8 == 0, norm weight and output set");
        if (qm == 2) rowgemv_go<8, true, 3, 2>(s, a, U);
        else if (qm == 1) rowgemv_go<8, true, 3, 1>(s, a, U);
        else rowgemv_go<8, true, 3, 0>(s, a, U);
    } else if (kind == ROWGEMV_NORM_SWIGLU) {
        FMCHECK(a.N % 8 == 0 && a.nw && a.Y && U <= 8 && !a.bias,
                "row GEMV (norm, swiglu): N % 8 == 0 (4 + 4 interleaved rows), norm weight and output set");
        if (qm == 2) rowgemv_go<8, true, 2, 2>(s, a, U);
        else if (qm == 1) rowgemv_go<8, true, 2, 1>(s, a, U);
        else rowgemv_go<8, true, 2, 0>(s, a, U);
    } else {
        FMCHECK(kind == ROWGEMV_NORM_STORE && a.N % 8 == 0 && a.nw && a.Y && U <= 8,
                "row GEMV (norm, store): N % 8 == 0, norm weight and output set");
        if (qm == 2) rowgemv_go<8, true, 0, 2>(s, a, U);
        else if (qm == 1) rowgemv_go<8, true, 0, 1>(s, a, U);
        else if (fm_tuning().row_qkv_rp == 4) rowgemv_go<4, true, 0, 0>(s, a, U);
        else if (fm_tuning().row_qkv_rp == 16) rowgemv_go<16, true, 0, 0>(s, a, U);
        else rowgemv_go<8, true, 0, 0>(s, a, U);
    }
}

constexpr int FW_MAXJ = 15;
constexpr int FW_MAXHD = 128;

template <int U, bool G, int QM>
__global__ __launch_bounds__(256) __attribute__((amdgpu_waves_per_eu(6)))
void fattn_wo_kernel(FattnWoArgs A) {
    __shared__ __attribute__((aligned(16))) bf16_t kvs[2 * FW_MAXJ * FW_MAXHD];
    __shared__ float red[8];
    const FastFusedArgs<bf16_t>& at = A.at;
    const int lane = threadIdx.x & 63, wave = threadIdx.x >> 6;
    const uint32_t gen = ((uint32_t)A.at.row_pos[0] * 41u + (uint32_t)A.gen) % 65535u + 1u;
    const unsigned long long ts0 = A.dbg ? __builtin_amdgcn_s_memrealtime() : 0;
    if ((int)blockIdx.x < at.nkv) {
        if (A.prio) __builtin_amdgcn_s_setprio(3);
        const int kvh = blockIdx.x, hd = at.hd, g = at.nh / at.nkv, cpos = at.cpos, half = hd >> 1;
        const int slot = at.row_slot[0];
        const bool live = wave < g;
        const int h = kvh * g + (live ? wave : 0);
        const float* tab = at.rope + (size_t)cpos * hd;
        float q0[2], q1[2], k0[2], k1[2], v0[2], v1[2], qw0[2], qw1[2], kw0[2], kw1[2], c_[2], s_[2];
#pragma unroll
        for (int u = 0; u < 2; ++u) {
            const int p = lane + 64 * u;
            const int pp = p < half ? p : 0;
            ld_pair_bf(at.qkv + (size_t)h * hd + 2 * pp, q0[u], q1[u]);
            ld_pair_bf(at.qkv + (size_t)(at.nh + kvh) * hd + 2 * pp, k0[u], k1[u]);
            ld_pair_bf(at.qkv + (size_t)(at.nh + at.nkv + kvh) * hd + 2 * pp, v0[u], v1[u]);
            if (at.qk_norm) {
                ld_pair_bf(at.qn + 2 * pp, qw0[u], qw1[u]);
                ld_pair_bf(at.kn + 2 * pp, kw0[u], kw1[u]);
            } else {
                qw0[u] = qw1[u] = kw0[u] = kw1[u] = 1.f;
            }
            c_[u] = tab[2 * pp];
            s_[u] = tab[2 * pp + 1];
            if (p >= half) q0[u] = q1[u] = k0[u] = k1[u] = v0[u] = v1[u] = 0.f;
        }
        const size_t base = (size_t)slot * at.slot_stride + at.layer_off + (size_t)kvh * at.S * hd;
        const int nck = cpos * hd / 8;
        for (int i = threadIdx.x; i < 2 * nck; i += 256) {
            const bool isv = i >= nck;
            const int c = isv ? i - nck : i;
            const u32x4_t v = *reinterpret_cast<const u32x4_t*>((isv ? at.vc : at.kc) + base + (size_t)c * 8);
            *reinterpret_cast<u32x4_t*>(kvs + (isv ? FW_MAXJ * FW_MAXHD : 0) + c * 8) = v;
        }
        auto prep = [&](float (&x0)[2], float (&x1)[2], const float (&w0)[2], const float (&w1)[2]) {
            if (at.qk_norm) {
                float ss = 0.f;
#pragma unroll
                for (int u = 0; u < 2; ++u) ss += x0[u] * x0[u] + x1[u] * x1[u];
                ss = wave_sum(ss);
                const float rs = 1.0f / sqrtf(ss / (float)hd + at.eps);
#pragma unroll
                for (int u = 0; u < 2; ++u) {
                    x0[u] = bfround((x0[u] * rs) * w0[u]);
                    x1[u] = bfround((x1[u] * rs) * w1[u]);
                }
            }
#pragma unroll
            for (int u = 0; u < 2; ++u) {
                const float y0 = bfround(x0[u] * c_[u] - x1[u] * s_[u]);
                const float y1 = bfround(x1[u] * c_[u] + x0[u] * s_[u]);
                x0[u] = y0;
                x1[u] = y1;
            }
        };
        prep(q0, q1, qw0, qw1);
        prep(k0, k1, kw0, kw1);
        if (wave == 0) {
            bf16_t* kd = at.kc + base + (size_t)cpos * hd;
            bf16_t* vd = at.vc + base + (size_t)cpos * hd;
#pragma unroll
            for (int u = 0; u < 2; ++u) {
                const int p = lane + 64 * u;
                if (p < half) {
                    *reinterpret_cast<uint32_t*>(kd + 2 * p) = (uint32_t)f2bf(k0[u]) | ((uint32_t)f2bf(k1[u]) << 16);
                    *reinterpret_cast<uint32_t*>(vd + 2 * p) = (uint32_t)f2bf(v0[u]) | ((uint32_t)f2bf(v1[u]) << 16);
                }
            }
        }
        __syncthreads();
        const unsigned long long ts1 = A.dbg ? __builtin_amdgcn_s_memrealtime() : 0;
        if (!live) return;
        const bf16_t* Ks = kvs;
        const bf16_t* Vs = kvs + FW_MAXJ * FW_MAXHD;
        float sc[FW_MAXJ + 1];
        float mx = -INFINITY;
#pragma unroll
        for (int j = 0; j <= FW_MAXJ; ++j) {
            if (j > cpos) break;
            float d = 0.f;
#pragma unroll
            for (int u = 0; u < 2; ++u) {
                const int p = lane + 64 * u;
                const int pp = p < half ? p : 0;
                float a0 = k0[u], a1 = k1[u];
                if (j < cpos) {
                    const uint32_t w = *reinterpret_cast<const uint32_t*>(Ks + j * hd + 2 * pp);
                    a0 = p < half ? lo16(w) : 0.f;
                    a1 = p < half ? hi16(w) : 0.f;
                }
                d += q0[u] * a0 + q1[u] * a1;
            }
            d = wave_sum(d);
            sc[j] = bfround(bfround(d) * at.scale);
            mx = fmaxf(mx, sc[j]);
        }
        float den = 0.f;
#pragma unroll
        for (int j = 0; j <= FW_MAXJ; ++j) {
            if (j > cpos) break;
            sc[j] = expf(sc[j] - mx);
            den += sc[j];
        }
        float o0[2] = {0.f, 0.f}, o1[2] = {0.f, 0.f};
#pragma unroll
        for (int j = 0; j <= FW_MAXJ; ++j) {
            if (j > cpos) break;
            const float pj = bfround(sc[j] / den);
#pragma unroll
            for (int u = 0; u < 2; ++u) {
                const int p = lane + 64 * u;
                const int pp = p < half ? p : 0;
                float b0 = v0[u], b1 = v1[u];
                if (j < cpos) {
                    const uint32_t w = *reinterpret_cast<const uint32_t*>(Vs + j * hd + 2 * pp);
                    b0 = lo16(w);
                    b1 = hi16(w);
                }
                o0[u] += pj * b0;
                o1[u] += pj * b1;
            }
        }
#pragma unroll
        for (int u = 0; u < 2; ++u) {
            const int p = lane + 64 * u;
            if (p < half) {
                const uint64_t w = (uint64_t)(((uint32_t)f2bf(o0[u]) << 16) | gen) |
                                   ((uint64_t)(((uint32_t)f2bf(o1[u]) << 16) | gen) << 32);
                __hip_atomic_store(reinterpret_cast<uint64_t*>(A.xt + (size_t)h * hd + 2 * p), w, __ATOMIC_RELAXED,
                                   __HIP_MEMORY_SCOPE_AGENT);
            }
        }
        if (A.dbg && lane == 0) {
            const unsigned long long t[7] = {ts0, ts1, __builtin_amdgcn_s_memrealtime(), 0, 0, 0, 0};
            dbg_record(A.dbg, 0xFFF9, (unsigned)h, t);
        }
        return;
    }
    rowgemv_body<U, 2, false, 1, G, QM, true>(A.wo, (int)blockIdx.x - at.nkv, A.xt, gen, A.err);
}

bool fattn_wo_ok(int nh, int nkv, int hd, int cpos, int N, int K, int qm) {
    const int U = rowgemv_u(K, qm);
    return nkv > 0 && nh % nkv == 0 && nh / nkv <= 4 && hd % 2 == 0 && hd <= FW_MAXHD && cpos >= 0 &&
           cpos < FW_MAXJ + 1 && K == nh * hd && N % 2 == 0 && U > 0 && U <= 8;
}

void launch_fattn_wo(hipStream_t s, const FattnWoArgs& A0) {
    FattnWoArgs A = A0;
    A.dbg = fm_tuning().dbg;
    A.wo.dbg = A.dbg;
    const FastFusedArgs<bf16_t>& at = A.at;
    const int qm = A.wo.Wq4 ? 2 : (A.wo.Wq ? 1 : 0);
    FMCHECK(fattn_wo_ok(at.nh, at.nkv, at.hd, at.cpos, A.wo.N, A.wo.K, qm) && A.xt && A.err && A.gen > 0 && A.gen <= 40 && at.row_pos &&
                A.wo.res && A.wo.res_out &&
                (qm == 2 ? (A.wo.wsz && A.wo.gs % 8 == 0 && !A.wo.bias) : (qm == 1 ? (A.wo.wscale && !A.wo.bias) : A.wo.W != nullptr)),
            "fused fast attention + wo: shapes, tag and buffers");
    const dim3 grid(at.nkv + A.wo.N / 2), block(256);
    const bool G = A.wo.residx != nullptr;
    auto go = [&](auto q) {
        constexpr int Q = decltype(q)::value;
        switch (rowgemv_u(A.wo.K, Q)) {
#define FW(u) \
    case u: (G ? fattn_wo_kernel<u, true, Q> : fattn_wo_kernel<u, false, Q>)<<<grid, block, 0, s>>>(A); break;
            FW(2) FW(3) FW(4) FW(5) FW(6)
            default: (G ? fattn_wo_kernel<8, true, Q> : fattn_wo_kernel<8, false, Q>)<<<grid, block, 0, s>>>(A); break;
#undef FW
        }
    };
    if (qm == 2) go(std::integral_constant<int, 2>{});
    else if (qm == 1) go(std::integral_constant<int, 1>{});
    else go(std::integral_constant<int, 0>{});
}
```

Before: 11.43 audio-sec/wall-sec.

## Precompute first fast-layer QKV per code and skip Q at codebook zero

For the first layer of the fast (Dual-AR inner) transformer, the QKV projection of each codebook embedding is computed once into a table and gathered by code index inside the fused attention+wo kernel. This removes one QKV GEMV per frame step. It also adds a mode for cpos 0 where attention reduces to copying V. In that mode the Q projection rows, Q norm, RoPE and softmax are skipped and only the K/V rows are computed. The table is rebuilt whenever a tuning key changes (epoch), and K/V cache loads are issued earlier in the table form. The cost is extra device memory, a one-time build, and more kernel template variants.

Result: faster. 11.67 audio-sec/wall-sec, median of 6 (+2.1%).

```diff
diff --git a/fish-speech_amd/csrc/fm_attn_dev.h b/fish-speech_amd/csrc/fm_attn_dev.h
--- a/fish-speech_amd/csrc/fm_attn_dev.h
+++ b/fish-speech_amd/csrc/fm_attn_dev.h
@@ -41,13 +41,16 @@
     const int hd = a.hd, g = a.nh / a.nkv, kvh = h / g, cpos = a.cpos, half = hd >> 1;
     const float* tab = a.rope + (size_t)cpos * hd;
     const int slot = a.row_slot[r];
+    const bool noq = a.noq && cpos == 0;
     float q0[2], q1[2], k0[2], k1[2], v0[2], v1[2], qw0[2], qw1[2], kw0[2], kw1[2], c_[2], s_[2];
 #pragma unroll
     for (int u = 0; u < 2; ++u) {
         const int p = lane + 64 * u;
         const bool ok = p < half;
         const int pp = ok ? p : 0;
-        raw_pair<T>(a.qkv, a.ldqkv, a.qslab, a.qslab_kp, gridDim.x, a.qbias, r, (size_t)h * hd + 2 * pp, q0[u], q1[u]);
+        q0[u] = q1[u] = 0.f;
+        if (!noq)
+            raw_pair<T>(a.qkv, a.ldqkv, a.qslab, a.qslab_kp, gridDim.x, a.qbias, r, (size_t)h * hd + 2 * pp, q0[u], q1[u]);
         raw_pair<T>(a.qkv, a.ldqkv, a.qslab, a.qslab_kp, gridDim.x, a.qbias, r, (size_t)(a.nh + kvh) * hd + 2 * pp,
                     k0[u], k1[u]);
         raw_pair<T>(a.qkv, a.ldqkv, a.qslab, a.qslab_kp, gridDim.x, a.qbias, r,
@@ -99,7 +102,7 @@
             x1[u] = y1;
         }
     };
-    prep(q0, q1, qw0, qw1, a.qk_norm);
+    if (!noq) prep(q0, q1, qw0, qw1, a.qk_norm);
     prep(k0, k1, kw0, kw1, a.qk_norm);
     if (a.qdbg) {
 #pragma unroll
@@ -124,6 +127,18 @@
             }
         }
     }
+    T* out = a.out + (size_t)r * a.nh * hd + (size_t)h * hd;
+    if (noq) {
+#pragma unroll
+        for (int u = 0; u < 2; ++u) {
+            const int p = lane + 64 * u;
+            if (p < half) {
+                st(out, 2 * p, 0.f + v0[u]);
+                st(out, 2 * p + 1, 0.f + v1[u]);
+            }
+        }
+        return;
+    }
     float sc[FAST_ATTN_MAXJ + 1];
     float mx = -INFINITY;
 #pragma unroll
@@ -159,7 +174,6 @@
             o1[u] += p * (j < cpos ? V1[j < FAST_ATTN_MAXJ ? j : 0][u] : v1[u]);
         }
     }
-    T* out = a.out + (size_t)r * a.nh * hd + (size_t)h * hd;
 #pragma unroll
     for (int u = 0; u < 2; ++u) {
         const int p = lane + 64 * u;
diff --git a/fish-speech_amd/csrc/fm_kernels.h b/fish-speech_amd/csrc/fm_kernels.h
--- a/fish-speech_amd/csrc/fm_kernels.h
+++ b/fish-speech_amd/csrc/fm_kernels.h
@@ -149,6 +149,7 @@
     int qslab_kp = 1;
     const T* qbias = nullptr;
     const int* row_pos = nullptr;
+    int noq = 0;
 };
 template <typename T> struct GemvArgs {
     const T* W;
@@ -260,10 +261,11 @@
     int fattn_wo = 1;
     int row_qkv_rp = 8;
     int rowgemv_q4 = 31;
-    int rowgemv = 27;
+    int rowgemv = 123;
     int row_copies = 1;
     int prefix_vec = 1;
     unsigned long long* dbg = nullptr;
+    unsigned epoch = 0;
 };
 FmTuning& fm_tuning();
 struct KvPrefixArgs {
@@ -328,6 +330,10 @@
     int cheap;
     int prio;
     unsigned long long* dbg;
+    const bf16_t* qtab;
+    const int32_t* qidx;
+    int qcol, qrows;
+    int kv0;
 };
 bool fattn_wo_ok(int nh, int nkv, int hd, int cpos, int N, int K, int qm);
 void launch_fattn_wo(hipStream_t s, const FattnWoArgs& a);
diff --git a/fish-speech_amd/csrc/fm_llm.cpp b/fish-speech_amd/csrc/fm_llm.cpp
--- a/fish-speech_amd/csrc/fm_llm.cpp
+++ b/fish-speech_amd/csrc/fm_llm.cpp
@@ -166,6 +166,10 @@
     uint32_t* fxt = nullptr;
     void* fout_rm = nullptr;
     int32_t* fiota = nullptr;
+    void* qkv0 = nullptr;
+    int32_t* qkv0_iota = nullptr;
+    unsigned qkv0_epoch = 0;
+    bool qkv0_built = false;
     struct Prefix {
         void* buf = nullptr;
         int npos = 0;
@@ -800,6 +804,81 @@
         };
         return KsbPlan{fin_ksb(d.dim, d.nq()), fin_ksb(d.dim, d.inter)};
     }
+    void qkv_row(const StackDims& d, const LayerW& L, const GemvArgs<T>& a, bool first, const void* x, int ldx,
+                 const int32_t* xidx, int xcol, void* Y, bool kv_rows) {
+        RowGemvArgs r{};
+        if (m->quant == FM_QUANT_INT4) {
+            r.Wq4 = (const uint32_t*)L.wqkv_rm;
+            r.wsz = (const uint32_t*)m->rowsz.at(L.wqkv);
+            r.gs = m->q4_gs;
+        } else {
+            r.W = (const bf16_t*)L.wqkv_rm;
+        }
+        if (first) {
+            r.X = (const bf16_t*)x;
+            r.ldx = ldx;
+            r.xidx = xidx;
+            r.xcol = xcol;
+            r.xrows = xidx ? m->cb : 0;
+        } else {
+            r.X = (const bf16_t*)x;
+        }
+        r.bias = (const bf16_t*)L.bqkv;
+        r.nw = (const bf16_t*)L.an;
+        r.eps = m->c.norm_eps;
+        r.Y = (bf16_t*)Y;
+        r.N = d.nqkv();
+        r.K = d.dim;
+        if (kv_rows) {
+            r.W += (size_t)d.nq() * d.dim;
+            if (r.bias) r.bias += d.nq();
+            r.Y += d.nq();
+            r.N -= d.nq();
+        }
+        r.pf_kc = (const bf16_t*)a.pf_kc;
+        r.pf_vc = (const bf16_t*)a.pf_vc;
+        r.pf_slot = a.pf_slot;
+        r.pf_pos = a.pf_pos;
+        r.pf_slot_stride = a.pf_slot_stride;
+        r.pf_layer_off = a.pf_layer_off;
+        r.pf_S = a.pf_S;
+        r.pf_nkv = a.pf_nkv;
+        r.pf_hd = a.pf_hd;
+        rowgemv(r, ROWGEMV_NORM_STORE);
+    }
+    bool qkv_first_row(int n) const { return row_qkv(n) && (row_bits() & 16); }
+    void qkv_first(const StackDims& d, const LayerW& L, GemvArgs<T> a, int n, const void* x_in, int ldx_in,
+                   const int32_t* xidx, int xcol, void* Y, bool kv_rows) {
+        if (qkv_first_row(n)) {
+            qkv_row(d, L, a, true, x_in, ldx_in, xidx, xcol, Y, kv_rows);
+            return;
+        }
+        a.Y = (T*)Y;
+        a.X = (const T*)x_in;
+        a.ldx = ldx_in;
+        a.xidx = xidx;
+        a.xidx_ld = m->C1;
+        a.xidx_col = xcol;
+        a.xidx_rows = xidx ? m->cb : 0;
+        gemv(a, PRO_NORM, EPI_STORE, 1, "linear");
+    }
+    GemvArgs<T> qkv_args(const StackDims& d, const LayerW& L, int n) {
+        GemvArgs<T> a = ga();
+        a.W = (const T*)L.wqkv;
+        a.bias = (const T*)L.bqkv;
+        a.nw = (const T*)L.an;
+        a.R = n;
+        a.N = d.nqkv();
+        a.K = d.dim;
+        a.Y = (T*)m->qkv;
+        a.ldy = d.nqkv();
+        return a;
+    }
+    bool qkv0_live() const {
+        return sizeof(T) == 2 && !m->quant && (row_bits() & 32) && m->qkv0 && m->qkv0_built &&
+               m->qkv0_epoch == fm_tuning().epoch;
+    }
+
     void block_small(const StackDims& d, const LayerW& L, int n, bool first, const void* x_in, int ldx_in,
                      const int32_t* xidx, int xcol, void* xb, void* hb, bool is_fast, int cpos, int layer,
                      const KsbPlan& kp, void* xo, bool kv_only = false) {
@@ -830,16 +909,14 @@
                         fattn_wo_ok(d.nh, d.nkv, d.hd, cpos, d.dim, d.nq(), fq);
         const bool att_wo = is_fast && !kv_only && fm_tuning().attn_wo && !m->quant && n == 1 && cpos < 16 && d.hd % 16 == 0 &&
                             d.hd <= 128 && d.nh % d.nkv == 0 && (d.nq() / kp.wo) % d.hd == 0 && d.nqkv() % 8 == 0;
-        {
-            GemvArgs<T> a = ga();
-            a.W = (const T*)L.wqkv;
-            a.bias = (const T*)L.bqkv;
-            a.nw = (const T*)L.an;
-            a.R = n;
-            a.N = d.nqkv();
-            a.K = d.dim;
-            a.Y = (T*)m->qkv;
-            a.ldy = d.nqkv();
+        const bool row_here = row_qkv(n) && (!first || (row_bits() & 16));
+        const bool bits56 = sizeof(T) == 2 && !m->quant && is_fast && n == 1;
+        const bool tab = bits56 && first && xidx && fw && qkv0_live();
+        const bool kv0 = bits56 && cpos == 0 && (row_bits() & 64) && row_here && !att_wo && d.hd <= 256 &&
+                         (d.nqkv() - d.nq()) % fm_tuning().row_qkv_rp == 0;
+        fa.noq = kv0;
+        if (!tab) {
+            GemvArgs<T> a = qkv_args(d, L, n);
             if (!is_fast && n == 1 && fm_tuning().kv_prefetch) {
                 a.pf_kc = (const T*)m->kc;
                 a.pf_vc = (const T*)m->vc;
@@ -861,49 +938,16 @@
                 a.pf_nkv = d.nkv;
                 a.pf_hd = d.hd;
             }
-            const int epi = EPI_STORE;
-            if (row_qkv(n) && (!first || (row_bits() & 16))) {
-                RowGemvArgs r{};
-                row_w(r, L.wqkv_rm, L.wqkv);
-                if (first) {
-                    r.X = (const bf16_t*)x_in;
-                    r.ldx = ldx_in;
-                    r.xidx = xidx;
-                    r.xcol = xcol;
-                    r.xrows = xidx ? m->cb : 0;
-                } else {
-                    r.X = (const bf16_t*)xb;
-                }
-                r.bias = (const bf16_t*)L.bqkv;
-                r.nw = (const bf16_t*)L.an;
-                r.eps = m->c.norm_eps;
-                r.Y = (bf16_t*)m->qkv;
-                r.N = d.nqkv();
-                r.K = d.dim;
-                r.pf_kc = (const bf16_t*)a.pf_kc;
-                r.pf_vc = (const bf16_t*)a.pf_vc;
-                r.pf_slot = a.pf_slot;
-                r.pf_pos = a.pf_pos;
-                r.pf_slot_stride = a.pf_slot_stride;
-                r.pf_layer_off = a.pf_layer_off;
-                r.pf_S = a.pf_S;
-                r.pf_nkv = a.pf_nkv;
-                r.pf_hd = a.pf_hd;
-                rowgemv(r, ROWGEMV_NORM_STORE);
-            } else if (first) {
-                a.X = (const T*)x_in;
-                a.ldx = ldx_in;
-                a.xidx = xidx;
-                a.xidx_ld = C1;
-                a.xidx_col = xcol;
-                a.xidx_rows = xidx ? m->cb : 0;
-                gemv(a, PRO_NORM, epi, 1, "linear");
+            if (first) {
+                qkv_first(d, L, a, n, x_in, ldx_in, xidx, xcol, m->qkv, kv0);
+            } else if (row_here) {
+                qkv_row(d, L, a, false, xb, 0, nullptr, 0, m->qkv, kv0);
             } else {
                 a.X = (const T*)xb;
                 a.ldx = d.dim;
                 a.ss_in = m->ssX;
                 a.ss_gran = rf ? 1 : 0;
-                gemv(a, PRO_PRENORM, epi, 1, "linear");
+                gemv(a, PRO_PRENORM, EPI_STORE, 1, "linear");
             }
         }
         if (!is_fast) {
@@ -960,6 +1004,13 @@
             A.delay = fm_tuning().fw_delay;
             A.cheap = fm_tuning().fw_cheap;
             A.prio = fm_tuning().fw_prio;
+            if (tab) {
+                A.qtab = (const bf16_t*)m->qkv0;
+                A.qidx = xidx;
+                A.qcol = xcol;
+                A.qrows = m->cb;
+            }
+            A.kv0 = kv0;
             chain_flush();
             const int64_t bytes = r.Wq4 ? (int64_t)r.N * r.K / 2 + (int64_t)r.N * (r.K / r.gs) * 4
                                   : (r.Wq ? (int64_t)r.N * r.K + (int64_t)r.N * 2 : (int64_t)r.N * r.K * 2);
@@ -1920,7 +1971,46 @@
                   "attention + wo; counters reset)"};
 }
 
+static void ensure_qkv0(fm_llm* m) {
+    FmTuning& t = fm_tuning();
+    if (!m->finalized || m->prec != FM_PREC_BF16 || m->quant || !(t.rowgemv & 32) || !m->fxt || m->C < 2 ||
+        !t.fattn_wo || t.gemv_chain || m->fast.empty())
+        return;
+    if (m->qkv0_built && m->qkv0_epoch == t.epoch) return;
+    const StackDims& d = m->fdm;
+    if (!m->qkv0) {
+        m->qkv0 = m->dalloc((size_t)m->cb * d.nqkv() * sizeof(bf16_t), false);
+        std::vector<int32_t> io((size_t)m->cb);
+        for (size_t i = 0; i < io.size(); ++i) io[i] = (int32_t)i;
+        m->qkv0_iota = (int32_t*)m->dalloc(io.size() * sizeof(int32_t), false);
+        HIPCHK(hipMemcpy(m->qkv0_iota, io.data(), io.size() * sizeof(int32_t), hipMemcpyHostToDevice));
+    }
+    unsigned long long* dbg = t.dbg;
+    const bool prof_on = m->prof.on;
+    t.dbg = nullptr;
+    m->prof.on = false;
+    try {
+        Run<bf16_t> r(m);
+        const GemvArgs<bf16_t> a = r.qkv_args(d, m->fast[0], 1);
+        for (int code = 0; code < m->cb; ++code)
+            r.qkv_first(d, m->fast[0], a, 1, m->femb, m->c.fast_dim, m->qkv0_iota, code,
+                        (bf16_t*)m->qkv0 + (size_t)code * d.nqkv(), false);
+        r.chain_flush();
+        HIPCHK(hipGetLastError());
+        HIPCHK(hipStreamSynchronize(m->stream));
+    } catch (...) {
+        t.dbg = dbg;
+        m->prof.on = prof_on;
+        throw;
+    }
+    t.dbg = dbg;
+    m->prof.on = prof_on;
+    m->qkv0_epoch = t.epoch;
+    m->qkv0_built = true;
+}
+
 static void launch_frame(fm_llm* m, int n) {
+    ensure_qkv0(m);
     if (m->use_graph && !m->prof.on) {
         auto it = m->graphs.find(n);
         if (it == m->graphs.end()) {
@@ -2084,6 +2174,7 @@
         FMCHECK(m, "null handle");
         HIPCHK(hipSetDevice(m->device));
         finalize(m);
+        ensure_qkv0(m);
     });
 }
 
@@ -2097,6 +2188,7 @@
     const int32_t one = slot;
     m->uploaded_slots.clear();
     HIPCHK(hipMemcpyAsync(m->frame_slot, &one, 4, hipMemcpyHostToDevice, m->stream));
+    ensure_qkv0(m);
     with_prec(m, [&](auto& r) {
         const void* last = r.prefill_slow(slot, tokens, T, pos0);
         const void* hid = r.head_small(last, false, 1, 1);
@@ -2133,6 +2225,7 @@
     for (int i = 0; i < n; ++i) reset_slot(m, slots[i], sps ? sps + i : nullptr);
     m->uploaded_slots.clear();
     HIPCHK(hipMemcpyAsync(m->frame_slot, slots, (size_t)n * 4, hipMemcpyHostToDevice, m->stream));
+    ensure_qkv0(m);
     with_prec(m, [&](auto& r) {
         r.prefill_multi(n, slots, tk.data(), T, pos0);
         if (n <= GEMV_MAX_ROWS) {
@@ -2439,6 +2532,7 @@
         HIPCHK(hipMemcpyAsync(m->frame_slot, &one, 4, hipMemcpyHostToDevice, m->stream));
         m->uploaded_slots.clear();
         std::vector<float> lg(m->Nhead);
+        ensure_qkv0(m);
         with_prec(m, [&](auto& r) {
             const void* last = r.prefill_slow(slot, x, S, pos0);
             const void* hid = r.head_small(last, false, 1, 1);
@@ -2528,6 +2622,7 @@
         FMCHECK(key, "null key");
         FmTuning& t = fm_tuning();
         const std::string k = key;
+        if (k != "debug_ts") ++t.epoch;
         if (k == "gemv_nt") {
             t.gemv_nt = value != 0;
         } else if (k == "gemv_u") {
@@ -2696,7 +2791,8 @@
         } else if (k == "row_copies") {
             t.row_copies = value != 0;
         } else if (k == "rowgemv") {
-            FMCHECK(value >= 0 && value <= 31, "rowgemv must be 0..31 (bit 0 wo / w2, bit 1 wqkv, bit 2 w1 || w3, bit 3 fast head, bit 4 first-layer wqkv)");
+            FMCHECK(value >= 0 && value <= 127, "rowgemv must be 0..127 (bit 0 wo / w2, bit 1 wqkv, bit 2 w1 || w3, bit 3 fast head, bit 4 first-layer wqkv, "
+                                                "bit 5 first fast layer's QKV from its table, bit 6 K / V only at codebook 0)");
             t.rowgemv = value;
         } else if (k == "rmsnorm_block") {
             t.rmsnorm_block = value != 0;
@@ -2736,6 +2832,7 @@
         HIPCHK(hipSetDevice(m->device));
         const int n = (int)m->uploaded_slots.size();
         const bool was_on = m->prof.on;
+        ensure_qkv0(m);
         m->prof.on = false;
         m->prof.rec.clear();
         m->prof.rec_bytes.clear();
diff --git a/fish-speech_amd/csrc/fm_rowgemv.hip b/fish-speech_amd/csrc/fm_rowgemv.hip
--- a/fish-speech_amd/csrc/fm_rowgemv.hip
+++ b/fish-speech_amd/csrc/fm_rowgemv.hip
@@ -365,9 +365,11 @@
 constexpr int FW_MAXJ = 15;
 constexpr int FW_MAXHD = 128;
 
-template <int U, bool G, int QM>
+template <int U, bool G, int QM, int M>
 __global__ __launch_bounds__(256) __attribute__((amdgpu_waves_per_eu(6)))
 void fattn_wo_kernel(FattnWoArgs A) {
+    static_assert(M == 0 || QM == 0, "table / K-V-only forms: bf16 only");
+    static_assert(2 * FW_MAXJ * FW_MAXHD / 8 <= 512, "cached rows: at most two 16-B chunks per thread");
     __shared__ __attribute__((aligned(16))) bf16_t kvs[2 * FW_MAXJ * FW_MAXHD];
     __shared__ float red[8];
     const FastFusedArgs<bf16_t>& at = A.at;
@@ -377,20 +379,43 @@
     if ((int)blockIdx.x < at.nkv) {
         if (A.prio) __builtin_amdgcn_s_setprio(3);
         const int kvh = blockIdx.x, hd = at.hd, g = at.nh / at.nkv, cpos = at.cpos, half = hd >> 1;
+        const bf16_t* qkv = at.qkv;
+        if constexpr (M == 1) {
+            const int32_t iv = A.qidx[A.qcol];
+            const int xi = iv < 0 ? 0 : (iv >= A.qrows ? A.qrows - 1 : iv);
+            qkv = A.qtab + (size_t)xi * at.ldqkv;
+        }
         const int slot = at.row_slot[0];
         const bool live = wave < g;
         const int h = kvh * g + (live ? wave : 0);
         const float* tab = at.rope + (size_t)cpos * hd;
+        const size_t base = (size_t)slot * at.slot_stride + at.layer_off + (size_t)kvh * at.S * hd;
+        const int nck = cpos * hd / 8;
+        auto kv_src = [&](int i) {
+            const bool ok = i < 2 * nck, isv = ok && i >= nck;
+            const int c = ok ? (isv ? i - nck : i) : 0;
+            return reinterpret_cast<const u32x4_t*>((isv ? at.vc : at.kc) + base + (size_t)c * 8);
+        };
+        auto kv_dst = [&](int i) {
+            const bool isv = i >= nck;
+            return reinterpret_cast<u32x4_t*>(kvs + (isv ? FW_MAXJ * FW_MAXHD : 0) + (isv ? i - nck : i) * 8);
+        };
+        u32x4_t kvr[2];
+        if constexpr (M == 1) {
+#pragma unroll
+            for (int q = 0; q < 2; ++q) kvr[q] = *kv_src((int)threadIdx.x + 256 * q);
+        }
         float q0[2], q1[2], k0[2], k1[2], v0[2], v1[2], qw0[2], qw1[2], kw0[2], kw1[2], c_[2], s_[2];
 #pragma unroll
         for (int u = 0; u < 2; ++u) {
             const int p = lane + 64 * u;
             const int pp = p < half ? p : 0;
-            ld_pair_bf(at.qkv + (size_t)h * hd + 2 * pp, q0[u], q1[u]);
-            ld_pair_bf(at.qkv + (size_t)(at.nh + kvh) * hd + 2 * pp, k0[u], k1[u]);
-            ld_pair_bf(at.qkv + (size_t)(at.nh + at.nkv + kvh) * hd + 2 * pp, v0[u], v1[u]);
+            if constexpr (M == 2) q0[u] = q1[u] = 0.f;
+            else ld_pair_bf(qkv + (size_t)h * hd + 2 * pp, q0[u], q1[u]);
+            ld_pair_bf(qkv + (size_t)(at.nh + kvh) * hd + 2 * pp, k0[u], k1[u]);
+            ld_pair_bf(qkv + (size_t)(at.nh + at.nkv + kvh) * hd + 2 * pp, v0[u], v1[u]);
             if (at.qk_norm) {
-                ld_pair_bf(at.qn + 2 * pp, qw0[u], qw1[u]);
+                if constexpr (M != 2) ld_pair_bf(at.qn + 2 * pp, qw0[u], qw1[u]);
                 ld_pair_bf(at.kn + 2 * pp, kw0[u], kw1[u]);
             } else {
                 qw0[u] = qw1[u] = kw0[u] = kw1[u] = 1.f;
@@ -399,13 +424,12 @@
             s_[u] = tab[2 * pp + 1];
             if (p >= half) q0[u] = q1[u] = k0[u] = k1[u] = v0[u] = v1[u] = 0.f;
         }
-        const size_t base = (size_t)slot * at.slot_stride + at.layer_off + (size_t)kvh * at.S * hd;
-        const int nck = cpos * hd / 8;
-        for (int i = threadIdx.x; i < 2 * nck; i += 256) {
-            const bool isv = i >= nck;
-            const int c = isv ? i - nck : i;
-            const u32x4_t v = *reinterpret_cast<const u32x4_t*>((isv ? at.vc : at.kc) + base + (size_t)c * 8);
-            *reinterpret_cast<u32x4_t*>(kvs + (isv ? FW_MAXJ * FW_MAXHD : 0) + c * 8) = v;
+        if constexpr (M == 1) {
+#pragma unroll
+            for (int q = 0; q < 2; ++q)
+                if ((int)threadIdx.x + 256 * q < 2 * nck) *kv_dst((int)threadIdx.x + 256 * q) = kvr[q];
+        } else if constexpr (M == 0) {
+            for (int i = threadIdx.x; i < 2 * nck; i += 256) *kv_dst(i) = *kv_src(i);
         }
         auto prep = [&](float (&x0)[2], float (&x1)[2], const float (&w0)[2], const float (&w1)[2]) {
             if (at.qk_norm) {
@@ -428,7 +452,7 @@
                 x1[u] = y1;
             }
         };
-        prep(q0, q1, qw0, qw1);
+        if constexpr (M != 2) prep(q0, q1, qw0, qw1);
         prep(k0, k1, kw0, kw1);
         if (wave == 0) {
             bf16_t* kd = at.kc + base + (size_t)cpos * hd;
@@ -447,6 +471,14 @@
         if (!live) return;
         const bf16_t* Ks = kvs;
         const bf16_t* Vs = kvs + FW_MAXJ * FW_MAXHD;
+        float o0[2] = {0.f, 0.f}, o1[2] = {0.f, 0.f};
+        if constexpr (M == 2) {
+#pragma unroll
+            for (int u = 0; u < 2; ++u) {
+                o0[u] = 0.f + v0[u];
+                o1[u] = 0.f + v1[u];
+            }
+        } else {
         float sc[FW_MAXJ + 1];
         float mx = -INFINITY;
 #pragma unroll
@@ -476,7 +508,6 @@
             sc[j] = expf(sc[j] - mx);
             den += sc[j];
         }
-        float o0[2] = {0.f, 0.f}, o1[2] = {0.f, 0.f};
 #pragma unroll
         for (int j = 0; j <= FW_MAXJ; ++j) {
             if (j > cpos) break;
@@ -494,6 +525,7 @@
                 o0[u] += pj * b0;
                 o1[u] += pj * b1;
             }
+        }
         }
 #pragma unroll
         for (int u = 0; u < 2; ++u) {
@@ -532,13 +564,27 @@
             "fused fast attention + wo: shapes, tag and buffers");
     const dim3 grid(at.nkv + A.wo.N / 2), block(256);
     const bool G = A.wo.residx != nullptr;
+    FMCHECK(!A.qtab || (qm == 0 && G && !A.kv0 && A.qidx == A.wo.residx && A.qcol == A.wo.res_col && A.qrows > 0 &&
+                        A.qrows == A.wo.res_rows),
+            "fused fast attention + wo: the QKV table form is bf16, gathered by the residual's index");
+    FMCHECK(!A.kv0 || (qm == 0 && !G && at.cpos == 0), "fused fast attention + wo: the K / V-only form is bf16 at codebook 0");
+    if (A.qtab || A.kv0) {
+        switch (rowgemv_u(A.wo.K, 0)) {
+#define FW(u) \
+    case u: (A.qtab ? fattn_wo_kernel<u, true, 0, 1> : fattn_wo_kernel<u, false, 0, 2>)<<<grid, block, 0, s>>>(A); break;
+            FW(2) FW(3) FW(4) FW(5) FW(6)
+            default: (A.qtab ? fattn_wo_kernel<8, true, 0, 1> : fattn_wo_kernel<8, false, 0, 2>)<<<grid, block, 0, s>>>(A); break;
+#undef FW
+        }
+        return;
+    }
     auto go = [&](auto q) {
         constexpr int Q = decltype(q)::value;
         switch (rowgemv_u(A.wo.K, Q)) {
 #define FW(u) \
-    case u: (G ? fattn_wo_kernel<u, true, Q> : fattn_wo_kernel<u, false, Q>)<<<grid, block, 0, s>>>(A); break;
+    case u: (G ? fattn_wo_kernel<u, true, Q, 0> : fattn_wo_kernel<u, false, Q, 0>)<<<grid, block, 0, s>>>(A); break;
             FW(2) FW(3) FW(4) FW(5) FW(6)
-            default: (G ? fattn_wo_kernel<8, true, Q> : fattn_wo_kernel<8, false, Q>)<<<grid, block, 0, s>>>(A); break;
+            default: (G ? fattn_wo_kernel<8, true, Q, 0> : fattn_wo_kernel<8, false, Q, 0>)<<<grid, block, 0, s>>>(A); break;
 #undef FW
         }
     };
```
